# ikergarcia1996/AI-Generated-GTAV

Measured on AMD Instinct MI355X. Metric: generated frames/sec (32-frame clip, 100 noise steps), higher is better.
Workload: dtype fp16 (fp32 accumulate/residual)

## Files before the change

### ai-generated-gtav_amd/csrc/api.hip

```cpp
#include "api_internal.h"

#include <type_traits>

namespace gtav_shared {
thread_local hipEvent_t g_launch_ev[2] = {nullptr, nullptr};
static thread_local char g_err[1024] = "";
void set_error(const char* fmt, ...) {
    va_list ap;
    va_start(ap, fmt);
    vsnprintf(g_err, sizeof(g_err), fmt, ap);
    va_end(ap);
}
const char* last_error() { return g_err; }
}

namespace {
template <class T> struct twin_arg { typedef T type; };
template <> struct twin_arg<const f16*> { typedef const __bf16* type; };
template <> struct twin_arg<f16*> { typedef __bf16* type; };
#define GTAV_TWIN_STRUCT(S)                                                                                                                     \
    static_assert(sizeof(S) == sizeof(gtav_bf16::S) && alignof(S) == alignof(gtav_bf16::S) && std::is_standard_layout<S>::value &&             \
                      std::is_standard_layout<gtav_bf16::S>::value, #S ": the fp16 and the bf16 view differ");                                  \
    template <> struct twin_arg<const S&> { typedef const gtav_bf16::S& type; };                                                                \
    template <> struct twin_arg<const S*> { typedef const gtav_bf16::S* type; };
GTAV_TWIN_STRUCT(GemmParams)
GTAV_TWIN_STRUCT(LnPending)
GTAV_TWIN_STRUCT(GemmDwGroup)
GTAV_TWIN_STRUCT(AdamParam)
GTAV_TWIN_STRUCT(AdamItem)
#undef GTAV_TWIN_STRUCT
template <class Sig, class TwinSig, TwinSig* Fn> struct twin_call;
template <class... A, class... B, int (*Fn)(B...)> struct twin_call<int(A...), int(B...), Fn> {
    static_assert((std::is_same<typename twin_arg<A>::type, B>::value && ...), "a bf16 twin's signature differs from its fp16 launcher's");
    template <class To, class From> static To cast(From a) {
        if constexpr (std::is_same<To, From>::value) return a;
        else return reinterpret_cast<To>(a);
    }
    static int call(A... a) { return Fn(cast<B, A>(a)...); }
};
#define GTAV_OPS_F16(field, launcher) &launcher,
#define GTAV_OPS_BF16(field, launcher) &twin_call<decltype(launcher), decltype(gtav_bf16::launcher), &gtav_bf16::launcher>::call,
const OperandOps OPS_F16 = {GTAV_OPERAND_OPS(GTAV_OPS_F16) false};
const OperandOps OPS_BF16 = {GTAV_OPERAND_OPS(GTAV_OPS_BF16) true};
#undef GTAV_OPS_F16
#undef GTAV_OPS_BF16
}
const OperandOps& gtav::operand_ops(bool bf16) { return bf16 ? OPS_BF16 : OPS_F16; }

static thread_local bool g_op_bf16 = false;
static const OperandOps& op_ops() { return operand_ops(g_op_bf16); }
#define GTAV_OP_F16_ONLY(name) GTAV_REQUIRE(!g_op_bf16, name ": fp16 operands only, there is no bf16 twin of this launch (gtav_op_set_operand_dtype)")

extern "C" {

const char* gtav_last_error(void) { return last_error(); }
int gtav_abi_version(void) { return 4; }

int gtav_clamp_frames(float* x, int32_t B, int32_t F, int32_t first, int32_t n, float lo, float hi, void* stream) {
    GTAV_REQUIRE(x && B >= 1 && first >= 0 && first <= F && n >= 1, "clamp_frames: bad arguments");
    if (first == F) return 0;
    GTAV_REQUIRE((int64_t)F * n < (int64_t)1 << 31, "clamp_frames: sample of %d x %d floats too large", F, n);
    return launch_clamp_cols(x, B, F * n, first * n, F * n, lo, hi, (hipStream_t)stream);
}
int gtav_ddim_update(const float* x, const float* v, float* out, int32_t rows, int32_t n, const float* alpha_t,
                     const float* alpha_next, int32_t is_final, void* stream) {
    GTAV_REQUIRE(x && v && out && alpha_t && (alpha_next || is_final), "ddim_update: null argument");
    return launch_ddim_update(x, n, v, n, out, n, rows, n, alpha_t, alpha_next, is_final, (hipStream_t)stream);
}
int gtav_add_noise(const float* x, const float* noise, const float* alpha, float* out, int32_t rows, int32_t n, float clamp_abs,
                   void* stream) {
    return launch_add_noise(x, noise, alpha, out, rows, n, clamp_abs, (hipStream_t)stream);
}
int gtav_vtarget(const float* x, const float* noise, const float* alpha, float* vt, int32_t rows, int32_t n, float clamp_abs,
                 void* stream) {
    return launch_vtarget(x, noise, alpha, vt, rows, n, clamp_abs, (hipStream_t)stream);
}
static bool aligned16(const void* p) { return ((uintptr_t)p & 15) == 0; }
#define GTAV_RNG_ROWS(name, rows, n)                                                                                                    \
// ... 409 lines not shown
```

### ai-generated-gtav_amd/csrc/api_dit.hip

```cpp
#include "api_internal.h"

#ifdef GTAV_EXPERIMENTS
static int fold_alloc(gtav_dit* h) {
    gtav_dit::Fold& f = h->fold;
    if (f.ok) return 0;
    GTAV_REQUIRE(f.geom_ok, "dit_set_fold: this geometry has no LayerNorm fold (tokens per frame %d must be a multiple of 16 and >= 64, hidden %% 256 == 0)", h->P);
    Arena& a = h->arena;
    const int D = h->D;
    const size_t Mx = round_up(h->Mmax, 128);
    int rc = 0;
#define A_(expr) do { if (!rc) rc = (expr); } while (0)
    {
        const int nhb = h->L * 2, nseam = 2 * nhb + 1;
        f.col_c.assign(nseam, 0);
        int col = 0;
        for (int hb = 0; hb < nhb; ++hb) { f.col_c[2 * hb + 1] = col; col += 2 * h->Hm; }
        for (int hb = 0; hb < nhb; ++hb) { f.col_c[2 * hb] = col; col += 2 * 3 * D; }
        f.col_c[2 * nhb] = col; col += 2 * h->Nfin;
        f.CTW = col;
        f.n_groups = 2 * nseam; f.n_groups_a = 2 * nhb;
        f.Rp = round_up(h->max_rows, 128);
        A_(a.alloc_t(&f.ctab, (size_t)h->max_rows * f.CTW));
        A_(a.alloc_t(&f.ctab_cur, (size_t)h->maxB * h->maxT * f.CTW));
        A_(a.alloc_t(&f.stats, Mx * (size_t)(D / 64) * 2));
// ... 72 lines not shown

static int dit_cond_mlp(gtav_dit* h, int rows, bool have_actions, hipStream_t s) {
    const int ldhc = h->D + h->Apad;
    RET_IF(launch_skinny_f32(h->E, 256, h->w_t0, h->b_t0, h->HC, ldhc, rows, h->D, 256, 1, s));
    RET_IF(launch_skinny_f32(h->HC, ldhc, h->w_t2cat, have_actions ? h->b_t2a : h->b_t2, h->Sc, h->D, rows, h->D, ldhc, 1, s));
    return launch_skinny_f32(h->Sc, h->D, h->w_ada, h->b_ada, h->mod, h->MODW, rows, h->MODW, h->D, 0, s);
}

static int dit_cond(gtav_dit* h, const int64_t* t64, int rows, int Tq, const StepParams* sp, int use_cur, const float* actions,
                    int64_t act_outer, int64_t act_inner, hipStream_t s) {
    GTAV_REQUIRE(rows <= h->max_rows, "conditioning rows %d exceed max_cond_rows %d", rows, h->max_rows);
    RET_IF(launch_cond_inputs(t64, rows, Tq, sp, use_cur, h->sincos, h->E, actions, act_outer, act_inner, h->A, h->HC, h->D + h->Apad,
                              h->D, h->Apad, h->err_flag, s));
    RET_IF(dit_cond_mlp(h, rows, actions != nullptr, s));
    bool fa, fb;
    fold_policy(h, rows * h->P, fa, fb);
    return dit_fold_tables(h, rows, fa, fb, s);
}

struct DitPrefetch {
    const gtav_dit* h;
    int M, Tq, t0;
    bool on;
    DitPrefetch(const gtav_dit* h_, int M_, int Tq_, int t0_) : h(h_), M(M_), Tq(Tq_), t0(t0_) {
        const int pf_max_m = 1536;
        static const int pf_min_m = GTAV_ENV_INT("GTAV_PF_MIN_M", 256);
        on = h->w_prefetch && M >= pf_min_m && M <= pf_max_m;
        fill_on = M <= pf_max_m;
    }
    bool fill_on;
    int fill(int cls) const { return fill_on ? h->w_fill_cls[cls] : 0; }
    PrefetchDesc after(int hb, int pos) const {
        const int q = pos + 1, hb2 = hb + q / 4, consumer = (q + 3) % 4;
        if (!on || hb2 >= 2 * h->L) return kNoPrefetch;
        const int v = h->w_prefetch_cls[consumer];
        if (!v) return kNoPrefetch;
        const gtav_dit::Half& w2 = h->halves[hb2];
        const int D = h->D;
        const f16* W; int N, K, sk = 1;
        if (consumer == 3) { W = dit_half_fused(h, hb2, M, Tq, t0) ? w2.w_qkv_hm : w2.w_qkv; N = 3 * D; K = D; }
        else if (consumer == 0) { W = w2.w_out; N = D; K = D; sk = gemm_choose_splitk(M, D, D); }
        else if (consumer == 1) { W = w2.w_fc1; N = h->Hm; K = D; }
        else { W = w2.w_fc2; N = D; K = h->Hm_pad; sk = gemm_choose_splitk(M, D, h->Hm_pad); }
        const int nkt = K / 64;
        if (sk < 1 || nkt % sk || (sk >= 8 ? sk % 8 : 8 % sk)) sk = 1;
        return PrefetchDesc{W, cdiv(N, 128), nkt, sk, v >= 2 ? v : 0};
    }
};

static bool dit_resid_inplace(const gtav_dit* h, int M, int K) {
    return gemm_pp_ok(M, h->D, K, EPI_RESID) || (gemm_choose_splitk(M, h->D, K) == 1 && M >= h->resid_inplace_min_m) || gemm_resid_inplace_ok(M, h->D, K, h->P);
}

static int dit_forward_core(gtav_dit* h, const float* x_src, const int* frame_index, int B, int Tq, int t0,
                            const float* mod, const int* mod_rows, const float* ctab, float* v_out, hipStream_t s) {
    const int D = h->D, P = h->P, NB = B * Tq, M = NB * P;
    GTAV_REQUIRE(M <= h->Mmax, "forward: %d tokens exceed workspace (%d)", M, h->Mmax);
    bool fold_a, fold_b;
    fold_policy(h, M, fold_a, fold_b);
    const DitPrefetch pf(h, M, Tq, t0);
    DeferredResid rd{h->parts, h->parts_rows * (size_t)D, h->resid, M, D, &h->prof, s};
    auto gate = [&](const float* g) { return ResidGate{g, h->MODW, mod_rows, P}; };
    auto ln = [&](const OperandOps& o, const float* shift, const float* scale, int* ef) -> int {
        PROF(h, PC_LN, s, o.ln_modulate(h->resid, D, h->xn, D, M, D, shift, scale, h->MODW, mod_rows, P, rd.take(), ef, s));
        return 0;
    };
    const int g_embed = 2 * h->L, g_final = 2 * h->L + 1;
    PROF(h, PC_OTHER, s, h->ops(g_embed).patchify(x_src, frame_index, NB, h->C, h->H, h->W, h->p, h->xp, h->Kpe, 1.f, 0.f, h->err_of(g_embed), s));
    GemmParams pe = gemm_params(h->xp, h->Kpe, h->w_pe, M, D, h->Kpe);
    pe.bias = h->b_pe; pe.out = h->resid; pe.ldo = D;
    PROF(h, PC_OTHER, s, h->ops(g_embed).gemm(pe, EPI_F32, s));
    bool folded_in = false;
    for (int hb = 0; hb < 2 * h->L; ++hb) {
        const int l = hb / 2, hf = hb % 2;
        const gtav_dit::Half& w = h->halves[hb];
        const OperandOps& ops = h->ops(hb);
        int* const ef = h->err_of(hb);
        const float* mb = mod + (size_t)hb * 6 * D;
        const bool fused = dit_half_fused(h, hb, M, Tq, t0), fused_t = fused && hf == 1, fused_s = fused && hf == 0 && !folded_in;
        if (fused_t) rd.permute_rows(Tq, P);
        if (!folded_in) RET_IF(ln(ops, mb, mb + D, ef));
        GemmParams g = gemm_params(h->xn, D, fused_t || fused_s ? w.w_qkv_hm : w.w_qkv, M, 3 * D, D);
        g.D = D; g.S = P; g.err_flag = ef; g.pf = pf.after(hb, 0); g.wfill = pf.fill(3);
        if (folded_in) fold_consumer(h, g, 2 * hb, 3 * D, mod_rows, ctab);
        if (hf == 0) { g.qkv_mode = QKV_SPATIAL; g.rope_cs = h->rope_s.cs_dev; }
        else { g.qkv_mode = QKV_TEMPORAL; g.k = h->kvcache[l]; g.v = h->kvcache[l]; g.Tq = Tq; g.t0 = t0; g.Tmax = h->maxT; g.rope_cs = h->rope_t.cs_dev; }
        if (fused_t || fused_s) {
            g.out = h->ao; g.ldo = D;
            if (fused_t) PROF(h, PC_ATTN_T, s, launch_gemm_qkvt_attn(g, s));
            else PROF(h, PC_ATTN_S, s, launch_gemm_qkvs_attn(g, s));
        } else {
            if (hf == 0) { g.q = h->qs; g.k = h->ks; g.v = h->vts; }
            else g.q = h->qt;
            PROF(h, PC_QKV, s, ops.gemm(g, folded_in ? EPI_QKV_FOLD : EPI_QKV, s));
            if (hf == 0) PROF(h, PC_ATTN_S, s, ops.attn_spatial(h->qs, h->ks, h->vts, h->ao, NB, h->heads, P, s, false));
            else PROF(h, PC_ATTN_T, s, ops.attn_temporal(h->qt, h->kvcache[l], h->ao, B, P, D, Tq, t0, h->maxT, s));
        }
        folded_in = false;
        GemmParams fc1 = gemm_params(h->xn, D, w.w_fc1, M, h->Hm, D);
        fc1.bias = w.b_fc1; fc1.out = h->hbuf; fc1.ldo = h->Hm_pad; fc1.err_flag = ef; fc1.pf = pf.after(hb, 2); fc1.wfill = pf.fill(1);
        if (fold_a) {
            RET_IF(fold_producer(h, PC_OUT, h->ao, w.w_out, M, D, w.b_out, gate(mb + 2 * D), mb + 4 * D, s));
            fold_consumer(h, fc1, 2 * hb + 1, h->Hm, mod_rows, ctab);
            PROF(h, PC_FC1, s, launch_gemm(fc1, EPI_GELU_TANH_FOLD, s));
        } else {
            RET_IF(rd.gemm(ops, PC_OUT, h->ao, D, w.w_out, D, w.b_out, gate(mb + 2 * D), dit_resid_inplace(h, M, D), pf.after(hb, 1), nullptr, nullptr, pf.fill(0)));
            RET_IF(ln(ops, mb + 3 * D, mb + 4 * D, ef));
            PROF(h, PC_FC1, s, ops.gemm(fc1, EPI_GELU_TANH, s));
        }
        if (fold_b) {
            const float* next_scale = hb + 1 < 2 * h->L ? mod + (size_t)(hb + 1) * 6 * D + D : mod + (size_t)h->L * 12 * D + D;
            RET_IF(fold_producer(h, PC_FC2, h->hbuf, w.w_fc2, M, h->Hm_pad, w.b_fc2, gate(mb + 5 * D), next_scale, s));
            folded_in = true;
        } else {
            RET_IF(rd.gemm(ops, PC_FC2, h->hbuf, h->Hm_pad, w.w_fc2, h->Hm_pad, w.b_fc2, gate(mb + 5 * D), dit_resid_inplace(h, M, h->Hm_pad), pf.after(hb, 3), nullptr, nullptr, pf.fill(2)));
        }
    }
    const float* mf = mod + (size_t)h->L * 12 * D;
    if (!folded_in) RET_IF(ln(h->ops(g_final), mf, mf + D, h->err_of(g_final)));
    GemmParams fin = gemm_params(h->xn, D, h->w_final, M, h->Nfin, D);
    fin.bias = h->b_final; fin.out = h->fo; fin.ldo = h->Nfin;
    if (folded_in) fold_consumer(h, fin, 4 * h->L, h->Nfin, mod_rows, ctab);
    PROF(h, PC_OTHER, s, h->ops(g_final).gemm(fin, folded_in ? EPI_F32_FOLD : EPI_F32, s));
    PROF(h, PC_OTHER, s, launch_unpatchify(h->fo, h->Nfin, v_out, NB, h->C, h->H, h->W, h->p, 0, 1.f, 0.f, s));
    return h->prof.collect(s);
}

extern "C" {

int gtav_dit_create(const gtav_dit_config* c, gtav_dit** out) {
    GTAV_REQUIRE(c && out, "dit_create: null argument");
    GTAV_REQUIRE(c->hidden_size % 256 == 0 && c->hidden_size <= 2048, "hidden_size=%d must be a multiple of 256, <= 2048", c->hidden_size);
    GTAV_REQUIRE(c->num_heads > 0 && c->hidden_size / c->num_heads == 64 && c->hidden_size % c->num_heads == 0,
                 "only head_dim 64 is implemented (hidden %d, heads %d)", c->hidden_size, c->num_heads);
    GTAV_REQUIRE(c->input_h % c->patch_size == 0 && c->input_w % c->patch_size == 0, "input %dx%d not divisible by patch %d",
                 c->input_h, c->input_w, c->patch_size);
    GTAV_REQUIRE(c->max_frames >= 1 && c->max_frames <= 32, "max_frames=%d must be in [1, 32]", c->max_frames);
    GTAV_REQUIRE(c->max_batch >= 1 && c->depth >= 1, "bad max_batch/depth");
    RET_IF(skinny_init());
    gtav_dit* h = new gtav_dit();
    h->cfg = *c;
    h->D = c->hidden_size; h->L = c->depth; h->heads = c->num_heads; h->C = c->in_channels; h->p = c->patch_size;
    h->H = c->input_h; h->W = c->input_w; h->gh = h->H / h->p; h->gw = h->W / h->p; h->P = h->gh * h->gw;
    const int D = h->D;
    if ((h->P % 8) != 0) {
        set_error("tokens per frame P=%d must be a multiple of 8", h->P);
        delete h;
        return 2;
    }
    h->Hm = (int)(D * c->mlp_ratio); h->Hm_pad = round_up(h->Hm, 128);
    h->A = c->external_cond_dim > 0 ? c->external_cond_dim : 0; h->Apad = round_up(h->A > 0 ? h->A : 1, 32);
    h->MODW = h->L * 12 * D + 2 * D;
    h->Kpe = round_up(h->C * h->p * h->p, 64);
    h->Nfin = h->p * h->p * h->C;
    h->maxB = c->max_batch; h->maxT = c->max_frames; h->Mmax = h->maxB * h->maxT * h->P;
    h->max_rows = c->max_cond_rows > h->maxB * h->maxT ? c->max_cond_rows : h->maxB * h->maxT;
    Arena& a = h->arena;
    WeightTable& wt = h->wt;
    int rc = 0;
#define A_(expr) do { if (!rc) rc = (expr); } while (0)
    A_(a.alloc_t(&h->w_pe, (size_t)round_up(D, 128) * h->Kpe));
    h->n_groups = 2 * h->L + 2;
    h->grp_bf16.assign(h->n_groups, 0);
    wt.add_f16("x_embedder.proj.weight", D, h->C * h->p * h->p, h->w_pe, round_up(D, 128), h->Kpe, 2 * h->L);
    A_(a.alloc_t(&h->b_pe, D)); wt.add_f32("x_embedder.proj.bias", 1, D, h->b_pe, D);
    A_(a.alloc_t(&h->w_t0, (size_t)D * 256)); wt.add_f32("t_embedder.mlp.0.weight", D, 256, h->w_t0, 256);
    A_(a.alloc_t(&h->b_t0, D)); wt.add_f32("t_embedder.mlp.0.bias", 1, D, h->b_t0, D);
    const int ldhc = D + h->Apad;
    A_(a.alloc_t(&h->w_t2cat, (size_t)D * ldhc)); wt.add_f32("t_embedder.mlp.2.weight", D, D, h->w_t2cat, ldhc, 0);
    A_(a.alloc_t(&h->b_t2, D)); wt.add_f32("t_embedder.mlp.2.bias", 1, D, h->b_t2, D);
    A_(a.alloc_t(&h->b_ext, D)); A_(a.alloc_t(&h->b_t2a, D));
    if (h->A > 0) {
        wt.add_f32("external_cond.weight", D, h->A, h->w_t2cat, ldhc, D);
        wt.add_f32("external_cond.bias", 1, D, h->b_ext, D);
    }
// ... 1 lines not shown
    h->halves.resize(h->L * 2);
    h->fuse_sattn = h->P == 144 && D % 256 == 0;
    for (int l = 0; l < h->L && !rc; ++l)
        for (int hf = 0; hf < 2; ++hf) {
            gtav_dit::Half& w = h->halves[l * 2 + hf];
            char pre[64];
            snprintf(pre, sizeof(pre), "blocks.%d.%c_", l, hf == 0 ? 's' : 't');
            std::string P_(pre);
            const int grp = l * 2 + hf;
            A_(a.alloc_t(&w.w_qkv, (size_t)3 * D * D)); wt.add_f16(P_ + "attn.to_qkv.weight", 3 * D, D, w.w_qkv, 3 * D, D, grp);
            w.w_qkv_hm = nullptr;
            if (hf == 0 && h->P == 144 && D % 256 == 0) A_(a.alloc_t(&w.w_qkv_hm, (size_t)3 * D * D));
            A_(a.alloc_t(&w.w_out, (size_t)D * D)); wt.add_f16(P_ + "attn.to_out.weight", D, D, w.w_out, D, D, grp);
            A_(a.alloc_t(&w.b_out, D)); wt.add_f32(P_ + "attn.to_out.bias", 1, D, w.b_out, D);
            A_(a.alloc_t(&w.w_fc1, (size_t)h->Hm_pad * D)); wt.add_f16(P_ + "mlp.fc1.weight", h->Hm, D, w.w_fc1, h->Hm_pad, D, grp);
            A_(a.alloc_t(&w.b_fc1, h->Hm_pad)); wt.add_f32(P_ + "mlp.fc1.bias", 1, h->Hm, w.b_fc1, h->Hm);
            A_(a.alloc_t(&w.w_fc2, (size_t)D * h->Hm_pad)); wt.add_f16(P_ + "mlp.fc2.weight", D, h->Hm, w.w_fc2, D, h->Hm_pad, grp);
            A_(a.alloc_t(&w.b_fc2, D)); wt.add_f32(P_ + "mlp.fc2.bias", 1, D, w.b_fc2, D);
            const size_t row0 = (size_t)(l * 2 + hf) * 6 * D;
            wt.add_f32(P_ + "adaLN_modulation.1.weight", 6 * D, D, h->w_ada + row0 * D, D);
            wt.add_f32(P_ + "adaLN_modulation.1.bias", 1, 6 * D, h->b_ada + row0, 6 * D);
        }
    A_(a.alloc_t(&h->w_final, (size_t)round_up(h->Nfin, 128) * D));
    wt.add_f16("final_layer.linear.weight", h->Nfin, D, h->w_final, round_up(h->Nfin, 128), D, 2 * h->L + 1);
    A_(a.alloc_t(&h->b_final, round_up(h->Nfin, 128))); wt.add_f32("final_layer.linear.bias", 1, h->Nfin, h->b_final, h->Nfin);
    {
        const size_t row0 = (size_t)h->L * 12 * D;
        wt.add_f32("final_layer.adaLN_modulation.1.weight", 2 * D, D, h->w_ada + row0 * D, D);
        wt.add_f32("final_layer.adaLN_modulation.1.bias", 1, 2 * D, h->b_ada + row0, 2 * D);
    }
    A_(a.alloc_t(&h->sincos, (size_t)1000 * 256)); wt.add_f32("tables.timestep_sincos", 1000, 256, h->sincos, 256, 0, false);
    h->rope_s.npos = h->P; h->rope_t.npos = h->maxT;
    A_(a.alloc_t(&h->rope_s.cos_dev, (size_t)h->P * 64)); wt.add_f32("tables.rope_spatial_cos", h->P, 64, h->rope_s.cos_dev, 64, 0, false);
    A_(a.alloc_t(&h->rope_s.sin_dev, (size_t)h->P * 64)); wt.add_f32("tables.rope_spatial_sin", h->P, 64, h->rope_s.sin_dev, 64, 0, false);
    A_(a.alloc_t(&h->rope_t.cos_dev, (size_t)h->maxT * 64)); wt.add_f32("tables.rope_temporal_cos", h->maxT, 64, h->rope_t.cos_dev, 64, 0, false);
    A_(a.alloc_t(&h->rope_t.sin_dev, (size_t)h->maxT * 64)); wt.add_f32("tables.rope_temporal_sin", h->maxT, 64, h->rope_t.sin_dev, 64, 0, false);
    A_(a.alloc_t(&h->rope_s.cs_dev, (size_t)h->P * 64)); A_(a.alloc_t(&h->rope_t.cs_dev, (size_t)h->maxT * 64));
    A_(a.alloc_t(&h->freqs_s_dev, 16)); wt.add_f32("spatial_rotary_emb.freqs", 1, 16, h->freqs_s_dev, 16, 0, false);
    A_(a.alloc_t(&h->freqs_t_dev, 32)); wt.add_f32("temporal_rotary_emb.freqs", 1, 32, h->freqs_t_dev, 32, 0, false);
    const size_t Mx = round_up(h->Mmax, 128);
    A_(a.alloc_t(&h->xp, Mx * h->Kpe)); A_(a.alloc_t(&h->xn, Mx * D)); A_(a.alloc_t(&h->qs, Mx * D)); A_(a.alloc_t(&h->ks, Mx * D));
    A_(a.alloc_t(&h->vts, Mx * D)); A_(a.alloc_t(&h->qt, Mx * D)); A_(a.alloc_t(&h->ao, Mx * D)); A_(a.alloc_t(&h->hbuf, Mx * h->Hm_pad));
    h->kvcache.resize(h->L);
    for (int l = 0; l < h->L; ++l) A_(a.alloc_t(&h->kvcache[l], Mx * 2 * D));
    A_(a.alloc_t(&h->resid, Mx * D)); A_(a.alloc_t(&h->fo, Mx * h->Nfin));
    A_(a.alloc_t(&h->vout, Mx / h->P * h->C * h->H * h->W));
    h->parts_rows = (2 * Mx * D > (size_t)(8u << 20) ? 2 * Mx * D : (size_t)(8u << 20)) / D;
    A_(a.alloc_t(&h->parts, h->parts_rows * D));
    const size_t R = h->max_rows;
    A_(a.alloc_t(&h->E, R * 256)); A_(a.alloc_t(&h->HC, R * ldhc)); A_(a.alloc_t(&h->Sc, R * D)); A_(a.alloc_t(&h->mod, R * h->MODW));
    A_(a.alloc_t(&h->err_flag, 4 + h->n_groups)); A_(a.alloc_t(&h->frame_idx, (size_t)h->maxB * h->maxT)); A_(a.alloc_t(&h->ac_table, 1000));
    A_(a.alloc_t(&h->step_dev, 4)); A_(a.alloc_t(&h->mod_rows_dev, (size_t)h->maxB * h->maxT));
    A_(a.alloc_t(&h->mod_cur, (size_t)h->maxB * h->maxT * h->MODW)); A_(a.alloc_t(&h->mod_last, (size_t)h->maxB * h->maxT)); A_(a.alloc_t(&h->mod_changed, (size_t)h->maxB * h->maxT)); A_(a.alloc_t(&h->t_steps_dev, 1024));
    wt.err_words = h->err_flag; wt.err_per_group = true;
    h->use_graph = GTAV_ENV_INT("GTAV_GRAPH", 1) != 0;
    h->fold.geom_ok = h->P % 16 == 0 && h->P >= 64 && D % 256 == 0 && h->Hm % 128 == 0 && h->Nfin % 4 == 0;
#undef A_
    if (rc) {
        delete h;
        return rc;
    }
    *out = h;
    return 0;
}

void gtav_dit_destroy(gtav_dit* h) { delete h; }

int gtav_dit_set_weight(gtav_dit* h, const char* name, const float* src, int64_t numel, void* stream) {
    GTAV_REQUIRE(h && name && src, "dit_set_weight: null argument");
    std::string n(name);
    if (n.size() > 16 && n.compare(n.size() - 16, 16, "rotary_emb.freqs") == 0) {
        const bool spatial = n.rfind("spatial_", 0) == 0 || n.find(".s_attn.") != std::string::npos;
        n = spatial ? "spatial_rotary_emb.freqs" : "temporal_rotary_emb.freqs";
    }
    h->finalized = false;
    return h->wt.set(n.c_str(), src, numel, (hipStream_t)stream);
}

int gtav_dit_get_weight(gtav_dit* h, const char* name, float* dst, int64_t numel, void* stream) {
    GTAV_REQUIRE(h && name && dst, "dit_get_weight: null argument");
    return h->wt.get(name, dst, numel, (hipStream_t)stream);
}

int gtav_dit_finalize(gtav_dit* h, void* stream) {
    GTAV_REQUIRE(h, "dit_finalize: null handle");
    hipStream_t s = (hipStream_t)stream;
    RET_IF(h->wt.check_complete());
    GTAV_CHECK_HIP(hipStreamSynchronize(s));
    const int D = h->D;
    RET_IF(launch_add_f32(h->b_t2, h->b_ext, h->b_t2a, D, s));
    std::vector<float> fs(16), ft(32);
    if (h->wt.is_set("spatial_rotary_emb.freqs")) GTAV_CHECK_HIP(hipMemcpy(fs.data(), h->freqs_s_dev, 64, hipMemcpyDeviceToHost));
    else { std::vector<float> l = linspace_f32(1.0f, 128.0f, 16); for (int i = 0; i < 16; ++i) fs[i] = l[i] * (float)M_PI; }
    if (h->wt.is_set("temporal_rotary_emb.freqs")) GTAV_CHECK_HIP(hipMemcpy(ft.data(), h->freqs_t_dev, 128, hipMemcpyDeviceToHost));
    else for (int i = 0; i < 32; ++i) ft[i] = 1.0f / powf(10000.0f, (float)(2 * i) / 64.0f);
    if (!(h->wt.is_set("tables.rope_spatial_cos") && h->wt.is_set("tables.rope_spatial_sin"))) {
        std::vector<float> c, sn;
        build_axial_table(fs, h->gh, h->gw, c, sn);
        RET_IF(upload(h->rope_s.cos_dev, c)); RET_IF(upload(h->rope_s.sin_dev, sn));
    }
    if (!(h->wt.is_set("tables.rope_temporal_cos") && h->wt.is_set("tables.rope_temporal_sin"))) {
        std::vector<float> c((size_t)h->maxT * 64), sn((size_t)h->maxT * 64);
        for (int t = 0; t < h->maxT; ++t)
            for (int d = 0; d < 64; ++d) {
                const float ang = (float)t * ft[d / 2];
                c[t * 64 + d] = cosf(ang); sn[t * 64 + d] = sinf(ang);
            }
        RET_IF(upload(h->rope_t.cos_dev, c)); RET_IF(upload(h->rope_t.sin_dev, sn));
    }
    if (!h->wt.is_set("tables.timestep_sincos")) {
        std::vector<float> tab((size_t)1000 * 256);
        for (int k = 0; k < 128; ++k) {
            const float f = expf(-logf(10000.0f) * (float)k / 128.0f);
            for (int t = 0; t < 1000; ++t) {
                const float arg = (float)t * f;
                tab[(size_t)t * 256 + k] = cosf(arg);
                tab[(size_t)t * 256 + 128 + k] = sinf(arg);
            }
        }
        RET_IF(upload(h->sincos, tab));
    }
    for (size_t hb = 0; hb < h->halves.size(); ++hb) {
        gtav_dit::Half& w = h->halves[hb];
        if (w.w_qkv_hm) RET_IF(launch_qkv_head_major(w.w_qkv, w.w_qkv_hm, D, s, (hb & 1) ? 0 : 1));
    }
    RET_IF(launch_rope_interleave(h->rope_s.cos_dev, h->rope_s.sin_dev, h->rope_s.cs_dev, h->P, s));
    RET_IF(launch_rope_interleave(h->rope_t.cos_dev, h->rope_t.sin_dev, h->rope_t.cs_dev, h->maxT, s));
    GTAV_CHECK_HIP(hipStreamSynchronize(s));
    h->finalized = true;
    return 0;
}

int gtav_dit_forward(gtav_dit* h, const float* x, const int64_t* t, const float* actions, float* out, int32_t B, int32_t T,
                     void* stream) {
    GTAV_REQUIRE(h && x && t && out, "dit_forward: null argument");
    GTAV_REQUIRE(h->finalized, "dit_forward: call gtav_dit_finalize first");
    GTAV_REQUIRE(B >= 1 && B <= h->maxB && T >= 1 && T <= h->maxT, "dit_forward: B=%d T=%d outside capacity (%d, %d)", B, T, h->maxB, h->maxT);
    GTAV_REQUIRE(!actions || h->A > 0, "dit_forward: model has no external_cond");
    hipStream_t s = (hipStream_t)stream;
    h->prepared.valid = false;
    h->kvrec.valid = false;
    RET_IF(dit_cond(h, t, B * T, 1, nullptr, 0, actions, h->A, 0, s));
    return dit_forward_core(h, x, nullptr, B, T, 0, h->mod, nullptr, h->fold.ctab, out, s);
}

int gtav_dit_set_schedule(gtav_dit* h, const float* ac, int32_t n) {
    GTAV_REQUIRE(h && ac && n == 1000, "dit_set_schedule: expected 1000 alphas_cumprod values");
    h->ac_host.assign(ac, ac + n);
    GTAV_CHECK_HIP(hipMemcpy(h->ac_table, ac, n * sizeof(float), hipMemcpyHostToDevice));
    return 0;
}

static int denoise_step_body(gtav_dit* h, float* x, int B, int F, int T, const float* actions, int mode, float* v_out,
                             bool prepared, hipStream_t s) {
    const size_t fsz = (size_t)h->C * h->H * h->W;
    const int Tq = mode == 1 ? 1 : T, t0 = mode == 1 ? T - 1 : 0;
    if (!prepared) RET_IF(dit_cond(h, nullptr, B * Tq, Tq, h->step_dev, mode == 1, actions, (int64_t)F * h->A, h->A, s));
    RET_IF(dit_forward_core(h, x, h->frame_idx, B, Tq, t0, prepared ? h->mod_cur : h->mod, nullptr, prepared ? h->fold.ctab_cur : h->fold.ctab, h->vout, s));
    const float* vlast = h->vout + (size_t)(Tq - 1) * fsz;
    RET_IF(launch_ddim_update_step(x, F, vlast, (size_t)Tq * fsz, B, (int)fsz, h->step_dev, s));
    if (v_out) RET_IF(launch_copy_rows_f32(vlast, (size_t)Tq * fsz, v_out, fsz, B, fsz, s));
    return 0;
}

int gtav_dit_prepare_frame(gtav_dit* h, int32_t B, int32_t F, int32_t start, int32_t cur, int32_t t_ctx,
                           const int32_t* t_steps_host, int32_t n_steps, const float* actions, void* stream) {
    GTAV_REQUIRE(h && t_steps_host, "prepare_frame: null argument");
    GTAV_REQUIRE(h->finalized, "prepare_frame: finalize the model first");
    const int T = cur - start + 1;
    GTAV_REQUIRE(start >= 0 && cur < F && T >= 1 && T <= h->maxT && B >= 1 && B <= h->maxB && n_steps >= 1 && n_steps <= 1024,
                 "prepare_frame: bad window [%d, %d] / steps %d", start, cur, n_steps);
    GTAV_REQUIRE(!actions || h->A > 0, "prepare_frame: model has no external_cond");
    const int rows = B * (T - 1) + n_steps * B;
    GTAV_REQUIRE(rows <= h->max_rows, "prepare_frame: %d conditioning rows exceed max_cond_rows %d", rows, h->max_rows);
    hipStream_t s = (hipStream_t)stream;
    GTAV_CHECK_HIP(hipStreamSynchronize(s));
    GTAV_CHECK_HIP(hipMemcpy(h->t_steps_dev, t_steps_host, n_steps * sizeof(int), hipMemcpyHostToDevice));
    RET_IF(launch_cond_inputs_frame(rows, B, T, F, start, cur, t_ctx, h->t_steps_dev, h->sincos, h->E, actions, h->A, h->HC, h->D + h->Apad,
                                    h->D, h->Apad, h->err_flag, s));
    RET_IF(dit_cond_mlp(h, rows, actions != nullptr, s));
    {
        bool fa, fb, fa1, fb1;
        fold_policy(h, B * T * h->P, fa, fb);
        fold_policy(h, B * h->P, fa1, fb1);
        RET_IF(dit_fold_tables(h, rows, fa || fa1, fb || fb1, s));
        h->prepared.fold_tables = fa || fa1 || fb || fb1;
    }
    GTAV_CHECK_HIP(hipMemsetAsync(h->mod_last, 0xFF, (size_t)h->maxB * h->maxT * sizeof(int), s));
    h->prepared.valid = true; h->prepared.B = B; h->prepared.F = F; h->prepared.start = start; h->prepared.cur = cur;
    h->prepared.n_steps = n_steps; h->prepared.actions = actions;
    return 0;
}

static int dit_step_graph(gtav_dit* h, float* x, int B, int F, int T, const float* actions, int mode, float* v_out, bool prepared, hipGraphExec_t* out) {
    *out = nullptr;
    const gtav_dit::GraphKey key{B, F, T, mode * 2 + (prepared ? 1 : 0), x, actions, v_out};
    auto it = h->graphs.find(key);
    if (it == h->graphs.end()) {
        if (h->graphs.size() > 64) h->drop_graphs();
        h->graphs[key] = nullptr;
        return 0;
    }
    *out = it->second;
    if (*out) return 0;
    hipGraph_t graph = nullptr;
    hipGraphExec_t exec = nullptr;
    int rc = 0;
    bool ok = h->cap_stream || hipStreamCreateWithFlags(&h->cap_stream, hipStreamNonBlocking) == hipSuccess;
    if (ok && hipStreamBeginCapture(h->cap_stream, hipStreamCaptureModeThreadLocal) != hipSuccess) {
        (void)hipGetLastError();
        ok = false;
    } else if (ok) {
        rc = denoise_step_body(h, x, B, F, T, actions, mode, v_out, prepared, h->cap_stream);
        ok = hipStreamEndCapture(h->cap_stream, &graph) == hipSuccess && !rc && graph;
        ok = ok && hipGraphInstantiate(&exec, graph, nullptr, nullptr, 0) == hipSuccess && exec;
        if (graph) (void)hipGraphDestroy(graph);
    }
    if (ok) *out = it->second = exec;
    else h->use_graph = false;
    return rc;
}

int gtav_dit_denoise_step(gtav_dit* h, float* x, int32_t B, int32_t F, int32_t start, int32_t cur, int32_t t_ctx,
                          int32_t t_cur, int32_t t_next, int32_t is_final, const float* actions, int32_t mode,
                          int32_t cond_step, float* v_out, void* stream) {
    GTAV_REQUIRE(h && x, "denoise_step: null argument");
    GTAV_REQUIRE(h->finalized && !h->ac_host.empty(), "denoise_step: finalize the model and set the schedule first");
    const int T = cur - start + 1;
    GTAV_REQUIRE(start >= 0 && cur < F && T >= 1 && T <= h->maxT && B >= 1 && B <= h->maxB, "denoise_step: bad window [%d, %d] of %d frames", start, cur, F);
    GTAV_REQUIRE(t_cur >= 0 && t_cur < 1000 && t_next >= 0 && t_next < 1000 && t_ctx >= 0 && t_ctx < 1000, "denoise_step: timestep out of range");
    GTAV_REQUIRE(!actions || h->A > 0, "denoise_step: model has no external_cond");
    GTAV_REQUIRE(mode == 0 || mode == 1, "denoise_step: mode %d", mode);
    const bool prepared = cond_step >= 0;
    if (prepared)
        GTAV_REQUIRE(h->prepared.valid && h->prepared.B == B && h->prepared.F == F && h->prepared.start == start &&
                         h->prepared.cur == cur && cond_step < h->prepared.n_steps && h->prepared.actions == actions,
                     "denoise_step: cond_step=%d but gtav_dit_prepare_frame was not called for this window", cond_step);
    else
        h->prepared.valid = false;
    if (mode == 1) {
        GTAV_REQUIRE(h->kvrec.valid && h->kvrec.B == B && h->kvrec.F == F && h->kvrec.start == start && h->kvrec.cur == cur &&
                         h->kvrec.x == (const void*)x,
                     "denoise_step: context-cached step (mode 1) on window [%d, %d] without a preceding full-window step (mode 0) "
                     "on the same batch / window / latent buffer: the temporal K/V caches would be stale", start, cur);
    } else {
        h->kvrec.valid = true; h->kvrec.B = B; h->kvrec.F = F; h->kvrec.start = start; h->kvrec.cur = cur; h->kvrec.x = x;
    }
    hipStream_t s = (hipStream_t)stream;
    StepParams sp;
    sp.first = start; sp.cur = cur; sp.t_ctx = t_ctx; sp.t_cur = t_cur; sp.is_final = is_final != 0;
    sp.alpha_t = h->ac_host[t_cur]; sp.alpha_next = h->ac_host[t_next]; sp.cond_step = cond_step;
    RET_IF(launch_step_setup(h->step_dev, sp, h->frame_idx, h->mod_rows_dev, prepared ? h->mod_last : nullptr, h->mod_changed, B, mode == 1 ? 1 : T, T, F,
                             mode == 1, s));
    if (prepared) RET_IF(launch_gather_rows(h->mod, h->mod_rows_dev, h->mod_changed, h->mod_cur, B * (mode == 1 ? 1 : T), h->MODW,
                                            h->prepared.fold_tables ? h->fold.ctab : nullptr, h->fold.ctab_cur, h->fold.CTW, s));
    hipGraphExec_t exec = nullptr;
    if (h->use_graph && !h->prof.on) RET_IF(dit_step_graph(h, x, B, F, T, actions, mode, v_out, prepared, &exec));
    if (!exec) return denoise_step_body(h, x, B, F, T, actions, mode, v_out, prepared, s);
    GTAV_CHECK_HIP(hipGraphLaunch(exec, s));
    return 0;
}

int gtav_dit_set_graph(gtav_dit* h, int32_t enable) {
    GTAV_REQUIRE(h, "dit_set_graph: null handle");
    h->use_graph = enable != 0;
    return 0;
}

int gtav_dit_set_weight_prefetch(gtav_dit* h, int32_t enable) {
    GTAV_REQUIRE(h, "dit_set_weight_prefetch: null handle");
    GTAV_REQUIRE(enable == 0 || enable == 1 || (enable >> 16) == 1,
                 "dit_set_weight_prefetch: mode %d (0 off, 1 on, 0x10000 | per-class nibbles: bits 0-3 out-proj's weight, 4-7 fc1's, 8-11 fc2's, 12-15 to_qkv's; "
                 "nibble 0 = not prefetched, 1 = the whole slice, k >= 2 = the first k K tiles of every row tile)", enable);
    int cls[4];
    for (int c = 0; c < 4; ++c) cls[c] = enable == 0 ? 0 : enable == 1 ? 1 : (enable >> (4 * c)) & 15;
    const bool on = cls[0] || cls[1] || cls[2] || cls[3];
    if (h->w_prefetch != on || memcmp(cls, h->w_prefetch_cls, sizeof(cls))) h->drop_graphs();
    h->w_prefetch = on;
    memcpy(h->w_prefetch_cls, cls, sizeof(cls));
    return 0;
}

int gtav_dit_set_weight_fill_policy(gtav_dit* h, int32_t mode) {
    GTAV_REQUIRE(h, "dit_set_weight_fill_policy: null handle");
    GTAV_REQUIRE((mode & ~0x1111) == 0,
                 "dit_set_weight_fill_policy: mode %d (one nibble per class: bits 0-3 out-proj's weight, 4-7 fc1's, 8-11 fc2's, 12-15 to_qkv's; "
                 "nibble 0 = default cache policy, 1 = non-temporal fills)", mode);
    int cls[4];
    for (int c = 0; c < 4; ++c) cls[c] = (mode >> (4 * c)) & 15;
    if (memcmp(cls, h->w_fill_cls, sizeof(cls))) h->drop_graphs();
    memcpy(h->w_fill_cls, cls, sizeof(cls));
    return 0;
}

#ifdef GTAV_EXPERIMENTS
int gtav_dit_set_fold(gtav_dit* h, int32_t mode, int32_t min_tokens_a, int32_t min_tokens_b) {
    GTAV_REQUIRE(h && mode >= 0 && mode <= 2, "dit_set_fold: mode %d", mode);
    if (min_tokens_a >= 0) h->fold.min_m_a = min_tokens_a;
    if (min_tokens_b >= 0) h->fold.min_m_b = min_tokens_b;
    if (mode == 2 || (mode == 1 && (h->fold.min_m_a < (1 << 30) || h->fold.min_m_b < (1 << 30)))) RET_IF(fold_alloc(h));
    h->drop_graphs();
    h->prepared.valid = false;
    h->fold.mode = mode;
    return 0;
}
#endif

static int dit_set_fused(gtav_dit* h, bool& flag, int hf, bool geom_ok, bool enable) {
    if (flag != enable) h->drop_graphs();
    if (enable && geom_ok) {
        for (int l = 0; l < h->L; ++l) {
            gtav_dit::Half& w = h->halves[l * 2 + hf];
            if (w.w_qkv_hm) continue;
            RET_IF(h->arena.alloc_t(&w.w_qkv_hm, (size_t)3 * h->D * h->D));
            if (h->finalized) RET_IF(launch_qkv_head_major(w.w_qkv, w.w_qkv_hm, h->D, nullptr, hf ? 0 : 1));
        }
        if (h->finalized) GTAV_CHECK_HIP(hipDeviceSynchronize());
    }
    flag = enable;
    return 0;
}
int gtav_dit_set_fused_temporal(gtav_dit* h, int32_t enable) {
    GTAV_REQUIRE(h, "dit_set_fused_temporal: null handle");
    return dit_set_fused(h, h->fuse_tattn, 1, h->P % 16 == 0 && h->D % 256 == 0 && h->maxT >= 5, enable != 0);
}
int gtav_dit_set_fused_spatial(gtav_dit* h, int32_t enable) {
    GTAV_REQUIRE(h, "dit_set_fused_spatial: null handle");
    return dit_set_fused(h, h->fuse_sattn, 0, h->P == 144 && h->D % 256 == 0, enable != 0);
}

int gtav_dit_fused_launches(gtav_dit* h, int32_t B, int32_t T, int32_t t0) {
    if (!h || B < 1 || T < 1) return 0;
    int mask = 0;
    for (int hb = 0; hb < 2 * h->L; ++hb)
        if (dit_half_fused(h, hb, B * T * h->P, T, t0)) mask |= (hb & 1) ? 2 : 1;
    return mask;
}

int gtav_dit_profile(gtav_dit* h, int32_t enable) {
    GTAV_REQUIRE(h, "dit_profile: null handle");
    h->prof.reset(enable != 0);
    return 0;
}
int gtav_dit_profile_read(gtav_dit* h, double* ms_by_class, int64_t* launches_by_class) {
    GTAV_REQUIRE(h && ms_by_class && launches_by_class, "dit_profile_read: null argument");
    h->prof.read(ms_by_class, launches_by_class);
    return 0;
}

static int dit_read_err_words(gtav_dit* h, std::vector<int>& words, hipStream_t s) {
    words.assign(4 + h->n_groups, 0);
    GTAV_CHECK_HIP(hipMemcpyAsync(words.data(), h->err_flag, words.size() * sizeof(int), hipMemcpyDeviceToHost, s));
    GTAV_CHECK_HIP(hipStreamSynchronize(s));
    GTAV_CHECK_HIP(hipMemsetAsync(h->err_flag, 0, words.size() * sizeof(int), s));
    return 0;
}

int gtav_dit_check(gtav_dit* h, void* stream) {
    GTAV_REQUIRE(h, "dit_check: null handle");
    std::vector<int> w;
    RET_IF(dit_read_err_words(h, w, (hipStream_t)stream));
    int flag = w[0] | w[1];
    for (int g = 0; g < h->n_groups; ++g) flag |= w[4 + g];
    return report_err_flag(flag, "DiT");
}

int gtav_dit_set_operand_dtype(gtav_dit* h, int32_t group, int32_t dtype) {
    GTAV_REQUIRE(h, "dit_set_operand_dtype: null handle");
    GTAV_REQUIRE(dtype == GTAV_OPERAND_F16 || dtype == GTAV_OPERAND_BF16, "dit_set_operand_dtype: dtype %d (0 = fp16, 1 = bf16)", dtype);
    GTAV_REQUIRE(group >= -1 && group < h->n_groups, "dit_set_operand_dtype: group %d outside [-1, %d)", group, h->n_groups);
    if (h->tr.on && h->tr.bf16)
        GTAV_REQUIRE(dtype == GTAV_OPERAND_BF16, "dit_set_operand_dtype: a bf16 training handle keeps bf16 operands in every group (its masters, optimizer state and "
                     "loss scale were set up for them; create a new handle to train on fp16 operands)");
    else
        GTAV_REQUIRE(!h->tr.on || dtype == GTAV_OPERAND_F16, "dit_set_operand_dtype: a training handle keeps fp16 operands (its backward pass and loss scaling are fp16)");
    int changed = 0;
    for (int g = (group < 0 ? 0 : group); g < (group < 0 ? h->n_groups : group + 1); ++g) {
        if ((h->grp_bf16[g] != 0) == (dtype == GTAV_OPERAND_BF16)) continue;
        GTAV_REQUIRE(!(h->tr.on && h->tr.mixed), "dit_set_operand_dtype: group %d of this training handle has the other type; a training handle changes it with "
                     "gtav_dit_train_set_group_dtype", g);
        h->grp_bf16[g] = dtype == GTAV_OPERAND_BF16;
        changed += 1 + h->wt.set_dtype(g, dtype == GTAV_OPERAND_BF16);
    }
    if (changed) {
        h->finalized = false;
        h->kvrec.valid = false;
        h->drop_graphs();
    }
    h->any_bf16 = false;
    for (unsigned char b : h->grp_bf16) h->any_bf16 |= b != 0;
    return 0;
}

int gtav_dit_get_operand_dtype(gtav_dit* h, int32_t group, int32_t* dtype) {
    GTAV_REQUIRE(h && dtype && group >= 0 && group < h->n_groups, "dit_get_operand_dtype: bad argument (group %d of %d)", group, h ? h->n_groups : 0);
    *dtype = h->grp_bf16[group] ? GTAV_OPERAND_BF16 : GTAV_OPERAND_F16;
    return 0;
}

int gtav_dit_operand_groups(gtav_dit* h, int32_t* n_groups) {
    GTAV_REQUIRE(h && n_groups, "dit_operand_groups: null argument");
    *n_groups = h->n_groups;
    return 0;
}

int gtav_dit_autorange(gtav_dit* h, int32_t* n_switched, void* stream) {
    GTAV_REQUIRE(h && n_switched, "dit_autorange: null argument");
    *n_switched = 0;
    std::vector<int> w;
    RET_IF(dit_read_err_words(h, w, (hipStream_t)stream));
    int other = w[0];
    for (int g = 0; g < h->n_groups; ++g) {
        other |= w[4 + g] & ~ERR_F16_SAT;
        if ((w[4 + g] & ERR_F16_SAT) && !h->grp_bf16[g]) {
            RET_IF(gtav_dit_set_operand_dtype(h, g, GTAV_OPERAND_BF16));
            *n_switched += 1;
        }
    }
    return report_err_flag(other, "DiT");
}

}
```

### ai-generated-gtav_amd/csrc/api_internal.h

```cpp
#pragma once
#include "../../include/gtav_amd.h"
#include "../../include/gtav_amd_testing.h"
#include "ops.h"
#include "ops_bf16.h"

#include <cmath>
#include <cstdarg>
#include <cstdio>
#include <cstdlib>
#include <cstring>
#include <map>
#include <string>
#include <tuple>
#include <vector>

using namespace gtav;

#define RET_IF(expr)            \
    do {                        \
        int _rc = (expr);       \
        if (_rc) return _rc;    \
    } while (0)

namespace gtav {
// ... 268 lines not shown
        GTAV_REQUIRE(!pending, "train_block_forward: a re-run starts from a stored block input");
        memset(&pend, 0, sizeof(pend));
        pend.k_load = k;
        pending = true;
        return 0;
    }
};

}
}
using namespace gtav::api;

struct gtav_dit {
    Profiler prof;
    gtav_dit_config cfg;
    int D, L, heads, P, gh, gw, C, p, H, W, Hm, Hm_pad, A, Apad, MODW, Kpe, Nfin, maxB, maxT, Mmax, max_rows;
    Arena arena;
    WeightTable wt;
    f16 *w_pe = nullptr, *w_final = nullptr;
    struct Half { f16 *w_qkv, *w_out, *w_fc1, *w_fc2; float *b_out, *b_fc1, *b_fc2; f16* w_qkv_hm; };
    std::vector<Half> halves;
    float *b_pe = nullptr, *b_final = nullptr;
    float *w_t0, *b_t0, *w_t2cat, *b_t2, *b_ext, *b_t2a, *w_ada, *b_ada;
    float* sincos = nullptr;
    bool sincos_set = false;
    RopeTable rope_s, rope_t;
    std::vector<float> freqs_s, freqs_t;
    float *freqs_s_dev = nullptr, *freqs_t_dev = nullptr;
    f16 *xp, *xn, *qs, *ks, *vts, *qt, *ao, *hbuf;
    std::vector<f16*> kvcache;
    float *resid, *fo, *vout, *E, *HC, *Sc, *mod, *parts;
    size_t parts_rows = 0;
    int* err_flag = nullptr;
    std::vector<unsigned char> grp_bf16;
    int n_groups = 0;
    bool any_bf16 = false;
    const OperandOps& ops(int g) const { return operand_ops(grp_bf16[g] != 0); }
    int* err_of(int g) const { return err_flag + 4 + g; }
    int* frame_idx = nullptr;
    StepParams* step_dev = nullptr;
    int* mod_rows_dev = nullptr;
    float* mod_cur = nullptr;
    int *mod_last = nullptr, *mod_changed = nullptr;
    int* t_steps_dev = nullptr;
    struct { bool valid = false, fold_tables = false; int B = 0, F = 0, start = 0, cur = 0, n_steps = 0; const float* actions = nullptr; } prepared;
    struct { bool valid = false; int B = 0, F = 0, start = 0, cur = 0; const void* x = nullptr; } kvrec;
    struct GraphKey {
        int B, F, T, mode;
        const void *x, *actions, *vout;
        bool operator<(const GraphKey& o) const {
            return std::tie(B, F, T, mode, x, actions, vout) < std::tie(o.B, o.F, o.T, o.mode, o.x, o.actions, o.vout);
        }
    };
    std::map<GraphKey, hipGraphExec_t> graphs;
    bool use_graph = true;
    bool fuse_tattn = false;
    bool fuse_sattn = false;
    bool w_prefetch = true;
    int w_prefetch_cls[4] = {1, 4, 4, 1};
    int w_fill_cls[4] = {0, 0, 0, 0};
    int resid_inplace_min_m = GTAV_ENV_INT("GTAV_RESID_INPLACE_MIN_M", 1 << 30);
    struct Fold {
        bool geom_ok = false;
        bool ok = false;
        int mode = 1;
        int min_m_a = 1 << 30, min_m_b = 1 << 30;
        int CTW = 0, n_groups = 0, n_groups_a = 0, Rp = 0;
        std::vector<int> col_c;
        float *ctab = nullptr, *ctab_cur = nullptr, *stats = nullptr;
        f16* sx = nullptr;
        GemmGroup* groups_dev = nullptr;
        int *gcol_dev = nullptr, *gscale_dev = nullptr;
    } fold;
    hipStream_t cap_stream = nullptr;
    void drop_graphs() {
        for (auto& kv : graphs)
            if (kv.second) (void)hipGraphExecDestroy(kv.second);
        graphs.clear();
    }
    ~gtav_dit() {
        drop_graphs();
        if (cap_stream) (void)hipStreamDestroy(cap_stream);
    }
    float* ac_table = nullptr;
    std::vector<float> ac_host;
    bool finalized = false;
    struct Train {
        bool on = false, have_fwd = false, have_actions = false;
        bool bf16 = false;
        bool mixed = false;
        int* range_words = nullptr;
        std::vector<AdamItem> adam_items_host;
        int adam_n[2] = {0, 0};
        int window = 8;
        bool recompute = false;
        int rc_block = -1;
        std::vector<float*> kshift;
        size_t saved_bytes = 0;
        int B = 0, T = 0, M = 0, Mp = 0, rows = 0;
        float loss_scale = 65536.0f;
        float grad_div = 1.0f;
        std::vector<Slot*> params;
        struct Linear { Slot *w = nullptr, *b = nullptr; };
        struct HalfSlots { Linear qkv, out, fc1, fc2, ada; };
        std::vector<HalfSlots> hs;
        Linear fin, fin_ada, pe, t0, t2, ext;
        float* grad_arena = nullptr;
        size_t grad_count = 0;
        float* ctl = nullptr;
        float *ln_part = nullptr;
        float *red_ws = nullptr, *sumsq_part = nullptr;
        size_t red_ws_floats = 0;
        AdamParam* adam_params = nullptr;
        AdamItem* adam_items = nullptr;
        int adam_n_items = 0;
        std::vector<float*> res;
        struct HB { f16 *xnA, *ao, *y1, *xnB, *u, *hh, *y2, *q, *k, *v; };
        std::vector<HB> hb;
        f16 *xnF = nullptr, *xp = nullptr;
        float *z0 = nullptr, *cpre = nullptr;
        float *dres = nullptr, *dtmp = nullptr, *stats = nullptr, *dmod = nullptr, *dSc = nullptr, *ada_part = nullptr, *dc = nullptr, *dh0 = nullptr, *dz0 = nullptr;
        f16 *g_d = nullptr, *g_d2 = nullptr, *g_h = nullptr, *g_u = nullptr, *g_qkv = nullptr, *dao = nullptr, *tA = nullptr, *tB = nullptr, *dfo = nullptr;
        f16 *tAg[4] = {nullptr, nullptr, nullptr, nullptr}, *tBg[4] = {nullptr, nullptr, nullptr, nullptr};
    } tr;
};
```

### ai-generated-gtav_amd/csrc/api_train.hip

```cpp
#include "api_internal.h"

static int g_dw_grouped = GTAV_ENV_INT("GTAV_DW_GROUPED", 1);
static int g_fuse_gelu_fwd = GTAV_ENV_INT("GTAV_FUSE_GELU_FWD", 1);
static int g_fuse_gelu = GTAV_ENV_INT("GTAV_FUSE_GELU_BWD", 1);
static int g_fuse_ln = GTAV_ENV_INT("GTAV_FUSE_LN_BWD", 1);
static int g_fuse_gate = GTAV_ENV_INT("GTAV_FUSE_GATE", 1);
static int g_dw_tn = GTAV_ENV_INT("GTAV_DW_TN", 1);

static int train_window_ok(const gtav_dit* h) {
    if (h->tr.window > 8) {
        GTAV_REQUIRE(h->maxT <= h->tr.window, "train_enable: gtav_dit_train_allow_window allowed training windows of at most %d frames on this handle; it was created "
                     "with max_frames=%d", h->tr.window, h->maxT);
        return 0;
    }
    GTAV_REQUIRE(h->maxT <= 8, "train_enable: training is implemented for windows of at most 8 frames (the backward temporal attention and the adaLN-gradient "
                 "reduction are sized for it); this handle was created with max_frames=%d", h->maxT);
    return 0;
}

static int train_linear(gtav_dit* h, const std::string& n, gtav_dit::Train::Linear* out, bool bias = true) {
    out->w = h->wt.find(n + ".weight");
    out->b = bias ? h->wt.find(n + ".bias") : nullptr;
    GTAV_REQUIRE(out->w && out->w->grad && (!bias || (out->b && out->b->grad)), "train_enable: the model has no trainable Linear '%s'", n.c_str());
    return 0;
// ... 260 lines not shown
    RET_IF(train_branch_seam(h, i - 1, gn, rd, s));
    RET_IF(h->ops(gn).ln_modulate(tr.res[2 * i - 1], D, last ? tr.xnF : tr.g_d, D, tr.M, D, mb, mb + D, h->MODW, nullptr, h->P, rd.take(), train_fwd_err(h, gn), s));
    tr.rc_block = l;
    return 0;
}

extern "C" {


int gtav_dit_train_param_count(gtav_dit* h, int64_t* numel) {
    GTAV_REQUIRE(h && numel, "train_param_count: null argument");
    int64_t c = 0;
    for (auto& kv : h->wt.slots)
        if (WeightTable::trainable_name(kv.first)) c += (int64_t)kv.second.R * kv.second.C;
    *numel = c;
    return 0;
}

int gtav_dit_set_loss_scale(gtav_dit* h, float scale) {
    GTAV_REQUIRE(h && scale > 0.f, "set_loss_scale: bad argument");
    h->tr.loss_scale = scale;
    return 0;
}

int gtav_dit_set_grad_divisor(gtav_dit* h, float divisor) {
    GTAV_REQUIRE(h && h->tr.on && divisor >= 1.0f, "set_grad_divisor: bad argument");
    h->tr.grad_div = divisor;
    return 0;
}
int gtav_dit_zero_grad(gtav_dit* h, void* stream) {
    GTAV_REQUIRE(h && h->tr.on, "zero_grad: training is not enabled");
    RET_IF(launch_fill_f32(h->tr.grad_arena, h->tr.grad_count, 0.f, (hipStream_t)stream));
    if (h->tr.mixed) RET_IF(launch_err_fold(h->err_flag, nullptr, 1, h->n_groups, (hipStream_t)stream));
    return launch_err_clear(h->err_flag, ERR_F16_SAT | ERR_NONFINITE, (hipStream_t)stream);
}

int gtav_dit_get_grad(gtav_dit* h, const char* name, float* dst, int64_t numel, void* stream) {
    GTAV_REQUIRE(h && name && dst && h->tr.on, "get_grad: bad argument / training is not enabled");
    auto it = h->wt.slots.find(name);
    GTAV_REQUIRE(it != h->wt.slots.end() && it->second.grad, "get_grad: '%s' is not a trainable parameter", name);
    GTAV_REQUIRE(numel == (int64_t)it->second.R * it->second.C, "get_grad: '%s' size mismatch", name);
    GTAV_CHECK_HIP(hipMemcpyAsync(dst, it->second.grad, numel * sizeof(float), hipMemcpyDeviceToDevice, (hipStream_t)stream));
    return 0;
}

int gtav_dit_train_forward(gtav_dit* h, const float* x, const int64_t* t64, const float* actions, float* out, int32_t B, int32_t T, void* stream) {
    GTAV_REQUIRE(h && x && t64 && out, "train_forward: null argument");
    GTAV_REQUIRE(h->tr.on && h->finalized, "train_forward: call gtav_dit_train_enable, load the weights and finalize first");
    GTAV_REQUIRE(B >= 1 && B <= h->maxB && T >= 1 && T <= h->maxT, "train_forward: B=%d T=%d outside capacity (%d, %d)", B, T, h->maxB, h->maxT);
    GTAV_REQUIRE(!actions || h->A > 0, "train_forward: model has no external_cond");
    hipStream_t s = (hipStream_t)stream;
    gtav_dit::Train& tr = h->tr;
    const int D = h->D, P = h->P, NB = B * T, M = NB * P, L = h->L, rows = NB, ldhc = D + h->Apad;
    h->prepared.valid = false;
    h->kvrec.valid = false;
    tr.rc_block = -1;
    RET_IF(launch_cond_inputs(t64, rows, 1, nullptr, 0, h->sincos, h->E, actions, h->A, 0, h->A, h->HC, ldhc, D, h->Apad, h->err_flag, s));
    RET_IF(launch_skinny_f32(h->E, 256, h->w_t0, h->b_t0, tr.z0, D, rows, D, 256, 0, s));
    RET_IF(launch_silu(tr.z0, D, h->HC, ldhc, rows, D, s));
    RET_IF(launch_skinny_f32(h->HC, ldhc, h->w_t2cat, actions ? h->b_t2a : h->b_t2, tr.cpre, D, rows, D, ldhc, 0, s));
    RET_IF(launch_silu(tr.cpre, D, h->Sc, D, rows, D, s));
    RET_IF(launch_skinny_f32(h->Sc, D, h->w_ada, h->b_ada, h->mod, h->MODW, rows, h->MODW, D, 0, s));
    const float* mod = h->mod;
    const OperandOps& oe = h->ops(2 * L), &ofin = h->ops(2 * L + 1);
    RET_IF(oe.patchify(x, nullptr, NB, h->C, h->H, h->W, h->p, tr.xp, h->Kpe, 1.f, 0.f, train_fwd_err(h, 2 * L), s));
    GemmParams g = gemm_params(tr.xp, h->Kpe, h->w_pe, M, D, h->Kpe);
    g.bias = h->b_pe; g.out = tr.res[0]; g.ldo = D;
    RET_IF(oe.gemm(g, EPI_F32, s));
    DeferredResid rd{h->parts, h->parts_rows * (size_t)D, nullptr, M, D, nullptr, s};
    for (int l = 0; l < L; ++l) RET_IF(train_block_forward(h, l, B, T, false, rd, s));
    const float* mf = mod + (size_t)L * 12 * D;
    RET_IF(train_branch_seam(h, 2 * L - 1, 2 * L + 1, rd, s));
    RET_IF(ofin.ln_modulate(tr.res[4 * L - 1], D, tr.xnF, D, M, D, mf, mf + D, h->MODW, nullptr, P, rd.take(), train_fwd_err(h, 2 * L + 1), s));
    g = gemm_params(tr.xnF, D, h->w_final, M, h->Nfin, D);
    g.bias = h->b_final; g.out = h->fo; g.ldo = h->Nfin;
    RET_IF(ofin.gemm(g, EPI_F32, s));
    RET_IF(launch_unpatchify(h->fo, h->Nfin, out, NB, h->C, h->H, h->W, h->p, 0, 1.f, 0.f, s));
    if (tr.mixed) RET_IF(launch_err_fold(h->err_flag, tr.range_words, 0, h->n_groups, s));
    tr.B = B; tr.T = T; tr.M = M; tr.Mp = round_up(M, 64); tr.rows = rows; tr.have_actions = actions != nullptr; tr.have_fwd = true;
    tr.rc_block = L - 1;
    return 0;
}

int gtav_dit_train_get_residual(gtav_dit* h, int32_t k, float* dst, int64_t numel, void* stream) {
    GTAV_REQUIRE(h && dst && h->tr.on && h->tr.have_fwd, "train_get_residual: no saved forward");
    GTAV_REQUIRE(k >= 0 && k <= 4 * h->L, "train_get_residual: k=%d must be in [0, %d]", k, 4 * h->L);
    GTAV_REQUIRE(!h->tr.recompute || k % 4 == 0, "train_get_residual: k=%d is a state inside a block, which a handle in recompute mode (gtav_dit_train_set_recompute) "
                 "does not keep: k must be a multiple of 4 (block inputs, 4 * depth = the input of the final layer)", k);
    GTAV_REQUIRE(numel == (int64_t)h->tr.M * h->D, "train_get_residual: expected %lld elements", (long long)h->tr.M * h->D);
    GTAV_CHECK_HIP(hipMemcpyAsync(dst, h->tr.res[k], numel * sizeof(float), hipMemcpyDeviceToDevice, (hipStream_t)stream));
    return 0;
}

}

struct TrainBackward {
    gtav_dit* h;
    gtav_dit::Train& tr;
    hipStream_t s;
    const int D, P, L, B, T, M, Mp, NB, rows, Hp, MODW;
    const OperandOps* op;
    bool defer_dw = false, tn_dw, fuse_ln, fuse_gate, defer_bias;
    GemmDwGroup dwg[GEMM_DW_MAX_GROUPS];
    int ndw = 0;

    TrainBackward(gtav_dit* h_, hipStream_t s_)
        : h(h_), tr(h_->tr), s(s_), D(h->D), P(h->P), L(h->L), B(tr.B), T(tr.T), M(tr.M), Mp(tr.Mp), NB(B * T), rows(tr.rows), Hp(h->Hm_pad), MODW(h->MODW), op(&h->ops(2 * L + 1)) {
// ... 147 lines not shown
    GTAV_REQUIRE(h && v_pred && v_target, "train_backward: null argument");
    GTAV_REQUIRE(h->tr.on && h->tr.have_fwd, "train_backward: no saved forward (gtav_dit_train_forward)");
    GTAV_REQUIRE(phase_begin >= 0 && phase_begin <= phase_end && phase_end <= h->L + 2, "train_backward: phases [%d, %d) outside [0, %d]", phase_begin, phase_end,
                 h->L + 2);
    GTAV_REQUIRE(h->Nfin <= 64, "train_backward: a final projection wider than 64 features is not implemented");
    TrainBackward bw(h, (hipStream_t)stream);
    const int L = h->L;
    if (phase_begin <= 0 && 0 < phase_end) RET_IF(bw.final_layer(v_pred, v_target));
    for (int i = 2 * L - 1; i >= 0; --i) {
        const int l = i / 2, phase = L - l;
        if (phase < phase_begin || phase >= phase_end) continue;
        if (h->tr.recompute && h->tr.rc_block != l) RET_IF(train_rerun_block(h, l, bw.s));
        RET_IF(bw.half_block(i));
    }
    if (phase_begin <= L + 1 && L + 1 < phase_end) RET_IF(bw.embedders());
    return 0;
}

int gtav_dit_train_backward(gtav_dit* h, const float* v_pred, const float* v_target, void* stream) {
    GTAV_REQUIRE(h, "train_backward: null handle");
    return gtav_dit_train_backward_phases(h, v_pred, v_target, 0, h->L + 2, stream);
}

int gtav_dit_train_param_range(gtav_dit* h, const char* prefix, int64_t* offset, int64_t* count) {
    GTAV_REQUIRE(h && prefix && offset && count && h->tr.on, "train_param_range: bad argument / training is not enabled");
    const size_t plen = strlen(prefix);
    int64_t off = -1, cnt = 0, last_end = -1;
    for (auto& kv : h->wt.slots) {
        Slot& sl = kv.second;
        if (!sl.grad || kv.first.compare(0, plen, prefix) != 0) continue;
        const int64_t o = sl.grad - h->tr.grad_arena, n = (int64_t)sl.R * sl.C;
        if (off < 0) off = o;
        GTAV_REQUIRE(last_end < 0 || o == last_end, "train_param_range: parameters with prefix '%s' are not contiguous in the arena", prefix);
        last_end = o + n;
        cnt += n;
    }
    GTAV_REQUIRE(off >= 0, "train_param_range: no trainable parameter starts with '%s'", prefix);
    *offset = off;
    *count = cnt;
    return 0;
}

int gtav_dit_adamw_step(gtav_dit* h, float lr, float beta1, float beta2, float eps, float weight_decay, float max_grad_norm, void* stream) {
    GTAV_REQUIRE(h && h->tr.on, "adamw_step: training is not enabled");
    hipStream_t s = (hipStream_t)stream;
    gtav_dit::Train& tr = h->tr;
    if (tr.mixed) RET_IF(launch_err_fold(h->err_flag, tr.range_words, 0, h->n_groups, s));
    RET_IF(launch_sumsq(tr.grad_arena, tr.grad_count, tr.sumsq_part, s));
    RET_IF(launch_clip_coef(tr.ctl, tr.sumsq_part, sumsq_parts(tr.grad_count), 1.0f / (tr.loss_scale * tr.grad_div), max_grad_norm, beta1, beta2, h->err_flag, s));
    for (int ty = 0; ty < 2; ++ty)
        if (tr.adam_n[ty])
            RET_IF(operand_ops(ty != 0).adamw_multi(tr.adam_params, tr.adam_items + (ty ? tr.adam_n[0] : 0), tr.adam_n[ty], tr.ctl, lr, beta1, beta2, eps, weight_decay, s));
    RET_IF(launch_add_f32(h->b_t2, h->b_ext, h->b_t2a, h->D, s));
    h->prepared.valid = false;
    h->kvrec.valid = false;
    return 0;
}

}

static int train_partition_items(gtav_dit* h) {
    gtav_dit::Train& tr = h->tr;
    bool any_f16 = false;
    for (unsigned char b : h->grp_bf16) any_f16 |= b == 0;
    std::vector<AdamItem> part[2];
    for (const AdamItem& it : tr.adam_items_host) {
        const Slot* sl = tr.params[it.param];
        part[sl->kind == SLOT_F16_PAD ? (sl->bf16 ? 1 : 0) : (any_f16 ? 0 : 1)].push_back(it);
    }
    tr.adam_n[0] = (int)part[0].size(); tr.adam_n[1] = (int)part[1].size();
    part[0].insert(part[0].end(), part[1].begin(), part[1].end());
    GTAV_REQUIRE((int)part[0].size() == tr.adam_n_items, "train_set_group_dtype: the optimizer's work items do not add up");
    GTAV_CHECK_HIP(hipMemcpy(tr.adam_items, part[0].data(), part[0].size() * sizeof(AdamItem), hipMemcpyHostToDevice));
    return 0;
}

static int train_switch_groups(gtav_dit* h, int g0, int g1, bool bf16, hipStream_t s, int* n_changed) {
    int changed = 0;
    for (int g = g0; g < g1; ++g) {
        if ((h->grp_bf16[g] != 0) == bf16) continue;
        h->grp_bf16[g] = bf16;
        ++changed;
        for (auto& kv : h->wt.slots) {
            Slot& sl = kv.second;
            if (sl.kind != SLOT_F16_PAD || sl.group != g) continue;
            sl.bf16 = bf16;
            if (!sl.set) continue;
            GTAV_REQUIRE(sl.master, "train_set_group_dtype: '%s' has no fp32 master", kv.first.c_str());
            RET_IF(operand_ops(bf16).convert_pad(sl.master, sl.C, sl.R, sl.C, (f16*)sl.dst, sl.Rp, sl.Cp, 1.0f, 1, s, h->tr.range_words + g));
            if (sl.wT) RET_IF(operand_ops(bf16).convert_T(sl.master, sl.C, sl.R, sl.C, sl.wT, s));
        }
    }
    *n_changed = changed;
    if (!changed) return 0;
    h->any_bf16 = false;
    for (unsigned char b : h->grp_bf16) h->any_bf16 |= b != 0;
    h->tr.have_fwd = false;
    h->tr.rc_block = -1;
    h->prepared.valid = false;
    h->kvrec.valid = false;
    h->drop_graphs();
    GTAV_CHECK_HIP(hipStreamSynchronize(s));
    return train_partition_items(h);
}

static int train_mixed_handle(gtav_dit* h, const char* who) {
    GTAV_REQUIRE(h, "%s: null handle", who);
    GTAV_REQUIRE(h->tr.on, "%s: training is not enabled", who);
    GTAV_REQUIRE(h->tr.mixed, "%s: this training handle has one operand type for every group; opt in with gtav_dit_train_allow_mixed between gtav_dit_create and "
                 "gtav_dit_train_enable", who);
    return 0;
}

extern "C" {

int gtav_dit_train_set_group_dtype(gtav_dit* h, int32_t group, int32_t dtype, void* stream) {
    RET_IF(train_mixed_handle(h, "train_set_group_dtype"));
    GTAV_REQUIRE(dtype == GTAV_OPERAND_F16 || dtype == GTAV_OPERAND_BF16, "train_set_group_dtype: dtype %d (0 = fp16, 1 = bf16)", dtype);
    GTAV_REQUIRE(group >= -1 && group < h->n_groups, "train_set_group_dtype: group %d outside [-1, %d)", group, h->n_groups);
    int n = 0;
    return train_switch_groups(h, group < 0 ? 0 : group, group < 0 ? h->n_groups : group + 1, dtype == GTAV_OPERAND_BF16, (hipStream_t)stream, &n);
}

int gtav_dit_train_range_words(gtav_dit* h, int32_t* words_host, void* stream) {
    RET_IF(train_mixed_handle(h, "train_range_words"));
    GTAV_REQUIRE(words_host, "train_range_words: null argument");
    hipStream_t s = (hipStream_t)stream;
    static_assert(sizeof(int32_t) == sizeof(int), "the error words are 32-bit");
    GTAV_CHECK_HIP(hipMemcpyAsync(words_host, h->tr.range_words, (size_t)h->n_groups * sizeof(int), hipMemcpyDeviceToHost, s));
    GTAV_CHECK_HIP(hipStreamSynchronize(s));
    GTAV_CHECK_HIP(hipMemsetAsync(h->tr.range_words, 0, (size_t)h->n_groups * sizeof(int), s));
    return 0;
}

int gtav_dit_train_autorange(gtav_dit* h, const int32_t* merged_words_host, int32_t* n_switched, void* stream) {
    RET_IF(train_mixed_handle(h, "train_autorange"));
    GTAV_REQUIRE(n_switched, "train_autorange: null argument");
    *n_switched = 0;
    hipStream_t s = (hipStream_t)stream;
    std::vector<int32_t> sticky(h->n_groups, 0);
    if (merged_words_host) sticky.assign(merged_words_host, merged_words_host + h->n_groups);
    else RET_IF(gtav_dit_train_range_words(h, sticky.data(), stream));
    std::vector<int> w(4 + h->n_groups, 0);
    GTAV_CHECK_HIP(hipMemcpyAsync(w.data(), h->err_flag, w.size() * sizeof(int), hipMemcpyDeviceToHost, s));
    GTAV_CHECK_HIP(hipStreamSynchronize(s));
    GTAV_CHECK_HIP(hipMemsetAsync(h->err_flag, 0, w.size() * sizeof(int), s));
    int other = w[0] | w[1];
    for (int g = 0; g < h->n_groups; ++g) {
        other |= w[4 + g];
        const bool switch_it = (sticky[g] & ERR_F16_SAT) && !h->grp_bf16[g];
        other |= switch_it ? sticky[g] & ~ERR_F16_SAT : sticky[g];
        if (switch_it) {
// ... 59 lines not shown
```

### ai-generated-gtav_amd/csrc/common.h

```cpp
#pragma once
#include <hip/hip_runtime.h>
#include <hip/hip_fp16.h>
#include <hip/hip_ext.h>
#include <stdint.h>

#ifdef GTAV_BF16_OPERANDS
#define GTAV_F16_T __bf16
#else
#define GTAV_F16_T _Float16
#endif

namespace gtav {

typedef GTAV_F16_T f16;
typedef GTAV_F16_T f16x4 __attribute__((ext_vector_type(4)));
typedef GTAV_F16_T f16x8 __attribute__((ext_vector_type(8)));
typedef GTAV_F16_T f16x2 __attribute__((ext_vector_type(2)));
typedef float f32x4 __attribute__((ext_vector_type(4)));
typedef float f32x16 __attribute__((ext_vector_type(16)));

__device__ __forceinline__ f32x4 mfma16(f16x8 a, f16x8 b, f32x4 c, int, int, int) {
#ifdef GTAV_BF16_OPERANDS
    return __builtin_amdgcn_mfma_f32_16x16x32_bf16(a, b, c, 0, 0, 0);
#else
// ... 30 lines not shown
using gtav_shared::last_error;
#define GTAV_LAUNCH(kern, grid, block, shmem, stream, ...)                                                              \
    do {                                                                                                                \
        if (gtav_shared::g_launch_ev[0]) {                                                                                     \
            hipExtLaunchKernelGGL(kern, grid, block, shmem, stream, gtav_shared::g_launch_ev[0], gtav_shared::g_launch_ev[1], 0, __VA_ARGS__); \
            gtav_shared::g_launch_ev[0] = nullptr;                                                                             \
        } else {                                                                                                        \
            hipLaunchKernelGGL(kern, grid, block, shmem, stream, __VA_ARGS__);                                          \
        }                                                                                                               \
    } while (0)

#define GTAV_CHECK_HIP(expr)                                                              \
    do {                                                                                  \
        hipError_t _e = (expr);                                                           \
        if (_e != hipSuccess) {                                                           \
            gtav::set_error("%s failed: %s (%s:%d)", #expr, hipGetErrorString(_e), __FILE__, __LINE__); \
            return 1;                                                                     \
        }                                                                                 \
    } while (0)

#define GTAV_REQUIRE(cond, ...)                                                           \
    do {                                                                                  \
        if (!(cond)) {                                                                    \
            gtav::set_error(__VA_ARGS__);                                                 \
            return 2;                                                                     \
        }                                                                                 \
    } while (0)

#ifdef GTAV_EXPERIMENTS
#define GTAV_ENV_INT(name, dflt) (getenv(name) ? atoi(getenv(name)) : (dflt))
#define GTAV_DBG(p, bits) ((p).debug & (bits))
#define GTAV_LAB_BUILD true
#else
#define GTAV_ENV_INT(name, dflt) (dflt)
#define GTAV_DBG(p, bits) false
#define GTAV_LAB_BUILD false
#endif

static inline int cdiv(int a, int b) { return (a + b - 1) / b; }
static inline int round_up(int a, int b) { return cdiv(a, b) * b; }

__host__ __device__ __forceinline__ size_t tiled_off(int r, int k, int K) {
    return ((size_t)(r >> 7) * (size_t)(K >> 6) + (size_t)(k >> 6)) * 8192 + (size_t)((r & 127) * 64) +
           (size_t)(((((k >> 3) & 7) ^ (r & 7)) << 3) + (k & 7));
}

}
namespace gtav_shared {
struct PrefetchDesc {
    const void* next;
    int rt, nkt, splitk;
    int kt_limit;
};
}
namespace gtav {
using gtav_shared::PrefetchDesc;
__device__ __forceinline__ void l2_prefetch_slice(const PrefetchDesc& d, int xcd, int j, int nb, int t, int nt, unsigned& sink) {
    const int sk = d.splitk;
    int ks0, ksn, rt0, rtn;
    if (sk >= 8) {
        ksn = sk >> 3; ks0 = xcd * ksn; rt0 = 0; rtn = d.rt;
    } else {
        const int per = 8 / sk, part = xcd % per;
        ks0 = xcd / per; ksn = 1;
        rt0 = part * d.rt / per; rtn = (part + 1) * d.rt / per - rt0;
    }
    const int kpt = d.nkt / sk;
    const int lim = d.kt_limit > 0 && d.kt_limit < kpt ? d.kt_limit : kpt;
    const int per_rt = ksn * lim;
    const int lines = rtn * per_rt * 128;
    const int l0 = (int)((long long)lines * j / nb), l1 = (int)((long long)lines * (j + 1) / nb);
    for (int l = l0 + t; l < l1; l += nt) {
        const int tile = l >> 7, r = tile / per_rt, rem = tile - r * per_rt, sl = rem / lim, k = rem - sl * lim;
        const char* a = (const char*)d.next + ((size_t)(rt0 + r) * d.nkt + (size_t)(ks0 + sl) * kpt + k) * 16384 + (l & 127) * 128;
        asm volatile("global_load_dword %0, %1, off" : "+v"(sink) : "v"(a) : "memory");
    }
}
static inline bool prefetch_desc_ok(const PrefetchDesc& d) {
    return !d.next || (d.rt > 0 && d.nkt > 0 && d.splitk >= 1 && d.nkt % d.splitk == 0 && (d.splitk >= 8 ? d.splitk % 8 == 0 : 8 % d.splitk == 0));
}

#ifdef GTAV_BF16_OPERANDS
constexpr float F16_MAX = 3.3895313892515355e38f;
#else
constexpr float F16_MAX = 65504.0f;
#endif
constexpr int ERR_TIMESTEP = 1, ERR_F16_SAT = 2, ERR_NONFINITE = 4;
__device__ __forceinline__ f16x4 sat4(float a, float b, float c, float d, float& amax) {
    amax = __builtin_fmaxf(__builtin_fmaxf(__builtin_fabsf(a), __builtin_fabsf(b)), amax);
    amax = __builtin_fmaxf(__builtin_fmaxf(__builtin_fabsf(c), __builtin_fabsf(d)), amax);
    return f16x4{(f16)__builtin_amdgcn_fmed3f(a, -F16_MAX, F16_MAX), (f16)__builtin_amdgcn_fmed3f(b, -F16_MAX, F16_MAX),
                 (f16)__builtin_amdgcn_fmed3f(c, -F16_MAX, F16_MAX), (f16)__builtin_amdgcn_fmed3f(d, -F16_MAX, F16_MAX)};
}
__device__ __forceinline__ void sat_report(float amax, int* err_flag) {
    if (err_flag && amax > F16_MAX) atomicOr(err_flag, ERR_F16_SAT);
}

__device__ __forceinline__ float group8_sum(float v) {
    v += __builtin_bit_cast(float, __builtin_amdgcn_update_dpp(0, __builtin_bit_cast(int, v), 0xB1, 0xF, 0xF, true));
    v += __builtin_bit_cast(float, __builtin_amdgcn_update_dpp(0, __builtin_bit_cast(int, v), 0x4E, 0xF, 0xF, true));
    v += __builtin_bit_cast(float, __builtin_amdgcn_update_dpp(0, __builtin_bit_cast(int, v), 0x141, 0xF, 0xF, true));
    return v;
}

__device__ __forceinline__ float silu_f(float x) { return x / (1.0f + __expf(-x)); }

__device__ __forceinline__ float gelu_tanh_f(float x) {
    const float a = -2.0f * 1.4426950408889634f * 0.7978845608028654f, b = a * 0.044715f;
    const float e = __builtin_amdgcn_exp2f(x * __builtin_fmaf(x * x, b, a));
// ... 109 lines not shown
```

### ai-generated-gtav_amd/csrc/elementwise.hip

```cpp
#include "ops.h"

#include <cstdlib>
#include <type_traits>

#include <cstring>

namespace gtav {

namespace {

template <int MODE, int NV>
__global__ __launch_bounds__(256) void ln_wave_row_kernel(const float* __restrict__ x, int ldx, f16* __restrict__ out, int M, int D,
                                                          const float* __restrict__ p0, const float* __restrict__ p1, int mod_stride,
                                                          const int* __restrict__ rows, int rows_per_mod, int flags, int* err_flag) {
    const int lane = threadIdx.x & 63;
    const int m = blockIdx.x * 4 + (threadIdx.x >> 6);
    if (m >= M) return;
    const float* xr = x + (size_t)m * ldx;
    f32x4 v[NV], av[NV], bv[NV];
#pragma unroll
    for (int i = 0; i < NV; ++i) v[i] = *(const f32x4*)(xr + i * 256 + lane * 4);
    const float *a, *b;
    if (MODE == 0) {
        int row = m / rows_per_mod;
// ... 119 lines not shown
    if (lane == 0) { red[wid] = s1; red[8 + wid] = s2; }
    if (!LN_DBG(pd, 0x400)) __syncthreads();
    if (PEND && act) {
        float* xw = pd.x_out ? pd.x_out + (size_t)m * ldx + c : xr + c;
        if (LN_DBG(pd, 0x800)) {}
        else if (pd.flags & 1) store16_sc1(xw, v);
        else *(f32x4*)xw = v;
    }
    float t1 = 0.f, t2 = 0.f;
#pragma unroll
    for (int i = 0; i < 8; ++i) { t1 += i < nw ? red[i] : 0.f; t2 += i < nw ? red[8 + i] : 0.f; }
    const float m1 = t1 / (float)D;
    const float var = fmaxf(t2 / (float)D - m1 * m1, 0.f);
    const float rstd = 1.0f / sqrtf(var + 1e-6f);
    if (!act) return;
    const float dd[4] = {a0 - m1, a1 - m1, a2 - m1, a3 - m1};
    float yv[4], amax = 0.f;
#pragma unroll
    for (int e = 0; e < 4; ++e) {
        const float xh = dd[e] * rstd;
        if (MODE == 0) {
            const float sc = av[e] + 1e-6f;
            yv[e] = xh * (1.0f + sc) + bv[e];
        } else {
            yv[e] = xh * av[e] + bv[e];
        }
    }
    int mo = m;
    if (pd.tperm_T > 0) {
        const int fr = m / pd.tperm_P, pp = m - fr * pd.tperm_P, bb = fr / pd.tperm_T, tt = fr - bb * pd.tperm_T;
        mo = ((bb * (pd.tperm_P >> 4) + (pp >> 4)) * pd.tperm_T + tt) * 16 + (pp & 15);
    }
    if (!LN_DBG(pd, 0x1000)) store_f16x4_paired<1>(out + tiled_off(mo, c, D), sat4(yv[0], yv[1], yv[2], yv[3], amax), lane, pd.flags & 2);
    else if (yv[0] == 1.2345f) out[0] = (f16)yv[1];
    sat_report(amax, pd.err_flag);
}

__global__ __launch_bounds__(256) void branch_rows_kernel(const float* __restrict__ parts, int nsplit, size_t slab_stride, int ld, const float* __restrict__ bias,
                                                          f16* __restrict__ y, int N, size_t n4, int* err_flag) {
    const size_t i = (size_t)blockIdx.x * 256 + threadIdx.x;
    float am = 0.f;
    if (i < n4) {
        const int per_row = N >> 2;
        const size_t m = i / per_row;
        const int c = (int)(i - m * per_row) * 4;
        const float* pp = parts + m * ld + c;
        f32x4 acc = bias ? *(const f32x4*)(bias + c) : f32x4{0.f, 0.f, 0.f, 0.f};
        for (int sp = 0; sp < nsplit; ++sp) acc = acc + *(const f32x4*)(pp + (size_t)sp * slab_stride);
        *(f16x4*)(y + m * ld + c) = sat4(acc[0], acc[1], acc[2], acc[3], am);
    }
    sat_report(am, err_flag);
}

__global__ void patchify_kernel(const float* __restrict__ img, const int* __restrict__ frame_index, int NB, int C, int H,
                                int W, int p, f16* __restrict__ out, int ldo, float a, float b, int* err_flag) {
    const int gh = H / p, gw = W / p, Kp = C * p * p;
    const size_t total = (size_t)NB * gh * gw * ldo;
    for (size_t idx = (size_t)blockIdx.x * blockDim.x + threadIdx.x; idx < total; idx += (size_t)gridDim.x * blockDim.x) {
        const int k = (int)(idx % ldo);
        const size_t m = idx / ldo;
        float val = 0.f;
        if (k < Kp) {
            const int pw = k % p, ph = (k / p) % p, c = k / (p * p);
            const int x = (int)(m % gw), y = (int)((m / gw) % gh), nb = (int)(m / ((size_t)gw * gh));
            const int f = frame_index ? frame_index[nb] : nb;
            val = a * img[(((size_t)f * C + c) * H + (y * p + ph)) * W + (x * p + pw)] + b;
            if (!(__builtin_fabsf(val) <= F16_MAX)) {
                if (err_flag) atomicOr(err_flag, val != val || __builtin_isinf(val) ? ERR_NONFINITE : ERR_F16_SAT);
                if (val == val) val = __builtin_amdgcn_fmed3f(val, -F16_MAX, F16_MAX);
            }
        }
        out[tiled_off((int)m, k, ldo)] = (f16)val;
    }
}

__global__ __launch_bounds__(256) void patchify4_kernel(const float* __restrict__ img, const int* __restrict__ frame_index, int C, int H, int W, int p,
                                                      f16* __restrict__ out, int ldo, float a, float b, int* err_flag) {
    const int gh = H / p, gw = W / p, Kp = C * p * p, pp = p * p;
    const int m = blockIdx.x;
    const int x = m % gw, y = (m / gw) % gh, nb = m / (gw * gh);
    const int f = frame_index ? frame_index[nb] : nb;
    const float* base = img + ((size_t)f * C * H + (size_t)y * p) * W + x * p;
    int flags = 0;
    for (int k = 4 * threadIdx.x; k < ldo; k += 4 * blockDim.x) {
        float v[4] = {0.f, 0.f, 0.f, 0.f};
        if (k < Kp) {
            const int c = k / pp, rem = k - c * pp, ph = rem / p, pw = rem - ph * p;
            const float4 t = *(const float4*)(base + ((size_t)c * H + ph) * W + pw);
            v[0] = a * t.x + b; v[1] = a * t.y + b; v[2] = a * t.z + b; v[3] = a * t.w + b;
#pragma unroll
            for (int e = 0; e < 4; ++e)
                if (!(__builtin_fabsf(v[e]) <= F16_MAX)) {
                    flags |= (v[e] != v[e] || __builtin_isinf(v[e])) ? ERR_NONFINITE : ERR_F16_SAT;
                    if (v[e] == v[e]) v[e] = __builtin_amdgcn_fmed3f(v[e], -F16_MAX, F16_MAX);
                }
        }
        *(f16x4*)(out + tiled_off(m, k, ldo)) = f16x4{(f16)v[0], (f16)v[1], (f16)v[2], (f16)v[3]};
    }
    if (flags && err_flag) atomicOr(err_flag, flags);
}

__global__ void unpatchify_kernel(const float* __restrict__ y, int ldy, float* __restrict__ img, int NB, int C, int H, int W,
                                  int p, int order, float a, float b) {
    const int gh = H / p, gw = W / p;
    const size_t total = (size_t)NB * C * H * W;
    for (size_t idx = (size_t)blockIdx.x * blockDim.x + threadIdx.x; idx < total; idx += (size_t)gridDim.x * blockDim.x) {
        const int xx = (int)(idx % W), yy = (int)((idx / W) % H), c = (int)((idx / ((size_t)W * H)) % C);
        const int nb = (int)(idx / ((size_t)W * H * C));
        const int ph = yy % p, pw = xx % p;
        const size_t m = ((size_t)nb * gh + yy / p) * gw + xx / p;
        const int f = order == 0 ? (ph * p + pw) * C + c : (c * p + ph) * p + pw;
        img[idx] = a * y[m * ldy + f] + b;
    }
}

__global__ void convert_pad_f16_kernel(const float* __restrict__ src, int lds, int R, int C, f16* __restrict__ dst, int Rp,
                                       int Cp, float scale, int tiled, int* err_flag) {
    const size_t total = (size_t)Rp * Cp;
    bool sat = false;
    for (size_t idx = (size_t)blockIdx.x * blockDim.x + threadIdx.x; idx < total; idx += (size_t)gridDim.x * blockDim.x) {
        const int c = (int)(idx % Cp);
        const size_t r = idx / Cp;
        float v = 0.f;
        if (r < (size_t)R && c < C) v = src[r * lds + c] * scale;
        if (v == v) {
            sat |= __builtin_fabsf(v) > F16_MAX;
// ... 17 lines not shown
    const int i = blockIdx.x * blockDim.x + threadIdx.x;
    if (i < npos * 32) {
        const int pos = i >> 5, k = i & 31;
        cs[(size_t)pos * 64 + 2 * k] = cos_t[(size_t)pos * 64 + 2 * k];
        cs[(size_t)pos * 64 + 2 * k + 1] = sin_t[(size_t)pos * 64 + 2 * k];
    }
}

__global__ void fill_f32_kernel(float* dst, size_t n, float v) {
    for (size_t idx = (size_t)blockIdx.x * blockDim.x + threadIdx.x; idx < n; idx += (size_t)gridDim.x * blockDim.x) dst[idx] = v;
}

__global__ void axpy_f32_kernel(float* y, const float* x, float alpha, size_t n) {
    for (size_t idx = (size_t)blockIdx.x * blockDim.x + threadIdx.x; idx < n; idx += (size_t)gridDim.x * blockDim.x) y[idx] += alpha * x[idx];
}

__global__ void add_f32_kernel(const float* a, const float* b, float* out, size_t n) {
    for (size_t idx = (size_t)blockIdx.x * blockDim.x + threadIdx.x; idx < n; idx += (size_t)gridDim.x * blockDim.x)
        out[idx] = a[idx] + b[idx];
}

__global__ void step_setup_kernel(StepParams* dst, StepParams v, int* frame_idx, int* mod_rows, int* last_rows, int* changed, int B, int Tq, int T,
                                  int F, int use_cur) {
    if (threadIdx.x == 0) *dst = v;
    const int first = use_cur ? v.cur : v.first;
    for (int i = threadIdx.x; i < B * Tq; i += blockDim.x) {
        const int b = i / Tq, tl = i - b * Tq;
        frame_idx[i] = b * F + first + tl;
        if (v.cond_step >= 0) {
            const int tw = use_cur ? T - 1 : tl;
            const int r = tw < T - 1 ? b * (T - 1) + tw : B * (T - 1) + v.cond_step * B + b;
            mod_rows[i] = r;
            if (last_rows) {
                changed[i] = last_rows[i] != r;
                last_rows[i] = r;
            }
        }
    }
}

__global__ __launch_bounds__(256) void gather_rows_kernel(const float* __restrict__ table, const int* __restrict__ rows, const int* __restrict__ changed,
                                                          float* __restrict__ cur, int W, const float* __restrict__ table2, float* __restrict__ cur2, int W2) {
    const int slot = blockIdx.y;
    if (!changed[slot]) return;
    const int nb1 = (W + 1023) >> 10;
    if ((int)blockIdx.x < nb1) {
        const size_t c = ((size_t)blockIdx.x * 256 + threadIdx.x) * 4;
        if (c >= (size_t)W) return;
        *(f32x4*)(cur + (size_t)slot * W + c) = *(const f32x4*)(table + (size_t)rows[slot] * W + c);
    } else {
        const size_t c = ((size_t)(blockIdx.x - nb1) * 256 + threadIdx.x) * 4;
        if (c >= (size_t)W2) return;
        *(f32x4*)(cur2 + (size_t)slot * W2 + c) = *(const f32x4*)(table2 + (size_t)rows[slot] * W2 + c);
    }
}

__global__ __launch_bounds__(256) void ctab_inputs_kernel(const float* __restrict__ mod, int MODW, int R, int Rp, int D, const int* __restrict__ col,
                                                          const int* __restrict__ is_scale, f16* __restrict__ sx, size_t group_stride) {
    const int g = blockIdx.y;
    const size_t idx = (size_t)blockIdx.x * 256 + threadIdx.x;
    const int per_row = D >> 3;
    const int r = (int)(idx / per_row), k = (int)(idx - (size_t)r * per_row) * 8;
    if (r >= Rp) return;
    union { f16x8 h; u32x4 u; } o;
    if (r < R) {
        const float* src = mod + (size_t)r * MODW + col[g] + k;
        const f32x4 a = *(const f32x4*)src, b = *(const f32x4*)(src + 4);
        const bool sc = is_scale[g] != 0;
        float v[8] = {a[0], a[1], a[2], a[3], b[0], b[1], b[2], b[3]};
#pragma unroll
        for (int e = 0; e < 8; ++e) {
            float x = sc ? 1.0f + (v[e] + 1e-6f) : v[e];
            x = __builtin_amdgcn_fmed3f(x, -F16_MAX, F16_MAX);
            o.h[e] = (f16)x;
        }
    } else {
#pragma unroll
        for (int e = 0; e < 8; ++e) o.h[e] = (f16)0.f;
    }
    *(u32x4*)(sx + (size_t)g * group_stride + tiled_off(r, k, D)) = o.u;
}

__global__ void cond_inputs_frame_kernel(int rows, int B, int T, int F, int start, int cur, int t_ctx, const int* __restrict__ t_steps,
                                         const float* __restrict__ sincos, float* __restrict__ E,
                                         const float* __restrict__ actions, int A, float* __restrict__ HC, int ldhc, int D,
                                         int Apad, int* err_flag) {
    const int r = blockIdx.x;
    if (r >= rows) return;
    const int nctx = B * (T - 1);
    int t, b, frame;
    if (r < nctx) {
        b = r / (T - 1);
        frame = start + (r - b * (T - 1));
        t = t_ctx;
    } else {
        const int q = r - nctx;
        const int sidx = q / B;
        b = q - sidx * B;
        frame = cur;
        t = t_steps[sidx];
    }
    if (t < 0 || t > 999) {
        if (threadIdx.x == 0 && err_flag) atomicOr(err_flag, 1);
        t = t < 0 ? 0 : 999;
    }
    for (int j = threadIdx.x; j < 256; j += blockDim.x) E[(size_t)r * 256 + j] = sincos[(size_t)t * 256 + j];
    const float* arow = actions ? actions + ((size_t)b * F + frame) * A : nullptr;
    for (int j = threadIdx.x; j < Apad; j += blockDim.x) HC[(size_t)r * ldhc + D + j] = (arow && j < A) ? arow[j] : 0.f;
}

__global__ void cond_inputs_kernel(const int64_t* __restrict__ t64, int rows, int Tq, const StepParams* __restrict__ sp, int use_cur,
                                   const float* __restrict__ sincos, float* __restrict__ E, const float* __restrict__ actions,
                                   long long act_outer, long long act_inner, int A, float* __restrict__ HC, int ldhc, int D,
                                   int Apad, int* err_flag) {
    const int r = blockIdx.x;
    if (r >= rows) return;
    const int ro = r / Tq, ri = r - ro * Tq;
    long long t;
    int frame0 = 0;
    if (t64) {
        t = (long long)t64[r];
    } else {
        t = ri == Tq - 1 ? sp->t_cur : sp->t_ctx;
        frame0 = use_cur ? sp->cur : sp->first;
    }
    if (t < 0 || t > 999) {
        if (threadIdx.x == 0 && err_flag) atomicOr(err_flag, 1);
        t = t < 0 ? 0 : 999;
    }
    for (int j = threadIdx.x; j < 256; j += blockDim.x) E[(size_t)r * 256 + j] = sincos[(size_t)t * 256 + j];
    const float* arow = actions ? actions + ro * act_outer + (frame0 + ri) * act_inner : nullptr;
    for (int j = threadIdx.x; j < Apad; j += blockDim.x) HC[(size_t)r * ldhc + D + j] = (arow && j < A) ? arow[j] : 0.f;
}

__device__ __forceinline__ float ddim_one(float xc, float vp, float at, float an, int is_final) {
    const float x0 = sqrtf(at) * xc - sqrtf(1.0f - at) * vp;
    if (is_final) return x0;
    const float eps = (sqrtf(1.0f / at) * xc - x0) / sqrtf(1.0f / at - 1.0f);
    return sqrtf(an) * x0 + sqrtf(1.0f - an) * eps;
}

__global__ void ddim_update_kernel(const float* __restrict__ x, size_t x_stride, const float* __restrict__ v, size_t v_stride,
                                   float* __restrict__ out, size_t out_stride, int n, const float* __restrict__ alpha_t,
                                   const float* __restrict__ alpha_next, int is_final) {
    const int b = blockIdx.y;
    const float at = alpha_t[b];
    const float an = alpha_next ? alpha_next[b] : 1.f;
    for (int i = blockIdx.x * blockDim.x + threadIdx.x; i < n; i += gridDim.x * blockDim.x)
        out[b * out_stride + i] = ddim_one(x[b * x_stride + i], v[b * v_stride + i], at, an, is_final);
}

__global__ void ddim_update_step_kernel(float* __restrict__ x, size_t frames_per_sample, const float* __restrict__ v,
                                        size_t v_stride, int n, const StepParams* __restrict__ sp) {
    const int b = blockIdx.y;
    const float at = sp->alpha_t, an = sp->alpha_next;
    const int fin = sp->is_final;
    float* xf = x + ((size_t)b * frames_per_sample + sp->cur) * n;
    for (int i = blockIdx.x * blockDim.x + threadIdx.x; i < n; i += gridDim.x * blockDim.x)
        xf[i] = ddim_one(xf[i], v[b * v_stride + i], at, an, fin);
}

__device__ __forceinline__ float clamp_noise(float z, float clamp_abs) { return fminf(fmaxf(z, -clamp_abs), clamp_abs); }
__device__ __forceinline__ float add_noise_one(float x, float z, float sa, float s1) {
#pragma clang fp contract(off)
    return x * sa + s1 * z;
}
__device__ __forceinline__ float vtarget_one(float x, float z, float sa, float s1) {
#pragma clang fp contract(off)
    return sa * z - s1 * x;
}

__global__ void add_noise_kernel(const float* __restrict__ x, const float* __restrict__ noise, const float* __restrict__ alpha,
                                 float* __restrict__ out, int n, float clamp_abs) {
    const int r = blockIdx.y;
    const float a = alpha[r];
    const float sa = sqrtf(a), s1 = sqrtf(1.0f - a);
    for (int i = blockIdx.x * blockDim.x + threadIdx.x; i < n; i += gridDim.x * blockDim.x) {
        const size_t o = (size_t)r * n + i;
        out[o] = add_noise_one(x[o], clamp_noise(noise[o], clamp_abs), sa, s1);
    }
}

__global__ void vtarget_kernel(const float* __restrict__ x, const float* __restrict__ noise, const float* __restrict__ alpha,
                               float* __restrict__ vt, int n, float clamp_abs) {
    const int r = blockIdx.y;
    const float a = alpha[r];
    const float sa = sqrtf(a), s1 = sqrtf(1.0f - a);
    for (int i = blockIdx.x * blockDim.x + threadIdx.x; i < n; i += gridDim.x * blockDim.x) {
        const size_t o = (size_t)r * n + i;
        vt[o] = vtarget_one(x[o], clamp_noise(noise[o], clamp_abs), sa, s1);
    }
}
// ... 346 lines not shown

int launch_copy_f32(const float* src, int lds, int R, int C, float* dst, int ldd, int c0, hipStream_t stream) {
    hipLaunchKernelGGL(copy_f32_kernel, dim3(grid_for((size_t)R * C)), dim3(256), 0, stream, src, lds, R, C, dst, ldd, c0);
    GTAV_CHECK_HIP(hipGetLastError());
    return 0;
}

int launch_rope_interleave(const float* cos_t, const float* sin_t, float* cs, int npos, hipStream_t stream) {
    hipLaunchKernelGGL(rope_interleave_kernel, dim3(cdiv(npos * 32, 256)), dim3(256), 0, stream, cos_t, sin_t, cs, npos);
    GTAV_CHECK_HIP(hipGetLastError());
    return 0;
}

int launch_fill_f32(float* dst, size_t n, float v, hipStream_t stream) {
    hipLaunchKernelGGL(fill_f32_kernel, dim3(grid_for(n)), dim3(256), 0, stream, dst, n, v);
    GTAV_CHECK_HIP(hipGetLastError());
    return 0;
}

int launch_axpy_f32(float* y, const float* x, float alpha, size_t n, hipStream_t stream) {
    hipLaunchKernelGGL(axpy_f32_kernel, dim3(grid_for(n)), dim3(256), 0, stream, y, x, alpha, n);
    GTAV_CHECK_HIP(hipGetLastError());
    return 0;
}

int launch_calib_spin(unsigned long long ticks, unsigned long long* dev_ticks, hipStream_t stream) {
    GTAV_LAUNCH(calib_spin_kernel, dim3(1), dim3(64), 0, stream, ticks, dev_ticks);
    GTAV_CHECK_HIP(hipGetLastError());
    return 0;
}

int launch_add_f32(const float* a, const float* b, float* out, size_t n, hipStream_t stream) {
    hipLaunchKernelGGL(add_f32_kernel, dim3(grid_for(n)), dim3(256), 0, stream, a, b, out, n);
    GTAV_CHECK_HIP(hipGetLastError());
    return 0;
}

int launch_step_setup(StepParams* dst, const StepParams& v, int* frame_idx, int* mod_rows, int* last_rows, int* changed, int B, int Tq, int T, int F,
                      int use_cur, hipStream_t stream) {
    hipLaunchKernelGGL(step_setup_kernel, dim3(1), dim3(64), 0, stream, dst, v, frame_idx, mod_rows, last_rows, changed, B, Tq, T, F, use_cur);
    GTAV_CHECK_HIP(hipGetLastError());
    return 0;
}

int launch_gather_rows(const float* table, const int* rows, const int* changed, float* cur, int slots, int W, const float* table2, float* cur2, int W2,
                       hipStream_t stream) {
    GTAV_REQUIRE(W % 4 == 0 && W2 % 4 == 0 && slots > 0, "gather_rows: W=%d W2=%d slots=%d", W, W2, slots);
    hipLaunchKernelGGL(gather_rows_kernel, dim3(cdiv(W, 1024) + (table2 ? cdiv(W2, 1024) : 0), slots), dim3(256), 0, stream, table, rows, changed, cur, W,
                       table2, cur2, table2 ? W2 : 0);
    GTAV_CHECK_HIP(hipGetLastError());
    return 0;
}

int launch_ctab_inputs(const float* mod, int MODW, int R, int Rp, int D, const int* col, const int* is_scale, int n_groups, f16* sx, size_t group_stride,
                       hipStream_t stream) {
    GTAV_REQUIRE(D % 64 == 0 && Rp % 128 == 0 && R <= Rp && n_groups > 0, "ctab_inputs: bad geometry");
    const size_t threads = (size_t)Rp * (D >> 3);
    hipLaunchKernelGGL(ctab_inputs_kernel, dim3((unsigned)((threads + 255) / 256), n_groups), dim3(256), 0, stream, mod, MODW, R, Rp, D, col, is_scale, sx,
                       group_stride);
    GTAV_CHECK_HIP(hipGetLastError());
    return 0;
}

int launch_cond_inputs_frame(int rows, int B, int T, int F, int start, int cur, int t_ctx, const int* t_steps, const float* sincos,
                             float* E, const float* actions, int A, float* HC, int ldhc, int D, int Apad, int* err_flag,
                             hipStream_t stream) {
    hipLaunchKernelGGL(cond_inputs_frame_kernel, dim3(rows), dim3(256), 0, stream, rows, B, T, F, start, cur, t_ctx, t_steps, sincos,
                       E, actions, A, HC, ldhc, D, Apad, err_flag);
    GTAV_CHECK_HIP(hipGetLastError());
    return 0;
}

int launch_cond_inputs(const int64_t* t64, int rows, int Tq, const StepParams* sp, int use_cur, const float* sincos, float* E,
                       const float* actions, int64_t act_outer, int64_t act_inner, int A, float* HC, int ldhc, int D, int Apad,
                       int* err_flag, hipStream_t stream) {
    GTAV_REQUIRE(rows > 0 && Tq > 0 && (t64 || sp), "cond_inputs: bad rows/Tq/timesteps");
    hipLaunchKernelGGL(cond_inputs_kernel, dim3(rows), dim3(256), 0, stream, t64, rows, Tq, sp, use_cur, sincos, E, actions,
                       (long long)act_outer, (long long)act_inner, A, HC, ldhc, D, Apad, err_flag);
    GTAV_CHECK_HIP(hipGetLastError());
    return 0;
}

int launch_ddim_update(const float* x, size_t x_stride, const float* v, size_t v_stride, float* out, size_t out_stride,
                       int B, int n, const float* alpha_t, const float* alpha_next, int is_final, hipStream_t stream) {
    hipLaunchKernelGGL(ddim_update_kernel, dim3(cdiv(n, 256), B), dim3(256), 0, stream, x, x_stride, v, v_stride, out,
                       out_stride, n, alpha_t, alpha_next, is_final);
    GTAV_CHECK_HIP(hipGetLastError());
    return 0;
}

int launch_ddim_update_step(float* x, size_t frames_per_sample, const float* v, size_t v_stride, int B, int n,
                            const StepParams* sp, hipStream_t stream) {
    hipLaunchKernelGGL(ddim_update_step_kernel, dim3(cdiv(n, 256), B), dim3(256), 0, stream, x, frames_per_sample, v, v_stride,
                       n, sp);
    GTAV_CHECK_HIP(hipGetLastError());
    return 0;
}

int launch_add_noise(const float* x, const float* noise, const float* alpha, float* out, int rows, int n, float clamp_abs,
                     hipStream_t stream) {
    hipLaunchKernelGGL(add_noise_kernel, dim3(cdiv(n, 256), rows), dim3(256), 0, stream, x, noise, alpha, out, n, clamp_abs);
    GTAV_CHECK_HIP(hipGetLastError());
    return 0;
}

int launch_vtarget(const float* x, const float* noise, const float* alpha, float* vt, int rows, int n, float clamp_abs,
// ... 87 lines not shown
```

### ai-generated-gtav_amd/csrc/gemm.h

```cpp
#pragma once
#include "common.h"
#include "gemm_plan.h"

namespace gtav {

enum GemmEpi : int {
    EPI_F32 = 0,
    EPI_F16 = 1,
    EPI_GELU_TANH = 2,
    EPI_GELU_ERF = 3,
    EPI_RESID = 4,
    EPI_QKV = 5,
    EPI_PARTIAL = 6,
    EPI_F16_TILED = 7,
    EPI_RESID_FOLD = 8,
    EPI_QKV_FOLD = 9,
    EPI_GELU_TANH_FOLD = 10,
    EPI_F32_FOLD = 11,
};
constexpr bool epi_is_fold_consumer(int e) { return e == EPI_QKV_FOLD || e == EPI_GELU_TANH_FOLD || e == EPI_F32_FOLD; }
constexpr int epi_base(int e) { return e == EPI_QKV_FOLD ? EPI_QKV : e == EPI_GELU_TANH_FOLD ? EPI_GELU_TANH : e == EPI_F32_FOLD ? EPI_F32 : e; }

enum QkvMode : int {
    QKV_SPATIAL = 0,
    QKV_TEMPORAL = 1,
};

constexpr int GEMM_SK_MAX_SPLIT = 128;
constexpr size_t gemm_sk_ws_bytes() { return (size_t)GEMM_SK_MAX_SPLIT * 256 * 256 * 4; }
constexpr size_t gemm_sk_flag_bytes() { return (size_t)GEMM_SK_MAX_SPLIT * 4; }

#include "gemm_typed.inc"
using gtav_shared::gemm_pp_ok, gtav_shared::gemm_resid_inplace_ok, gtav_shared::gemm_choose_splitk;
#ifdef GTAV_EXPERIMENTS
void gemm_set_stamps(unsigned long long* buf, int max_blocks);
#endif

}
```

### ai-generated-gtav_amd/csrc/gemm.hip

```cpp
#include "gemm.h"
#include "attn_tile.h"

#include <cstdlib>
#include <cstring>
#include <type_traits>
#include <hip/hip_ext.h>

namespace gtav {
using namespace gtav_shared;

namespace {

constexpr int TN = 128, TK = 64;
constexpr int TILE_BYTES = 128 * TK * 2;

typedef const __attribute__((address_space(1))) void* gptr_t;
typedef __attribute__((address_space(3))) void* lptr_t;

__device__ __forceinline__ void glds16(const char* src, char* lds_wave_base) {
    __builtin_amdgcn_global_load_lds((gptr_t)src, (lptr_t)lds_wave_base, 16, 0, 0);
}

__device__ __forceinline__ void glds16_s(const void* sbase, unsigned voff, unsigned lds_addr) {
    unsigned keep;
// ... 1057 lines not shown
                const int nb = m / p.S;
                tok_a[j] = nb;
                tok_b[j] = m - nb * p.S;
                tok_pos[j] = tok_b[j];
            } else {
                const int fr = m / p.S;
                const int b = fr / p.Tq;
                const int tfr = p.t0 + (fr - b * p.Tq);
                tok_a[j] = (b * p.Tmax + tfr) * p.S + (m - fr * p.S);
                tok_b[j] = 0;
                tok_pos[j] = tfr;
            }
        }
    }
    if constexpr (EPI == EPI_RESID && !FOLD) {
        int grow[FJ];
#pragma unroll
        for (int j = 0; j < FJ; ++j) {
            int mm = m0 + 16 * FJ * wm + 16 * j + li;
            mm = mm < p.M ? mm : p.M - 1;
            grow[j] = 0;
            if (p.gate) {
                grow[j] = mm / p.rows_per_gate;
                if (p.gate_rows) grow[j] = p.gate_rows[grow[j]];
            }
        }
        f32x4 xo[2][FJ], gt[2][FJ];
        auto loads = [&](int i, f32x4 (&xv)[FJ], f32x4 (&gv)[FJ]) {
            const int n = n0 + 16 * FI * wn + 16 * i + 4 * g;
#pragma unroll
            for (int j = 0; j < FJ; ++j) {
                const int m = m0 + 16 * FJ * wm + 16 * j + li;
                xv[j] = f32x4{0.f, 0.f, 0.f, 0.f};
                gv[j] = f32x4{1.f, 1.f, 1.f, 1.f};
                if (n < p.N && m < p.M) {
                    xv[j] = *(const f32x4*)((const float*)p.out + (size_t)m * p.ldo + n);
                    if (p.gate) gv[j] = *(const f32x4*)(p.gate + (size_t)grow[j] * p.gate_stride + n);
                }
            }
        };
        loads(0, xo[0], gt[0]);
#pragma unroll
        for (int i = 0; i < FI; ++i) {
            if (i + 1 < FI) loads(i + 1, xo[(i + 1) & 1], gt[(i + 1) & 1]);
            const int n = n0 + 16 * FI * wn + 16 * i + 4 * g;
#pragma unroll
            for (int j = 0; j < FJ; ++j) {
                const int m = m0 + 16 * FJ * wm + 16 * j + li;
                if (n < p.N && m < p.M) {
                    const f32x4 x = xo[i & 1][j] + gt[i & 1][j] * (acc[i][j] + pbias[i]);
                    float* dst = (float*)p.out + (size_t)m * p.ldo + n;
                    if (p.out_sc1) store16_sc1(dst, x);
                    else *(f32x4*)dst = x;
                }
            }
        }
        return;
    }
#pragma unroll
    for (int i = 0; i < FI; ++i) {
        const int n = n0 + 16 * FI * wn + 16 * i + 4 * g;
        if (n >= p.N) continue;
        const f32x4 bv = pbias[i];
        int which = 0, nn = n, head = 0, d = 0;
        if constexpr (EPI == EPI_QKV) {
            which = n >= 2 * p.D ? 2 : (n >= p.D ? 1 : 0);
            nn = n - which * p.D;
            head = nn >> 6;
            d = nn & 63;
        }
#pragma unroll
        for (int j = 0; j < FJ; ++j) {
            const int m = m0 + 16 * FJ * wm + 16 * j + li;
            if (m >= p.M) continue;
            f32x4 v;
            if constexpr (FOLD) {
                const float* cf = (const float*)ft.cb + fold_frame_of(ft, m0 + 16 * FJ * wm + 16 * j) * 2 * TNB + (n - n0);
                v = fold_apply(acc[i][j], ft.mu[j], ft.rs[j], *(const f32x4*)cf, *(const f32x4*)(cf + TNB));
            } else {
                v = acc[i][j] + bv;
            }
            if constexpr (EPI == EPI_PARTIAL) {
                float* dst = (float*)p.out + ((size_t)ks * p.M + m) * p.ldo + n;
                if (p.out_sc1) store16_sc1(dst, v);
                else *(f32x4*)dst = v;
            } else if constexpr (EPI == EPI_F32) {
                *(f32x4*)((float*)p.out + (size_t)m * p.ldo + n) = v;
            } else if constexpr (EPI == EPI_F16) {
                *(uint2*)((f16*)p.out + (size_t)m * p.ldo + n) = pack4(amax, v[0], v[1], v[2], v[3]);
            } else if constexpr (EPI == EPI_QKV) {
                if (which < 2) {
                    const f32x4 cs = *(const f32x4*)(rope_tab(p, n) + tok_pos[j] * 64 + d);
                    v = rope4(v, cs);
                }
                const uint2 pk = pack4(amax, v[0], v[1], v[2], v[3]);
                if (p.qkv_mode == QKV_SPATIAL) {
                    const int heads = p.D >> 6;
                    f16* base = which == 0 ? p.q : p.k;
                    f16* dst = base + ((size_t)(tok_a[j] * heads + head) * p.S + tok_b[j]) * 64 + d;
                    *(uint2*)dst = pk;
                } else {
                    if (which == 0) {
                        *(uint2*)(p.q + (size_t)m * p.D + nn) = pk;
                    } else {
                        f16* base = p.k + (size_t)tok_a[j] * 2 * p.D + (which == 2 ? p.D : 0);
                        *(uint2*)(base + nn) = pk;
// ... 1282 lines not shown
    if (tn) {
        GTAV_REQUIRE(K % 128 == 0, "gemm_dw_grouped: the transpose-free form contracts over whole 128-token row tiles (K=%d)", K);
        GTAV_LAUNCH(gemm256_dw_grouped_kernel<true>, dim3(gs.first[n]), dim3(512), 0, stream, p, gs);
    } else {
        GTAV_LAUNCH(gemm256_dw_grouped_kernel<false>, dim3(gs.first[n]), dim3(512), 0, stream, p, gs);
    }
    GTAV_CHECK_HIP(hipGetLastError());
    return 0;
}

int launch_gemm_grouped(const GemmGroup* groups_dev, int n_groups, int max_N, int M, int K, hipStream_t stream) {
    GTAV_REQUIRE(groups_dev && n_groups > 0 && n_groups < 65536 && M > 0 && max_N > 0 && K > 0 && K % TK == 0, "gemm_grouped: bad arguments");
    GemmParams p;
    memset(&p, 0, sizeof(p));
    p.M = M; p.N = max_N; p.K = K; p.splitk = 1;
    const dim3 grid(cdiv(M, 96) * cdiv(max_N, 128), n_groups);
    hipLaunchKernelGGL((gemm_grouped_kernel<4, 4, 2, 3>), grid, dim3(384), 0, stream, p, groups_dev);
    GTAV_CHECK_HIP(hipGetLastError());
    return 0;
}


int launch_gemm(const GemmParams& p_in, int epi_x, hipStream_t stream) {
    GemmParams p = p_in;
    const int epi = epi_base(epi_x);
    const bool fold_c = epi_is_fold_consumer(epi_x), fold_p = epi_x == EPI_RESID_FOLD;
    if (fold_c || fold_p) {
        GTAV_REQUIRE(p.f_P > 0 && p.f_P % 16 == 0 && p.M % p.f_P == 0, "gemm/fold: %d tokens per frame must be a multiple of 16 and divide M=%d", p.f_P, p.M);
        if (fold_c) {
            GTAV_REQUIRE(p.f_stats && p.f_c1 && p.f_c2 && p.f_ldc >= p.N && p.f_nslot == p.K / 64 && p.f_nslot % 4 == 0,
                         "gemm/fold: consumer needs the row statistics (K/64 = %d slots, a multiple of 4) and the c1 / c2 tables", p.K / 64);
            GTAV_REQUIRE(!p.bias, "gemm/fold: the bias of a fold consumer lives in its c2 table");
            if (epi == EPI_QKV) GTAV_REQUIRE(p.qkv_mode == QKV_TEMPORAL || p.S % 16 == 0, "gemm/fold: spatial QKV needs S %% 16 == 0");
        } else {
            GTAV_REQUIRE(p.gate && p.f_scale && p.f_stats_out && p.f_a && p.N % 64 == 0 && p.ldo >= p.N,
                         "gemm/fold: producer needs gate, next scale, statistics and operand buffers, N %% 64 == 0");
        }
    }
    GTAV_REQUIRE(prefetch_desc_ok(p.pf), "gemm: bad prefetch descriptor (row tiles %d, K tiles %d, K slices %d)", p.pf.rt, p.pf.nkt, p.pf.splitk);
    GTAV_REQUIRE(p.K > 0 && p.K % TK == 0, "gemm: K=%d must be a positive multiple of %d", p.K, TK);
    GTAV_REQUIRE(p.M > 0 && p.N > 0 && p.N % 4 == 0, "gemm: bad M=%d N=%d", p.M, p.N);
    GTAV_REQUIRE(((uintptr_t)p.X & 15) == 0 && ((uintptr_t)p.W & 15) == 0, "gemm: operands must be 16-byte aligned");
    if (epi == EPI_QKV) {
        GTAV_REQUIRE(p.N == 3 * p.D && p.D % 128 == 0, "gemm/qkv: N=%d must equal 3*D, D=%d %% 128 == 0", p.N, p.D);
        GTAV_REQUIRE(p.S > 0 && p.q && p.k && p.rope_cs, "gemm/qkv: missing buffers");
        if (p.qkv_mode == QKV_SPATIAL) {
            GTAV_REQUIRE(p.S % 4 == 0 && p.M % p.S == 0 && p.v, "gemm/qkv spatial: S=%d must divide M=%d, S %% 4 == 0", p.S, p.M);
        } else {
            GTAV_REQUIRE(p.Tq > 0 && p.M % (p.S * p.Tq) == 0 && p.t0 + p.Tq <= p.Tmax, "gemm/qkv temporal: bad frame geometry");
        }
    } else {
        GTAV_REQUIRE(p.out && p.ldo >= p.N && p.ldo % 4 == 0, "gemm: bad output ldo=%d", p.ldo);
        if (epi == EPI_RESID && p.gate) GTAV_REQUIRE(p.rows_per_gate > 0, "gemm/resid: rows_per_gate");
        if (epi == EPI_GELU_TANH || epi == EPI_GELU_ERF || epi == EPI_F16_TILED) GTAV_REQUIRE(p.ldo % 64 == 0, "gemm/gelu: tile-major output needs ldo %% 64 == 0");
        if (fold_p) GTAV_REQUIRE(p.splitk <= 1, "gemm/fold: the producer epilogue needs the complete sum (no split-K)");
        if (epi == EPI_PARTIAL) GTAV_REQUIRE(p.splitk >= 1 && (p.K / TK) % p.splitk == 0, "gemm/partial: splitk=%d must divide K/64=%d", p.splitk, p.K / TK);
    }
    GemmPlan plan;
    if (int rc_ = gemm_plan(GemmProblem{p.M, p.N, p.K, epi_x, p.qkv_mode, p.S, p.splitk, p.gate ? p.rows_per_gate : 0}, &plan)) return rc_;
    if (fold_c || fold_p) {
        const int span = gemm_shape(plan.shape)->span();
        GTAV_REQUIRE(p.f_P >= span, "gemm/fold: frames of %d tokens are shorter than the token span (%d) of a wave of block shape %d", p.f_P, span, plan.shape);
    }
    const int dbg = gemm_debug();
    p.tm.gn = plan.gn;
    lab_fields(p, 3 | 16 | 32 | 2048 | 8192 | 16384 | 0x1F0000);
    p.out_sc1 = (dbg & 8) ? 0 : 1;
    if (dbg & 0x800000) p.pf.next = nullptr;
    switch (epi_x) {
#ifdef GTAV_EXPERIMENTS
        case EPI_RESID_FOLD: return launch_epi<EPI_RESID_FOLD>(p, plan, stream);
        case EPI_QKV_FOLD: return launch_epi<EPI_QKV_FOLD>(p, plan, stream);
        case EPI_GELU_TANH_FOLD: return launch_epi<EPI_GELU_TANH_FOLD>(p, plan, stream);
        case EPI_F32_FOLD: return launch_epi<EPI_F32_FOLD>(p, plan, stream);
#else
        case EPI_RESID_FOLD: case EPI_QKV_FOLD: case EPI_GELU_TANH_FOLD: case EPI_F32_FOLD:
            GTAV_REQUIRE(false, "gemm: the LayerNorm-fold epilogues exist only in the experiments build (csrc/build.sh exp)");
#endif
        case EPI_F32: return launch_epi<EPI_F32>(p, plan, stream);
        case EPI_F16: return launch_epi<EPI_F16>(p, plan, stream);
        case EPI_GELU_TANH: return launch_epi<EPI_GELU_TANH>(p, plan, stream);
        case EPI_GELU_ERF: return launch_epi<EPI_GELU_ERF>(p, plan, stream);
        case EPI_RESID: return launch_epi<EPI_RESID>(p, plan, stream);
        case EPI_QKV: return launch_epi<EPI_QKV>(p, plan, stream);
        case EPI_PARTIAL: return launch_epi<EPI_PARTIAL>(p, plan, stream);
        case EPI_F16_TILED: return launch_epi<EPI_F16_TILED>(p, plan, stream);
        default: GTAV_REQUIRE(false, "gemm: unknown epilogue %d", epi_x);
    }
    return 0;
}

}
```

### ai-generated-gtav_amd/csrc/gemm_plan.h

```cpp
#pragma once

namespace gtav_shared {

constexpr int GEMM_TK = 64;

enum GemmFamily : int {
    GF_K128,
    GF_G,
    GF_T256,
    GF_L,
    GF_LP,
    GF_LW,
    GF_LAB,
};

struct GemmShape {
    int id, family;
    int ns;
    int fi, fj, wn, wm, nl;
    bool product;
    constexpr int tokens() const { return 16 * fj * wm; }
    constexpr int features() const { return 16 * fi * wn; }
    constexpr int threads() const { return 64 * (wn * wm + nl); }
    constexpr int span() const { return 16 * fj; }
// ... 6 lines not shown
    {7,  GF_T256,   2, 8, 4, 2, 4, 0, true},
    {8,  GF_G,      4, 3, 2, 2, 3, 0, false},
    {9,  GF_G,      4, 4, 2, 2, 3, 0, false},
    {11, GF_G,      4, 2, 1, 2, 3, 0, true},
    {12, GF_G,      2, 4, 3, 2, 4, 0, true},
    {13, GF_G,      2, 4, 3, 2, 2, 0, true},
    {14, GF_G,      4, 2, 2, 2, 3, 0, true},
    {16, GF_LAB,    3, 4, 3, 2, 4, 8, false},
    {17, GF_T256,   2, 8, 4, 2, 4, 0, false},
    {18, GF_LW,     4, 1, 6, 8, 1, 4, false},
    {20, GF_L,      4, 2, 3, 4, 2, 4, true},
    {21, GF_L,      3, 4, 4, 4, 2, 4, false},
    {22, GF_LW,     4, 2, 3, 4, 2, 4, false},
    {23, GF_L,      4, 4, 3, 2, 2, 4, false},
    {24, GF_L,      4, 2, 1, 2, 3, 2, true},
    {25, GF_L,      5, 2, 3, 4, 2, 4, false},
    {26, GF_L,      4, 2, 2, 2, 3, 2, true},
    {27, GF_L,      8, 2, 1, 2, 3, 2, false},
    {28, GF_L,      8, 2, 1, 2, 3, 4, false},
    {29, GF_L,      4, 2, 3, 4, 3, 4, true},
    {30, GF_LP,     4, 4, 3, 2, 4, 4, false},
    {31, GF_LP,     3, 4, 3, 2, 4, 4, true},
    {32, GF_LP,     3, 4, 4, 4, 2, 4, false},
    {33, GF_LP,     3, 4, 4, 2, 4, 4, false},
    {40, GF_LAB,    2, 8, 4, 2, 4, 0, false},
    {41, GF_LAB,    2, 6, 4, 2, 4, 0, false},
    {42, GF_LAB,    2, 4, 4, 4, 4, 0, false},
};

constexpr const GemmShape* gemm_shape(int id) {
    for (const GemmShape& s : GEMM_SHAPES)
        if (s.id == id) return &s;
    return nullptr;
}
inline int gemm_tiles(int shape, int M, int N) {
    const GemmShape& s = *gemm_shape(shape);
    return ((M + s.tokens() - 1) / s.tokens()) * ((N + s.features() - 1) / s.features());
}

struct GemmProblem { int M, N, K, epi, qkv_mode, S, splitk, rows_per_gate; };
struct GemmPlan { int shape, ns, splitk, gn, tile_tokens, tile_features, blocks, threads; };

constexpr bool GEMM_LAB_BUILD = GTAV_LAB_BUILD;

int gemm_plan(const GemmProblem& g, GemmPlan* plan, bool lab = GEMM_LAB_BUILD);
int gemm_choose_gn(int M, int N, int K, int tmb, int tnb, int splitk, bool lab = GEMM_LAB_BUILD);
bool gemm_pp_ok(int M, int N, int K, int epi, bool lab = GEMM_LAB_BUILD);
bool gemm_resid_inplace_ok(int M, int N, int K, int rows_per_gate, bool lab = GEMM_LAB_BUILD);
int gemm_choose_splitk(int M, int N, int K, bool lab = GEMM_LAB_BUILD);

void gemm_set_stages(int ns);
void gemm_set_wm(int wm);
bool gemm_forced_wfill();
int gemm_debug(bool lab = GEMM_LAB_BUILD);
void gemm_set_debug(int bits);

}
```

### ai-generated-gtav_amd/csrc/gemm_plan.hip

```cpp
#include "gemm.h"

#include <cstdlib>

namespace gtav_shared {
using namespace gtav;

static thread_local int t_force_stages = 0, t_force_shape = 0, t_force_wfill = 0;
static thread_local int t_env_shape = GTAV_ENV_INT("GTAV_GEMM_SHAPE", 0);
void gemm_set_stages(int ns) { t_force_stages = ns; }
void gemm_set_wm(int wm) { t_force_shape = wm & 0xFF; t_force_wfill = wm >> 8 & 1; t_env_shape = 0; }
bool gemm_forced_wfill() { return t_force_wfill != 0; }
static int forced_shape(bool lab) { return t_force_shape ? t_force_shape : lab ? t_env_shape : 0; }

struct LabKnobs {
    int debug = 0;
    int lp = 1;
    int resid_inplace = 1;
    int splitk_old = 0;
    int l_for_8 = 1;
    int gn = 0;
    int pp = 0;
};
static const LabKnobs g_lab_off = {};
#ifdef GTAV_EXPERIMENTS
static LabKnobs g_lab = {GTAV_ENV_INT("GTAV_GEMM_DEBUG", 0), GTAV_ENV_INT("GTAV_LP", 1), GTAV_ENV_INT("GTAV_RESID_INPLACE", 1), GTAV_ENV_INT("GTAV_SPLITK_OLD", 0),
                         GTAV_ENV_INT("GTAV_L_FOR_8", 1), GTAV_ENV_INT("GTAV_GEMM_GN", 0), GTAV_ENV_INT("GTAV_PP", 0)};
static const LabKnobs& knobs(bool lab) { return lab ? g_lab : g_lab_off; }
void gemm_set_debug(int bits) { g_lab.debug = bits; }
bool gemm_pp_ok(int M, int N, int K, int epi, bool lab) {
    if (!(epi == EPI_GELU_TANH || epi == EPI_GELU_ERF || epi == EPI_QKV || epi == EPI_RESID)) return false;
    if (K % GEMM_TK != 0 || K / GEMM_TK < 14 || M % 8 != 0 || N % 8 != 0) return false;
    return knobs(lab).pp && gemm_tiles(16, M, N) >= 224;
}
static int lab_shape_for_20(const LabKnobs& k, bool foldish, int ksteps) {
    int wm = (k.debug & 128) ? 25 : 20;
    if (wm == 20 && (k.debug & 0x1000000) && !foldish && ksteps % 4 == 0) wm = 22;
    if (wm == 20 && (k.debug & 0x2000000) && !foldish && ksteps % 8 == 0) wm = 18;
    return wm;
}
static int lab_shape_for_fc1(const LabKnobs& k, int wm, int epi_x, int M, int N) {
    if (epi_x == EPI_GELU_TANH && (k.debug & 0x600000) && cdiv(M, 128) * cdiv(N, 256) >= 512) return (k.debug & 0x200000) ? 33 : 32;
    return wm;
}
#else
static const LabKnobs& knobs(bool) { return g_lab_off; }
bool gemm_pp_ok(int, int, int, int, bool) { return false; }
static int lab_shape_for_20(const LabKnobs&, bool, int) { return 20; }
static int lab_shape_for_fc1(const LabKnobs&, int wm, int, int, int) { return wm; }
#endif
int gemm_debug(bool lab) { return knobs(lab).debug; }

static bool lp_takes(int M, int N, int K, bool lab) { return knobs(lab).lp && N <= 2048 && N % 8 == 0 && K >= 512 && gemm_tiles(31, M, N) >= 160; }
bool gemm_resid_inplace_ok(int M, int N, int K, int rows_per_gate, bool lab) {
    const int forced = forced_shape(lab);
    return knobs(lab).resid_inplace && lp_takes(M, N, K, lab) && (rows_per_gate == 0 || rows_per_gate >= 32) && (forced == 0 || forced == 31);
}
int gemm_choose_splitk(int M, int N, int K, bool lab) {
    if (lp_takes(M, N, K, lab)) return 1;
    if (knobs(lab).debug & 256) return 1;
    const int tiles = gemm_tiles(3, M, N);
    int s = 1;
    const int min_slice = (tiles >= 48 && !knobs(lab).splitk_old) ? 512 : 256;
    while (tiles * s < 192 && s < 8 && (K / GEMM_TK) % (s * 2) == 0 && K / (s * 2) >= min_slice) s *= 2;
    if (s == 1 && K >= 4096 && (K / GEMM_TK) % 2 == 0) {
// ... 100 lines not shown
```

### ai-generated-gtav_amd/csrc/gemm_typed.inc

```
struct GemmParams {
    const f16* X;
    int ldx;
    int wfill;
    const f16* W;
    int M, N, K;
    int debug;
    unsigned long long* stamps;
    int* err_flag;
    int out_sc1;
    int splitk;
    const float* bias;
    void* out2;
    void* out;
    int ldo;
    const float* gate;
    int gate_stride;
    const int* gate_rows;
    int rows_per_gate;
    int qkv_mode;
    f16* q;
    f16* k;
    f16* v;
    int D;
    int S;
    int Tq;
    int t0;
    int Tmax;
    const float* rope_cs;
    const float* rope_cs_q;
    struct TileMap { int tiles_m, tiles_n, gn, group, tiles; unsigned rcp_tiles, rcp_group, rcp_gn, rcp_gnlast; } tm;
    int f_P;
    const int* f_rows;
    const float* f_stats;
    int f_nslot;
    const float* f_c1;
    const float* f_c2;
    int f_ldc;
    float* f_stats_out;
    const float* f_scale;
    f16* f_a;
    PrefetchDesc pf;
    float* sk_ws;
    int* sk_flags;
    int sk_dp, sk_r;
};
static_assert(sizeof(GemmParams) == 352, "GemmParams: every build and both operand types must see the same struct");

struct GemmGroup { const f16* X; const f16* W; float* out; const float* bias; int N; int ldo; };
int launch_gemm_grouped(const GemmGroup* groups_dev, int n_groups, int max_N, int M, int K, hipStream_t stream);

constexpr int GEMM_DW_MAX_GROUPS = 4;
struct GemmDwGroup { const f16* X; const f16* W; float* out; int M; int N; int ldo; };
static_assert(sizeof(GemmDwGroup) == 40, "GemmDwGroup: every build and both operand types must see the same struct");
bool gemm_dw_grouped_ok(const GemmDwGroup* g, int n, int K);
int launch_gemm_dw_grouped(const GemmDwGroup* g, int n, int K, int* err_flag, hipStream_t stream, bool tn = false);

int launch_gemm(const GemmParams& p, int epi, hipStream_t stream);
bool gemm_qkvt_attn_ok(int M, int D, int S, int Tq, int t0);
int launch_gemm_qkvt_attn(const GemmParams& p, hipStream_t stream);
bool gemm_qkvs_attn_ok(int M, int D, int S);
int launch_gemm_qkvs_attn(const GemmParams& p, hipStream_t stream);
bool gemm_tn_ok(int M, int N, int K);
bool gemm_tn_pays(int M, int N, int K);
int launch_gemm_tn(const GemmParams& p, hipStream_t stream);
```

### ai-generated-gtav_amd/csrc/ops.h

```cpp
#pragma once
#include "common.h"
#include "gemm.h"

namespace gtav {

#include "ops_typed.inc"

int launch_skinny_f32(const float* X, int ldx, const float* W, const float* bias, float* Y, int ldy, int M, int N,
                      int K, int act_silu, hipStream_t stream);
int skinny_init();

struct StepParams {
    int first;
    int cur;
    int t_ctx;
    int t_cur;
    int is_final;
    float alpha_t, alpha_next;
    int cond_step;
};
int launch_step_setup(StepParams* dst, const StepParams& v, int* frame_idx, int* mod_rows, int* last_rows, int* changed, int B, int Tq, int T, int F,
                      int use_cur, hipStream_t stream);
int launch_gather_rows(const float* table, const int* rows, const int* changed, float* cur, int slots, int W, const float* table2, float* cur2, int W2,
                       hipStream_t stream);
int launch_cond_inputs_frame(int rows, int B, int T, int F, int start, int cur, int t_ctx, const int* t_steps, const float* sincos,
                             float* E, const float* actions, int A, float* HC, int ldhc, int D, int Apad, int* err_flag,
                             hipStream_t stream);

int launch_unpatchify(const float* y, int ldy, float* img, int NB, int C, int H, int W, int p, int order, float a,
                      float b, hipStream_t stream);

int launch_copy_f32_strided(const float* src, int lds, int R, int C, float* dst, int ldd, hipStream_t stream);
int launch_copy_rows_f32(const float* src, size_t src_stride, float* dst, size_t dst_stride, int rows, size_t n, hipStream_t stream);
int launch_clamp_cols(float* buf, int M, int ld, int c0, int c1, float lo, float hi, hipStream_t stream);
int launch_frames_to_u8(const float* img, uint8_t* out, int N, int H, int W, hipStream_t stream);
int launch_moments_to_latents(const float* mom, float* lat, int N, int hw, int latent, int mom_ch, float scale, hipStream_t stream);
int launch_latents_to_tokens(const float* lat, float* z, int N, int hw, int latent, hipStream_t stream);
int launch_resize_aa(const void* src, int src_is_u8_strip, float* dst, int n, int H, int W, int OH, int OW, hipStream_t stream);
int launch_copy_f32(const float* src, int lds, int R, int C, float* dst, int ldd, int c0, hipStream_t stream);
int launch_fill_f32(float* dst, size_t n, float v, hipStream_t stream);
int launch_rope_interleave(const float* cos_t, const float* sin_t, float* cs, int npos, hipStream_t stream);
int launch_add_f32(const float* a, const float* b, float* out, size_t n, hipStream_t stream);
int launch_calib_spin(unsigned long long ticks, unsigned long long* dev_ticks, hipStream_t stream);
int launch_axpy_f32(float* y, const float* x, float alpha, size_t n, hipStream_t stream);

int launch_cond_inputs(const int64_t* t64, int rows, int Tq, const StepParams* sp, int use_cur, const float* sincos ,
                       float* E, const float* actions, int64_t act_outer, int64_t act_inner, int A, float* HC, int ldhc,
                       int D, int Apad, int* err_flag, hipStream_t stream);

int launch_ddim_update(const float* x, size_t x_stride, const float* v, size_t v_stride, float* out, size_t out_stride,
                       int B, int n, const float* alpha_t, const float* alpha_next, int is_final, hipStream_t stream);
int launch_ddim_update_step(float* x, size_t frames_per_sample, const float* v, size_t v_stride, int B, int n,
                            const StepParams* sp, hipStream_t stream);

int launch_add_noise(const float* x, const float* noise, const float* alpha , float* out, int rows, int n,
                     float clamp_abs, hipStream_t stream);
int launch_vtarget(const float* x, const float* noise, const float* alpha , float* vt, int rows, int n,
                   float clamp_abs, hipStream_t stream);
int launch_mse(const float* a, size_t a_stride, const float* b, size_t b_stride, int rows, int n, float* out_scalar,
               hipStream_t stream);

struct RngDraw {
    uint64_t seed;
    uint32_t draw, sample0, slot0, slots_per_sample;
};
int launch_rng_bits(uint32_t* out, int rows, int n, const RngDraw& d, hipStream_t stream);
int launch_rng_normal(float* out, size_t sample_stride, int rows, int n, const RngDraw& d, float clamp_abs, hipStream_t stream);
int launch_noise_window_rng(const float* x, const float* alpha , float* x_noisy, float* v_target , int B, int W, int n, const RngDraw& d,
                            float clamp_abs, hipStream_t stream);
int launch_vae_posterior_sample(const float* moments, float* z, int frames, int tokens, int L, const RngDraw& d, hipStream_t stream);

int launch_ln_mod_bwd(const float* dxn, const float* x, const float* scale, int mod_stride, int rows_per_mod, int M, int D, float* dres, int accumulate,
                      float* stats, hipStream_t stream);
// ... 30 lines not shown
```

### ai-generated-gtav_amd/csrc/ops_bf16.h

```cpp
#pragma once
#include "ops.h"

namespace gtav_bf16 {
typedef __bf16 f16;
using gtav_shared::PrefetchDesc;
#include "gemm_typed.inc"
#include "ops_typed.inc"
}

namespace gtav {

#define GTAV_OPERAND_OPS(F)                                 \
    F(gemm, launch_gemm)                                    \
    F(ln_modulate, launch_ln_modulate)                      \
    F(ln_affine, launch_ln_affine)                          \
    F(patchify, launch_patchify)                            \
    F(convert_pad, launch_convert_pad_f16)                  \
    F(unpad, launch_unpad_f16_to_f32)                       \
    F(attn_spatial, launch_attn_spatial)                    \
    F(attn_temporal, launch_attn_temporal)                  \
                     \
    F(gemm_tn, launch_gemm_tn)                              \
    F(gemm_dw_grouped, launch_gemm_dw_grouped)              \
    F(transpose_tiled, launch_transpose_tiled_f16)          \
    F(convert_T, launch_convert_T_f16)                      \
    F(gelu_tiled, launch_gelu_tiled)                        \
    F(gelu_bwd_tiled, launch_gelu_bwd_tiled)                \
    F(gelu_bwd_tiled_colsum, launch_gelu_bwd_tiled_colsum)  \
    F(gate_bwd, launch_gate_bwd)                            \
    F(frame_reduce_gate, launch_frame_reduce_gate)          \
    F(gate_bwd_fused, launch_gate_bwd_fused)                \
    F(colsum_tiled, launch_colsum_tiled_f16)                \
    F(to_tiled, launch_to_tiled_f16)                        \
    F(mse_bwd_patch, launch_mse_bwd_patch)                  \
    F(attn_spatial_bwd, launch_attn_spatial_bwd)            \
    F(attn_temporal_bwd, launch_attn_temporal_bwd)          \
    F(adamw_multi, launch_adamw_multi)                      \
    F(branch_rows, launch_branch_rows)

struct OperandOps {
#define GTAV_OPS_FIELD(field, launcher) decltype(&launcher) field;
    GTAV_OPERAND_OPS(GTAV_OPS_FIELD)
#undef GTAV_OPS_FIELD
    bool bf16;
};
const OperandOps& operand_ops(bool bf16);

}
```

### ai-generated-gtav_amd/csrc/ops_typed.inc

```

int launch_ctab_inputs(const float* mod, int MODW, int R, int Rp, int D, const int* col, const int* is_scale, int n_groups, f16* sx, size_t group_stride,
                       hipStream_t stream);

struct LnPending {
    const float* parts;
    int nsplit;
    size_t slab_stride;
    int ld;
    const float* bias;
    const float* gate;
    int gate_stride;
    const int* gate_rows;
    int rows_per_gate;
    int flags;
    int* err_flag;
    float* x_out;
    f16* y_save;
    int tperm_T, tperm_P;
    float* k_save;
    const float* k_load;
};
static_assert(sizeof(LnPending) == 120, "LnPending: every build and both operand types must see the same struct");

int launch_ln_modulate(float* x, int ldx, f16* out, int ldo, int M, int D, const float* shift, const float* scale,
                       int mod_stride, const int* rows, int rows_per_mod, const LnPending* pend, int* err_flag, hipStream_t stream);
int launch_ln_affine(float* x, int ldx, f16* out, int ldo, int M, int D, const float* gamma, const float* beta,
                     const LnPending* pend, int* err_flag, hipStream_t stream);
int launch_branch_rows(const float* parts, int nsplit, size_t slab_stride, int ld, const float* bias, f16* y, int M, int N, int* err_flag, hipStream_t stream);

int launch_patchify(const float* img, const int* frame_index, int NB, int C, int H, int W, int p, f16* out, int ldo,
                    float a, float b, int* err_flag, hipStream_t stream);

int launch_convert_pad_f16(const float* src, int lds, int R, int C, f16* dst, int Rp, int Cp, float scale, int tiled,
                           hipStream_t stream, int* err_flag = nullptr);
int launch_unpad_f16_to_f32(const f16* src, int lds, int R, int C, float* dst, int tiled, hipStream_t stream);
int launch_qkv_head_major(const f16* src, f16* dst, int D, hipStream_t stream, int mode = 0);

int launch_transpose_tiled_f16(const f16* src, int R, int C, f16* dst, hipStream_t stream);
int launch_convert_T_f16(const float* src, int lds, int R, int C, f16* dst, hipStream_t stream);
int launch_gelu_tiled(const f16* u, f16* h, size_t n, hipStream_t stream);
int launch_gelu_bwd_tiled(const f16* dh, const f16* u, f16* du, size_t n, int* err_flag, hipStream_t stream);
int launch_gelu_bwd_tiled_colsum(const f16* dh, const f16* u, f16* du, int M, int N, float* db, float* ws, int* err_flag, hipStream_t stream);
int launch_gate_bwd(const float* dres, const float* gate, int mod_stride, int rows_per_mod, int M, int D, f16* dy_tiled, int* err_flag, hipStream_t stream);
int launch_frame_reduce_gate(const float* dres, const f16* y, int frames, int P, int D, float* dgate, int mod_stride, hipStream_t stream);
int launch_gate_bwd_fused(const float* dres, const f16* y, const float* gate, int mod_stride, int frames, int P, int D, f16* dy_tiled, float* dgate, float* db,
                          float* ws, int* err_flag, hipStream_t stream);
int launch_colsum_tiled_f16(const f16* dy, int M, int N, float* db, float* ws, hipStream_t stream);
int launch_to_tiled_f16(const float* a, int M, int D, f16* out, int* err_flag, hipStream_t stream);
int launch_mse_bwd_patch(const float* vpred, const float* vtarget, int B, int T, int C, int H, int W, int p, float scale, f16* dfo, int ldf, int* err_flag,
                         hipStream_t stream);
int launch_attn_spatial_bwd(const f16* Q, const f16* K, const f16* Vt, const f16* dO, int NB, int heads, int S, int D, const float* rope_cs, f16* dqkv,
                            int* err_flag, hipStream_t stream);
int launch_attn_temporal_bwd(const f16* q, const f16* kv, const f16* dO, int B, int P, int D, int T, int Tmax, const float* rope_cs, f16* dqkv, int* err_flag,
                             hipStream_t stream);
struct AdamParam {
    float* p; int ldp, R, C;
    const float* g; float *m, *v;
    f16* w16; int Cp16;
    f16* wT; int RpT;
};
static_assert(sizeof(AdamParam) == 80, "AdamParam: every build and both operand types must see the same struct");
struct AdamItem { int param; unsigned start; };
static_assert(sizeof(AdamItem) == 8, "AdamItem: every build and both operand types must see the same struct");
int launch_adamw_multi(const AdamParam* params, const AdamItem* items, int n_items, const float* ctl, float lr, float beta1, float beta2, float eps, float wd,
                       hipStream_t stream);

int launch_attn_spatial(const f16* Q, const f16* K, const f16* Vt, f16* O, int NB, int heads, int S, hipStream_t stream, bool q_prescaled = false);
int launch_attn_temporal(const f16* q, const f16* kv, f16* O, int B, int P, int D, int Tq, int t0, int Tmax,
                         hipStream_t stream);
```

### include/gtav_amd_testing.h

```cpp
#ifndef GTAV_AMD_TESTING_H
#define GTAV_AMD_TESTING_H

#include <stdint.h>

#define GTAV_GEMM_WM_NT_WEIGHT_FILLS 0x100

#ifdef __cplusplus
extern "C" {
#endif

void gtav_op_gemm_set_stages(int32_t ns);
void gtav_op_gemm_set_wm(int32_t wm);
void gtav_op_set_operand_dtype(int32_t dtype);
int gtav_op_attn_spatial_prescaled(const void* q, const void* k, const void* vt, void* o, int32_t NB, int32_t heads, int32_t S, void* stream);

int gtav_op_train_ln_mod_bwd(int32_t fused, const float* dxn, const float* x, const float* scale, int32_t mod_stride, int32_t frames, int32_t P, int32_t D,
                             float* dres, int32_t accumulate, float* dshift, float* dscale, float* ws, int64_t ws_floats, void* stream);
int gtav_op_train_gate_bwd(int32_t fused, const float* dres, const void* y, const float* gate, int32_t mod_stride, int32_t frames, int32_t P, int32_t D,
                           void* dy_tiled, float* dgate, float* db, float* ws, int64_t ws_floats, int32_t* err, void* stream);
int gtav_op_train_gelu_bwd(int32_t fused, const void* dh, const void* u, void* du, int32_t M, int32_t N, float* db, float* ws, int64_t ws_floats, int32_t* err,
                           void* stream);
int gtav_op_train_colsum_tiled(const void* dy, int32_t M, int32_t N, float* db, float* ws, int64_t ws_floats, void* stream);
int gtav_op_train_colsum_f32(const float* a, int32_t lda, int32_t M, int32_t N, float* db, float* ws, int64_t ws_floats, void* stream);
int gtav_op_train_colsum_reduce_multi(const float* const* ws, float* const* db, const int32_t* splits, const int32_t* N, int32_t njobs, void* stream);
int gtav_op_train_mse_bwd_patch(const float* vpred, const float* vtarget, int32_t B, int32_t T, int32_t C, int32_t H, int32_t W, int32_t p, float scale, void* dfo,
                                int32_t ldf, int32_t* err, void* stream);
int gtav_op_train_to_tiled(const float* a, int32_t M, int32_t D, void* out, int32_t* err, void* stream);
int gtav_op_train_transpose_tiled(const void* src, int32_t R, int32_t C, void* dst, void* stream);
int gtav_op_train_convert_t(const float* src, int32_t lds, int32_t R, int32_t C, void* dst, void* stream);
int gtav_op_train_silu(const float* x, int32_t ldx, float* y, int32_t ldy, int32_t R, int32_t C, void* stream);
int gtav_op_train_silu_bwd(const float* dy, int32_t lddy, const float* x, int32_t ldx, float* dx, int32_t lddx, int32_t R, int32_t C, void* stream);
int gtav_op_train_gemm_tn_f32(const float* dY, int32_t lddy, const float* X, int32_t ldx, int32_t R, int32_t N, int32_t K, float* dW, int32_t lddw, void* stream);
int gtav_op_train_gemm_nn_f32(const float* dY, int32_t lddy, const float* W, int32_t ldw, int32_t R, int32_t N, int32_t K, float* dX, int32_t lddx, void* stream);
int gtav_op_train_ada_bwd_dx(const float* dmod, int32_t MODW, const float* W, int32_t D, int32_t R, float* dSc, float* part, int64_t part_floats, void* stream);

int gtav_op_ln_pending(int32_t mode, float* x, int32_t ldx, void* out, int32_t M, int32_t D, const float* p0, const float* p1, int32_t mod_stride,
                       const int32_t* rows, int32_t rows_per_mod, const float* parts, int32_t nsplit, int64_t slab_stride, int32_t ld, const float* bias,
                       const float* gate, int32_t gate_stride, const int32_t* gate_rows, int32_t rows_per_gate, float* x_out, void* y_save, int32_t tperm_T,
                       int32_t tperm_P, float* k_save, const float* k_load, int32_t* err, void* stream);
int gtav_op_branch_rows(const float* parts, int32_t nsplit, int64_t slab_stride, int32_t ld, const float* bias, void* y, int32_t M, int32_t N, int32_t* err,
                        void* stream);

#ifdef __cplusplus
}
#endif
#endif
```

Baseline: 5.500.

## Fuse sampler step setup, gather and patchify into one head kernel; fuse DDIM into final GEMM

Each denoise step now starts with a single head kernel that does step setup, modulation-row gather and patchify, where before it issued separate launches. The DDIM update and the copy of the last velocity are folded into the final projection GEMM epilogue, replacing unpatchify, ddim_update and copy_rows. The head node of the captured graph is patched per step through hipGraphExecKernelNodeSetParams, and prepare_frame is skipped when its conditioning key (step list, action rows) matches the last call. This adds graph-node patching logic, fallbacks when the node cannot be updated, and a blocking device-to-host copy of the action rows on every prepare_frame call.

```diff
diff --git a/ai-generated-gtav_amd/csrc/api.hip b/ai-generated-gtav_amd/csrc/api.hip
--- a/ai-generated-gtav_amd/csrc/api.hip
+++ b/ai-generated-gtav_amd/csrc/api.hip
@@ -22,8 +22,10 @@
     static_assert(sizeof(S) == sizeof(gtav_bf16::S) && alignof(S) == alignof(gtav_bf16::S) && std::is_standard_layout<S>::value &&             \
                       std::is_standard_layout<gtav_bf16::S>::value, #S ": the fp16 and the bf16 view differ");                                  \
     template <> struct twin_arg<const S&> { typedef const gtav_bf16::S& type; };                                                                \
-    template <> struct twin_arg<const S*> { typedef const gtav_bf16::S* type; };
+    template <> struct twin_arg<const S*> { typedef const gtav_bf16::S* type; };                                                                \
+    template <> struct twin_arg<S*> { typedef gtav_bf16::S* type; };
 GTAV_TWIN_STRUCT(GemmParams)
+GTAV_TWIN_STRUCT(StepHead)
 GTAV_TWIN_STRUCT(LnPending)
 GTAV_TWIN_STRUCT(GemmDwGroup)
 GTAV_TWIN_STRUCT(AdamParam)
diff --git a/ai-generated-gtav_amd/csrc/api_dit.hip b/ai-generated-gtav_amd/csrc/api_dit.hip
--- a/ai-generated-gtav_amd/csrc/api_dit.hip
+++ b/ai-generated-gtav_amd/csrc/api_dit.hip
@@ -148,8 +148,9 @@
     return gemm_pp_ok(M, h->D, K, EPI_RESID) || (gemm_choose_splitk(M, h->D, K) == 1 && M >= h->resid_inplace_min_m) || gemm_resid_inplace_ok(M, h->D, K, h->P);
 }
 
+struct StepFuse { bool head, tail; float* x; int F; float* v_last; };
 static int dit_forward_core(gtav_dit* h, const float* x_src, const int* frame_index, int B, int Tq, int t0,
-                            const float* mod, const int* mod_rows, const float* ctab, float* v_out, hipStream_t s) {
+                            const float* mod, const int* mod_rows, const float* ctab, float* v_out, hipStream_t s, const StepFuse* sf = nullptr) {
     const int D = h->D, P = h->P, NB = B * Tq, M = NB * P;
     GTAV_REQUIRE(M <= h->Mmax, "forward: %d tokens exceed workspace (%d)", M, h->Mmax);
     bool fold_a, fold_b;
@@ -162,7 +163,7 @@
         return 0;
     };
     const int g_embed = 2 * h->L, g_final = 2 * h->L + 1;
-    PROF(h, PC_OTHER, s, h->ops(g_embed).patchify(x_src, frame_index, NB, h->C, h->H, h->W, h->p, h->xp, h->Kpe, 1.f, 0.f, h->err_of(g_embed), s));
+    if (!(sf && sf->head)) PROF(h, PC_OTHER, s, h->ops(g_embed).patchify(x_src, frame_index, NB, h->C, h->H, h->W, h->p, h->xp, h->Kpe, 1.f, 0.f, h->err_of(g_embed), s));
     GemmParams pe = gemm_params(h->xp, h->Kpe, h->w_pe, M, D, h->Kpe);
     pe.bias = h->b_pe; pe.out = h->resid; pe.ldo = D;
     PROF(h, PC_OTHER, s, h->ops(g_embed).gemm(pe, EPI_F32, s));
@@ -217,6 +218,13 @@
     GemmParams fin = gemm_params(h->xn, D, h->w_final, M, h->Nfin, D);
     fin.bias = h->b_final; fin.out = h->fo; fin.ldo = h->Nfin;
     if (folded_in) fold_consumer(h, fin, 4 * h->L, h->Nfin, mod_rows, ctab);
+    if (sf && sf->tail) {
+        GTAV_REQUIRE(!folded_in, "forward: the fused tail of a sampler step has no LayerNorm-fold form");
+        fin.out = v_out;
+        fin.dd = GemmParams::Ddim{sf->x, sf->v_last, h->step_dev, h->C, h->H, h->W, h->p, Tq, sf->F};
+        PROF(h, PC_OTHER, s, h->ops(g_final).gemm(fin, EPI_F32_DDIM, s));
+        return h->prof.collect(s);
+    }
     PROF(h, PC_OTHER, s, h->ops(g_final).gemm(fin, folded_in ? EPI_F32_FOLD : EPI_F32, s));
     PROF(h, PC_OTHER, s, launch_unpatchify(h->fo, h->Nfin, v_out, NB, h->C, h->H, h->W, h->p, 0, 1.f, 0.f, s));
     return h->prof.collect(s);
@@ -324,6 +332,8 @@
     A_(a.alloc_t(&h->err_flag, 4 + h->n_groups)); A_(a.alloc_t(&h->frame_idx, (size_t)h->maxB * h->maxT)); A_(a.alloc_t(&h->ac_table, 1000));
     A_(a.alloc_t(&h->step_dev, 4)); A_(a.alloc_t(&h->mod_rows_dev, (size_t)h->maxB * h->maxT));
     A_(a.alloc_t(&h->mod_cur, (size_t)h->maxB * h->maxT * h->MODW)); A_(a.alloc_t(&h->mod_last, (size_t)h->maxB * h->maxT)); A_(a.alloc_t(&h->mod_changed, (size_t)h->maxB * h->maxT)); A_(a.alloc_t(&h->t_steps_dev, 1024));
+    h->head_last_words = (size_t)step_head_last_words(h->maxB * h->maxT, h->MODW, 0);
+    A_(a.alloc_t(&h->head_last, h->head_last_words));
     wt.err_words = h->err_flag; wt.err_per_group = true;
     h->use_graph = GTAV_ENV_INT("GTAV_GRAPH", 1) != 0;
     h->fold.geom_ok = h->P % 16 == 0 && h->P >= 64 && D % 256 == 0 && h->Hm % 128 == 0 && h->Nfin % 4 == 0;
@@ -346,6 +356,7 @@
         n = spatial ? "spatial_rotary_emb.freqs" : "temporal_rotary_emb.freqs";
     }
     h->finalized = false;
+    h->invalidate_prepared();
     return h->wt.set(n.c_str(), src, numel, (hipStream_t)stream);
 }
 
@@ -410,7 +421,7 @@
     GTAV_REQUIRE(B >= 1 && B <= h->maxB && T >= 1 && T <= h->maxT, "dit_forward: B=%d T=%d outside capacity (%d, %d)", B, T, h->maxB, h->maxT);
     GTAV_REQUIRE(!actions || h->A > 0, "dit_forward: model has no external_cond");
     hipStream_t s = (hipStream_t)stream;
-    h->prepared.valid = false;
+    h->invalidate_prepared();
     h->kvrec.valid = false;
     RET_IF(dit_cond(h, t, B * T, 1, nullptr, 0, actions, h->A, 0, s));
     return dit_forward_core(h, x, nullptr, B, T, 0, h->mod, nullptr, h->fold.ctab, out, s);
@@ -423,12 +434,43 @@
     return 0;
 }
 
+static int step_setup_unfused(gtav_dit* h, const StepParams& sp, int B, int F, int T, int mode, bool prepared, hipStream_t s) {
+    RET_IF(launch_step_setup(h->step_dev, sp, h->frame_idx, h->mod_rows_dev, prepared ? h->mod_last : nullptr, h->mod_changed, B, mode == 1 ? 1 : T, T, F,
+                             mode == 1, s));
+    if (prepared) RET_IF(launch_gather_rows(h->mod, h->mod_rows_dev, h->mod_changed, h->mod_cur, B * (mode == 1 ? 1 : T), h->MODW,
+                                            h->prepared.fold_tables ? h->fold.ctab : nullptr, h->fold.ctab_cur, h->fold.CTW, s));
+    return 0;
+}
+
+static int step_forget_rows(gtav_dit* h, hipStream_t s) {
+    GTAV_CHECK_HIP(hipMemsetAsync(h->mod_last, 0xFF, (size_t)h->maxB * h->maxT * sizeof(int), s));
+    GTAV_CHECK_HIP(hipMemsetAsync(h->head_last, 0xFF, h->head_last_words * sizeof(int), s));
+    return 0;
+}
+
+static StepHead step_head_args(gtav_dit* h, const StepParams& sp, const float* x, int B, int F, int T, int mode, bool prepared) {
+    StepHead a;
+    memset(&a, 0, sizeof(a));
+    a.v = sp;
+    a.step_dev = h->step_dev; a.frame_idx = h->frame_idx; a.mod_rows = h->mod_rows_dev;
+    a.B = B; a.Tq = mode == 1 ? 1 : T; a.T = T; a.F = F; a.use_cur = mode == 1;
+    if (prepared) { a.table = h->mod; a.cur = h->mod_cur; a.W = h->MODW; a.last = h->head_last; }
+    a.x = x; a.xp = h->xp; a.err_flag = h->err_of(2 * h->L);
+    a.C = h->C; a.H = h->H; a.Wimg = h->W; a.p = h->p; a.ldo = h->Kpe;
+    return a;
+}
+
 static int denoise_step_body(gtav_dit* h, float* x, int B, int F, int T, const float* actions, int mode, float* v_out,
-                             bool prepared, hipStream_t s) {
+                             bool prepared, hipStream_t s, StepHead* head, bool fuse_tail) {
     const size_t fsz = (size_t)h->C * h->H * h->W;
     const int Tq = mode == 1 ? 1 : T, t0 = mode == 1 ? T - 1 : 0;
+    if (head) PROF(h, PC_OTHER, s, h->ops(2 * h->L).step_head(head, s));
     if (!prepared) RET_IF(dit_cond(h, nullptr, B * Tq, Tq, h->step_dev, mode == 1, actions, (int64_t)F * h->A, h->A, s));
-    RET_IF(dit_forward_core(h, x, h->frame_idx, B, Tq, t0, prepared ? h->mod_cur : h->mod, nullptr, prepared ? h->fold.ctab_cur : h->fold.ctab, h->vout, s));
+    bool fa, fb;
+    fold_policy(h, B * Tq * h->P, fa, fb);
+    const StepFuse sf{head != nullptr, fuse_tail && !fb, x, F, v_out};
+    RET_IF(dit_forward_core(h, x, h->frame_idx, B, Tq, t0, prepared ? h->mod_cur : h->mod, nullptr, prepared ? h->fold.ctab_cur : h->fold.ctab, h->vout, s, &sf));
+    if (sf.tail) return 0;
     const float* vlast = h->vout + (size_t)(Tq - 1) * fsz;
     RET_IF(launch_ddim_update_step(x, F, vlast, (size_t)Tq * fsz, B, (int)fsz, h->step_dev, s));
     if (v_out) RET_IF(launch_copy_rows_f32(vlast, (size_t)Tq * fsz, v_out, fsz, B, fsz, s));
@@ -446,6 +488,21 @@
     const int rows = B * (T - 1) + n_steps * B;
     GTAV_REQUIRE(rows <= h->max_rows, "prepare_frame: %d conditioning rows exceed max_cond_rows %d", rows, h->max_rows);
     hipStream_t s = (hipStream_t)stream;
+    h->prepared.B = B; h->prepared.F = F; h->prepared.start = start; h->prepared.cur = cur; h->prepared.n_steps = n_steps; h->prepared.actions = actions;
+    gtav_dit::CondKey& ck = h->cond_key;
+    std::vector<float> arows;
+    if (actions) {
+        arows.resize((size_t)B * T * h->A);
+        GTAV_CHECK_HIP(hipMemcpy2DAsync(arows.data(), (size_t)T * h->A * sizeof(float), actions + (size_t)start * h->A, (size_t)F * h->A * sizeof(float),
+                                        (size_t)T * h->A * sizeof(float), B, hipMemcpyDeviceToHost, s));
+        GTAV_CHECK_HIP(hipStreamSynchronize(s));
+    }
+    if (gtav_shared::step_fusion_mode() != 0 && ck.valid && h->prepared.valid && ck.B == B && ck.T == T && ck.t_ctx == t_ctx && ck.have_actions == (actions != nullptr) &&
+        ck.t_steps.size() == (size_t)n_steps && !memcmp(ck.t_steps.data(), t_steps_host, n_steps * sizeof(int)) && ck.action_rows.size() == arows.size() &&
+        (arows.empty() || !memcmp(ck.action_rows.data(), arows.data(), arows.size() * sizeof(float))))
+        return 0;
+    h->invalidate_prepared();
+    RET_IF(h->prof.begin(PC_OTHER, s));
     GTAV_CHECK_HIP(hipStreamSynchronize(s));
     GTAV_CHECK_HIP(hipMemcpy(h->t_steps_dev, t_steps_host, n_steps * sizeof(int), hipMemcpyHostToDevice));
     RET_IF(launch_cond_inputs_frame(rows, B, T, F, start, cur, t_ctx, h->t_steps_dev, h->sincos, h->E, actions, h->A, h->HC, h->D + h->Apad,
@@ -458,23 +515,31 @@
         RET_IF(dit_fold_tables(h, rows, fa || fa1, fb || fb1, s));
         h->prepared.fold_tables = fa || fa1 || fb || fb1;
     }
-    GTAV_CHECK_HIP(hipMemsetAsync(h->mod_last, 0xFF, (size_t)h->maxB * h->maxT * sizeof(int), s));
-    h->prepared.valid = true; h->prepared.B = B; h->prepared.F = F; h->prepared.start = start; h->prepared.cur = cur;
-    h->prepared.n_steps = n_steps; h->prepared.actions = actions;
-    return 0;
-}
-
-static int dit_step_graph(gtav_dit* h, float* x, int B, int F, int T, const float* actions, int mode, float* v_out, bool prepared, hipGraphExec_t* out) {
+    RET_IF(step_forget_rows(h, s));
+    RET_IF(h->prof.end(s));
+    h->prepared.valid = true;
+    ck.valid = true; ck.have_actions = actions != nullptr; ck.B = B; ck.T = T; ck.t_ctx = t_ctx;
+    ck.t_steps.assign(t_steps_host, t_steps_host + n_steps);
+    ck.action_rows.swap(arows);
+    return h->prof.collect(s);
+}
+
+static int dit_step_graph(gtav_dit* h, float* x, int B, int F, int T, const float* actions, int mode, float* v_out, bool prepared, StepHead* head, bool fuse_tail,
+                          gtav_dit::StepGraph** out, bool* head_ok) {
     *out = nullptr;
+    *head_ok = true;
     const gtav_dit::GraphKey key{B, F, T, mode * 2 + (prepared ? 1 : 0), x, actions, v_out};
     auto it = h->graphs.find(key);
     if (it == h->graphs.end()) {
         if (h->graphs.size() > 64) h->drop_graphs();
-        h->graphs[key] = nullptr;
+        h->graphs[key] = gtav_dit::StepGraph();
         return 0;
     }
-    *out = it->second;
-    if (*out) return 0;
+    gtav_dit::StepGraph& g = it->second;
+    if (g.exec) {
+        *out = &g;
+        return 0;
+    }
     hipGraph_t graph = nullptr;
     hipGraphExec_t exec = nullptr;
     int rc = 0;
@@ -483,14 +548,39 @@
         (void)hipGetLastError();
         ok = false;
     } else if (ok) {
-        rc = denoise_step_body(h, x, B, F, T, actions, mode, v_out, prepared, h->cap_stream);
+        rc = denoise_step_body(h, x, B, F, T, actions, mode, v_out, prepared, h->cap_stream, head, fuse_tail);
         ok = hipStreamEndCapture(h->cap_stream, &graph) == hipSuccess && !rc && graph;
+        if (ok && head) {
+            hipGraphNode_t root = nullptr;
+            size_t n_roots = 0;
+            hipGraphNodeType type;
+            *head_ok = hipGraphGetRootNodes(graph, nullptr, &n_roots) == hipSuccess && n_roots == 1 && hipGraphGetRootNodes(graph, &root, &n_roots) == hipSuccess &&
+                       root && hipGraphNodeGetType(root, &type) == hipSuccess && type == hipGraphNodeTypeKernel &&
+                       hipGraphKernelNodeGetParams(root, &g.head_kp) == hipSuccess &&
+                       g.head_kp.gridDim.x == (unsigned)(head->nb_patch + head->B * head->Tq * head->nb_gather + 1) && g.head_kp.blockDim.x == 256;
+            if (!*head_ok) (void)hipGetLastError();
+            g.head = *head_ok ? root : nullptr;
+            g.head_args = *head;
+            ok = *head_ok;
+        }
         ok = ok && hipGraphInstantiate(&exec, graph, nullptr, nullptr, 0) == hipSuccess && exec;
-        if (graph) (void)hipGraphDestroy(graph);
-    }
-    if (ok) *out = it->second = exec;
-    else h->use_graph = false;
+        if (graph && !(ok && head)) (void)hipGraphDestroy(graph);
+    }
+    if (ok) {
+        g.exec = exec;
+        g.graph = head ? graph : nullptr;
+        *out = &g;
+    } else if (*head_ok) {
+        h->use_graph = false;
+    }
     return rc;
+}
+
+static int step_head_give_up(gtav_dit* h, const char* why, hipStream_t s) {
+    h->head_refused = true;
+    h->drop_graphs();
+    set_error("denoise_step: %s; this handle runs the step's setup launches in front of its captured steps from now on (same results)", why);
+    return step_forget_rows(h, s);
 }
 
 int gtav_dit_denoise_step(gtav_dit* h, float* x, int32_t B, int32_t F, int32_t start, int32_t cur, int32_t t_ctx,
@@ -509,7 +599,7 @@
                          h->prepared.cur == cur && cond_step < h->prepared.n_steps && h->prepared.actions == actions,
                      "denoise_step: cond_step=%d but gtav_dit_prepare_frame was not called for this window", cond_step);
     else
-        h->prepared.valid = false;
+        h->invalidate_prepared();
     if (mode == 1) {
         GTAV_REQUIRE(h->kvrec.valid && h->kvrec.B == B && h->kvrec.F == F && h->kvrec.start == start && h->kvrec.cur == cur &&
                          h->kvrec.x == (const void*)x,
@@ -522,14 +612,44 @@
     StepParams sp;
     sp.first = start; sp.cur = cur; sp.t_ctx = t_ctx; sp.t_cur = t_cur; sp.is_final = is_final != 0;
     sp.alpha_t = h->ac_host[t_cur]; sp.alpha_next = h->ac_host[t_next]; sp.cond_step = cond_step;
-    RET_IF(launch_step_setup(h->step_dev, sp, h->frame_idx, h->mod_rows_dev, prepared ? h->mod_last : nullptr, h->mod_changed, B, mode == 1 ? 1 : T, T, F,
-                             mode == 1, s));
-    if (prepared) RET_IF(launch_gather_rows(h->mod, h->mod_rows_dev, h->mod_changed, h->mod_cur, B * (mode == 1 ? 1 : T), h->MODW,
-                                            h->prepared.fold_tables ? h->fold.ctab : nullptr, h->fold.ctab_cur, h->fold.CTW, s));
-    hipGraphExec_t exec = nullptr;
-    if (h->use_graph && !h->prof.on) RET_IF(dit_step_graph(h, x, B, F, T, actions, mode, v_out, prepared, &exec));
-    if (!exec) return denoise_step_body(h, x, B, F, T, actions, mode, v_out, prepared, s);
-    GTAV_CHECK_HIP(hipGraphLaunch(exec, s));
+    const int fusion = gtav_shared::step_fusion_mode();
+    if (fusion != h->step_fusion) {
+        h->step_fusion = fusion;
+        h->drop_graphs();
+        RET_IF(step_forget_rows(h, s));
+    }
+    const bool fuse_tail = fusion != 0;
+    const bool fuse_head = fusion != 0 && !h->head_refused && !(prepared && h->prepared.fold_tables);
+    StepHead head = step_head_args(h, sp, x, B, F, T, mode, prepared);
+    if (!fuse_head) RET_IF(step_setup_unfused(h, sp, B, F, T, mode, prepared, s));
+    gtav_dit::StepGraph* g = nullptr;
+    if (h->use_graph && !h->prof.on) {
+        bool head_ok = true;
+        RET_IF(dit_step_graph(h, x, B, F, T, actions, mode, v_out, prepared, fuse_head ? &head : nullptr, fuse_tail, &g, &head_ok));
+        if (!head_ok) {
+            RET_IF(step_head_give_up(h, "the captured step does not start with its head launch", s));
+            RET_IF(step_setup_unfused(h, sp, B, F, T, mode, prepared, s));
+            return denoise_step_body(h, x, B, F, T, actions, mode, v_out, prepared, s, nullptr, fuse_tail);
+        }
+    }
+    if (!g) return denoise_step_body(h, x, B, F, T, actions, mode, v_out, prepared, s, fuse_head ? &head : nullptr, fuse_tail);
+    if (g->head) {
+        g->head_args.v = sp;
+        void* args[1] = {&g->head_args};
+        hipKernelNodeParams kp = g->head_kp;
+        kp.kernelParams = args;
+        kp.extra = nullptr;
+        const hipError_t e = fusion == 2 ? hipErrorNotSupported : hipGraphExecKernelNodeSetParams(g->exec, g->head, &kp);
+        if (e != hipSuccess) {
+            (void)hipGetLastError();
+            char why[160];
+            snprintf(why, sizeof(why), "the runtime refused to update the head node of a captured step (%s)", hipGetErrorString(e));
+            RET_IF(step_head_give_up(h, why, s));
+            RET_IF(step_setup_unfused(h, sp, B, F, T, mode, prepared, s));
+            return denoise_step_body(h, x, B, F, T, actions, mode, v_out, prepared, s, nullptr, fuse_tail);
+        }
+    }
+    GTAV_CHECK_HIP(hipGraphLaunch(g->exec, s));
     return 0;
 }
 
@@ -572,7 +692,7 @@
     if (min_tokens_b >= 0) h->fold.min_m_b = min_tokens_b;
     if (mode == 2 || (mode == 1 && (h->fold.min_m_a < (1 << 30) || h->fold.min_m_b < (1 << 30)))) RET_IF(fold_alloc(h));
     h->drop_graphs();
-    h->prepared.valid = false;
+    h->invalidate_prepared();
     h->fold.mode = mode;
     return 0;
 }
@@ -657,6 +777,7 @@
     if (changed) {
         h->finalized = false;
         h->kvrec.valid = false;
+        h->invalidate_prepared();
         h->drop_graphs();
     }
     h->any_bf16 = false;
diff --git a/ai-generated-gtav_amd/csrc/api_internal.h b/ai-generated-gtav_amd/csrc/api_internal.h
--- a/ai-generated-gtav_amd/csrc/api_internal.h
+++ b/ai-generated-gtav_amd/csrc/api_internal.h
@@ -344,8 +344,26 @@
             return std::tie(B, F, T, mode, x, actions, vout) < std::tie(o.B, o.F, o.T, o.mode, o.x, o.actions, o.vout);
         }
     };
-    std::map<GraphKey, hipGraphExec_t> graphs;
+    struct StepGraph {
+        hipGraphExec_t exec = nullptr;
+        hipGraph_t graph = nullptr;
+        hipGraphNode_t head = nullptr;
+        hipKernelNodeParams head_kp;
+        StepHead head_args;
+    };
+    std::map<GraphKey, StepGraph> graphs;
     bool use_graph = true;
+    int step_fusion = 1;
+    bool head_refused = false;
+    int* head_last = nullptr;
+    size_t head_last_words = 0;
+    struct CondKey {
+        bool valid = false, have_actions = false;
+        int B = 0, T = 0, t_ctx = 0;
+        std::vector<int> t_steps;
+        std::vector<float> action_rows;
+    } cond_key;
+    void invalidate_prepared() { prepared.valid = false; cond_key.valid = false; }
     bool fuse_tattn = false;
     bool fuse_sattn = false;
     bool w_prefetch = true;
@@ -366,8 +384,10 @@
     } fold;
     hipStream_t cap_stream = nullptr;
     void drop_graphs() {
-        for (auto& kv : graphs)
-            if (kv.second) (void)hipGraphExecDestroy(kv.second);
+        for (auto& kv : graphs) {
+            if (kv.second.exec) (void)hipGraphExecDestroy(kv.second.exec);
+            if (kv.second.graph) (void)hipGraphDestroy(kv.second.graph);
+        }
         graphs.clear();
     }
     ~gtav_dit() {
diff --git a/ai-generated-gtav_amd/csrc/api_train.hip b/ai-generated-gtav_amd/csrc/api_train.hip
--- a/ai-generated-gtav_amd/csrc/api_train.hip
+++ b/ai-generated-gtav_amd/csrc/api_train.hip
@@ -336,7 +336,7 @@
     hipStream_t s = (hipStream_t)stream;
     gtav_dit::Train& tr = h->tr;
     const int D = h->D, P = h->P, NB = B * T, M = NB * P, L = h->L, rows = NB, ldhc = D + h->Apad;
-    h->prepared.valid = false;
+    h->invalidate_prepared();
     h->kvrec.valid = false;
     tr.rc_block = -1;
     RET_IF(launch_cond_inputs(t64, rows, 1, nullptr, 0, h->sincos, h->E, actions, h->A, 0, h->A, h->HC, ldhc, D, h->Apad, h->err_flag, s));
@@ -590,7 +590,7 @@
         if (tr.adam_n[ty])
             RET_IF(operand_ops(ty != 0).adamw_multi(tr.adam_params, tr.adam_items + (ty ? tr.adam_n[0] : 0), tr.adam_n[ty], tr.ctl, lr, beta1, beta2, eps, weight_decay, s));
     RET_IF(launch_add_f32(h->b_t2, h->b_ext, h->b_t2a, h->D, s));
-    h->prepared.valid = false;
+    h->invalidate_prepared();
     h->kvrec.valid = false;
     return 0;
 }
@@ -635,7 +635,7 @@
     for (unsigned char b : h->grp_bf16) h->any_bf16 |= b != 0;
     h->tr.have_fwd = false;
     h->tr.rc_block = -1;
-    h->prepared.valid = false;
+    h->invalidate_prepared();
     h->kvrec.valid = false;
     h->drop_graphs();
     GTAV_CHECK_HIP(hipStreamSynchronize(s));
diff --git a/ai-generated-gtav_amd/csrc/common.h b/ai-generated-gtav_amd/csrc/common.h
--- a/ai-generated-gtav_amd/csrc/common.h
+++ b/ai-generated-gtav_amd/csrc/common.h
@@ -106,9 +106,26 @@
     int rt, nkt, splitk;
     int kt_limit;
 };
+struct StepParams {
+    int first;
+    int cur;
+    int t_ctx;
+    int t_cur;
+    int is_final;
+    float alpha_t, alpha_next;
+    int cond_step;
+};
 }
 namespace gtav {
 using gtav_shared::PrefetchDesc;
+using gtav_shared::StepParams;
+__device__ __forceinline__ float ddim_one(float xc, float vp, float at, float an, int is_final) {
+#pragma clang fp contract(off)
+    const float x0 = __builtin_fmaf(sqrtf(at), xc, -(sqrtf(1.0f - at) * vp));
+    if (is_final) return x0;
+    const float eps = __builtin_fmaf(sqrtf(1.0f / at), xc, -x0) / sqrtf(1.0f / at - 1.0f);
+    return sqrtf(an) * x0 + sqrtf(1.0f - an) * eps;
+}
 __device__ __forceinline__ void l2_prefetch_slice(const PrefetchDesc& d, int xcd, int j, int nb, int t, int nt, unsigned& sink) {
     const int sk = d.splitk;
     int ks0, ksn, rt0, rtn;
diff --git a/ai-generated-gtav_amd/csrc/elementwise.hip b/ai-generated-gtav_amd/csrc/elementwise.hip
--- a/ai-generated-gtav_amd/csrc/elementwise.hip
+++ b/ai-generated-gtav_amd/csrc/elementwise.hip
@@ -195,26 +195,31 @@
     sat_report(am, err_flag);
 }
 
+template <class FrameOf>
+__device__ __forceinline__ void patchify_elem(const float* __restrict__ img, FrameOf frame_of, size_t idx, int C, int H, int W, int p, f16* __restrict__ out, int ldo,
+                                              float a, float b, int* err_flag) {
+    const int gh = H / p, gw = W / p, Kp = C * p * p;
+    const int k = (int)(idx % ldo);
+    const size_t m = idx / ldo;
+    float val = 0.f;
+    if (k < Kp) {
+        const int pw = k % p, ph = (k / p) % p, c = k / (p * p);
+        const int x = (int)(m % gw), y = (int)((m / gw) % gh), nb = (int)(m / ((size_t)gw * gh));
+        const int f = frame_of(nb);
+        val = a * img[(((size_t)f * C + c) * H + (y * p + ph)) * W + (x * p + pw)] + b;
+        if (!(__builtin_fabsf(val) <= F16_MAX)) {
+            if (err_flag) atomicOr(err_flag, val != val || __builtin_isinf(val) ? ERR_NONFINITE : ERR_F16_SAT);
+            if (val == val) val = __builtin_amdgcn_fmed3f(val, -F16_MAX, F16_MAX);
+        }
+    }
+    out[tiled_off((int)m, k, ldo)] = (f16)val;
+}
+
 __global__ void patchify_kernel(const float* __restrict__ img, const int* __restrict__ frame_index, int NB, int C, int H,
                                 int W, int p, f16* __restrict__ out, int ldo, float a, float b, int* err_flag) {
-    const int gh = H / p, gw = W / p, Kp = C * p * p;
-    const size_t total = (size_t)NB * gh * gw * ldo;
-    for (size_t idx = (size_t)blockIdx.x * blockDim.x + threadIdx.x; idx < total; idx += (size_t)gridDim.x * blockDim.x) {
-        const int k = (int)(idx % ldo);
-        const size_t m = idx / ldo;
-        float val = 0.f;
-        if (k < Kp) {
-            const int pw = k % p, ph = (k / p) % p, c = k / (p * p);
-            const int x = (int)(m % gw), y = (int)((m / gw) % gh), nb = (int)(m / ((size_t)gw * gh));
-            const int f = frame_index ? frame_index[nb] : nb;
-            val = a * img[(((size_t)f * C + c) * H + (y * p + ph)) * W + (x * p + pw)] + b;
-            if (!(__builtin_fabsf(val) <= F16_MAX)) {
-                if (err_flag) atomicOr(err_flag, val != val || __builtin_isinf(val) ? ERR_NONFINITE : ERR_F16_SAT);
-                if (val == val) val = __builtin_amdgcn_fmed3f(val, -F16_MAX, F16_MAX);
-            }
-        }
-        out[tiled_off((int)m, k, ldo)] = (f16)val;
-    }
+    const size_t total = (size_t)NB * (H / p) * (W / p) * ldo;
+    for (size_t idx = (size_t)blockIdx.x * blockDim.x + threadIdx.x; idx < total; idx += (size_t)gridDim.x * blockDim.x)
+        patchify_elem(img, [&](int nb) { return frame_index ? frame_index[nb] : nb; }, idx, C, H, W, p, out, ldo, a, b, err_flag);
 }
 
 __global__ __launch_bounds__(256) void patchify4_kernel(const float* __restrict__ img, const int* __restrict__ frame_index, int C, int H, int W, int p,
@@ -338,6 +343,47 @@
         const size_t c = ((size_t)(blockIdx.x - nb1) * 256 + threadIdx.x) * 4;
         if (c >= (size_t)W2) return;
         *(f32x4*)(cur2 + (size_t)slot * W2 + c) = *(const f32x4*)(table2 + (size_t)rows[slot] * W2 + c);
+    }
+}
+
+__global__ __launch_bounds__(256) void step_head_kernel(StepHead a) {
+    const StepParams v = a.v;
+    const int first = a.use_cur ? v.cur : v.first, slots = a.B * a.Tq;
+    const int bid = blockIdx.x;
+    if (bid < a.nb_patch) {
+        const size_t total = (size_t)slots * (a.H / a.p) * (a.Wimg / a.p) * a.ldo;
+        for (size_t idx = (size_t)bid * 256 + threadIdx.x; idx < total; idx += (size_t)a.nb_patch * 256)
+            patchify_elem(a.x, [&](int nb) { const int b = nb / a.Tq; return b * a.F + first + (nb - b * a.Tq); }, idx, a.C, a.H, a.Wimg, a.p, a.xp, a.ldo, 1.f, 0.f,
+                          a.err_flag);
+        return;
+    }
+    const int gid = bid - a.nb_patch;
+    if (gid < slots * a.nb_gather) {
+        const int slot = gid / a.nb_gather, g = gid - slot * a.nb_gather;
+        const int b = slot / a.Tq, tw = a.use_cur ? a.T - 1 : slot - b * a.Tq;
+        const int r = tw < a.T - 1 ? b * (a.T - 1) + tw : a.B * (a.T - 1) + v.cond_step * a.B + b;
+        const bool same = a.last[gid] == r;
+        __syncthreads();
+        if (same) return;
+        if (threadIdx.x == 0) a.last[gid] = r;
+        const int nb1 = (a.W + 1023) >> 10;
+        if (g < nb1) {
+            const size_t c = ((size_t)g * 256 + threadIdx.x) * 4;
+            if (c < (size_t)a.W) *(f32x4*)(a.cur + (size_t)slot * a.W + c) = *(const f32x4*)(a.table + (size_t)r * a.W + c);
+        } else {
+            const size_t c = ((size_t)(g - nb1) * 256 + threadIdx.x) * 4;
+            if (c < (size_t)a.W2) *(f32x4*)(a.cur2 + (size_t)slot * a.W2 + c) = *(const f32x4*)(a.table2 + (size_t)r * a.W2 + c);
+        }
+        return;
+    }
+    if (threadIdx.x == 0) *a.step_dev = v;
+    for (int i = threadIdx.x; i < slots; i += 256) {
+        const int b = i / a.Tq, tl = i - b * a.Tq;
+        a.frame_idx[i] = b * a.F + first + tl;
+        if (v.cond_step >= 0) {
+            const int tw = a.use_cur ? a.T - 1 : tl;
+            a.mod_rows[i] = tw < a.T - 1 ? b * (a.T - 1) + tw : a.B * (a.T - 1) + v.cond_step * a.B + b;
+        }
     }
 }
 
@@ -417,13 +463,6 @@
     for (int j = threadIdx.x; j < 256; j += blockDim.x) E[(size_t)r * 256 + j] = sincos[(size_t)t * 256 + j];
     const float* arow = actions ? actions + ro * act_outer + (frame0 + ri) * act_inner : nullptr;
     for (int j = threadIdx.x; j < Apad; j += blockDim.x) HC[(size_t)r * ldhc + D + j] = (arow && j < A) ? arow[j] : 0.f;
-}
-
-__device__ __forceinline__ float ddim_one(float xc, float vp, float at, float an, int is_final) {
-    const float x0 = sqrtf(at) * xc - sqrtf(1.0f - at) * vp;
-    if (is_final) return x0;
-    const float eps = (sqrtf(1.0f / at) * xc - x0) / sqrtf(1.0f / at - 1.0f);
-    return sqrtf(an) * x0 + sqrtf(1.0f - an) * eps;
 }
 
 __global__ void ddim_update_kernel(const float* __restrict__ x, size_t x_stride, const float* __restrict__ v, size_t v_stride,
@@ -876,6 +915,25 @@
     return 0;
 }
 
+int step_head_last_words(int slots, int W, int W2) { return slots * (cdiv(W, 1024) + cdiv(W2, 1024)); }
+
+int launch_step_head(StepHead* a, hipStream_t stream) {
+    GTAV_REQUIRE(a && a->step_dev && a->frame_idx && a->mod_rows && a->x && a->xp && a->B > 0 && a->Tq > 0 && a->T >= a->Tq, "step_head: missing buffers / bad window");
+    GTAV_REQUIRE(a->p > 0 && a->H % a->p == 0 && a->Wimg % a->p == 0 && a->ldo >= a->C * a->p * a->p, "step_head: bad patch geometry");
+    if (a->table) {
+        GTAV_REQUIRE(a->cur && a->last && a->W > 0 && a->W % 4 == 0 && a->W2 % 4 == 0 && (!a->table2 || (a->cur2 && a->W2 > 0)) && a->v.cond_step >= 0,
+                     "step_head: gather W=%d W2=%d cond_step=%d", a->W, a->W2, a->v.cond_step);
+        if (!a->table2) a->W2 = 0;
+        a->nb_gather = cdiv(a->W, 1024) + cdiv(a->W2, 1024);
+    } else {
+        a->nb_gather = 0;
+    }
+    a->nb_patch = grid_for((size_t)a->B * a->Tq * (a->H / a->p) * (a->Wimg / a->p) * a->ldo);
+    hipLaunchKernelGGL(step_head_kernel, dim3(a->nb_patch + a->B * a->Tq * a->nb_gather + 1), dim3(256), 0, stream, *a);
+    GTAV_CHECK_HIP(hipGetLastError());
+    return 0;
+}
+
 int launch_ctab_inputs(const float* mod, int MODW, int R, int Rp, int D, const int* col, const int* is_scale, int n_groups, f16* sx, size_t group_stride,
                        hipStream_t stream) {
     GTAV_REQUIRE(D % 64 == 0 && Rp % 128 == 0 && R <= Rp && n_groups > 0, "ctab_inputs: bad geometry");
diff --git a/ai-generated-gtav_amd/csrc/gemm.h b/ai-generated-gtav_amd/csrc/gemm.h
--- a/ai-generated-gtav_amd/csrc/gemm.h
+++ b/ai-generated-gtav_amd/csrc/gemm.h
@@ -17,9 +17,10 @@
     EPI_QKV_FOLD = 9,
     EPI_GELU_TANH_FOLD = 10,
     EPI_F32_FOLD = 11,
+    EPI_F32_DDIM = 12,
 };
 constexpr bool epi_is_fold_consumer(int e) { return e == EPI_QKV_FOLD || e == EPI_GELU_TANH_FOLD || e == EPI_F32_FOLD; }
-constexpr int epi_base(int e) { return e == EPI_QKV_FOLD ? EPI_QKV : e == EPI_GELU_TANH_FOLD ? EPI_GELU_TANH : e == EPI_F32_FOLD ? EPI_F32 : e; }
+constexpr int epi_base(int e) { return e == EPI_QKV_FOLD ? EPI_QKV : e == EPI_GELU_TANH_FOLD ? EPI_GELU_TANH : e == EPI_F32_FOLD || e == EPI_F32_DDIM ? EPI_F32 : e; }
 
 enum QkvMode : int {
     QKV_SPATIAL = 0,
diff --git a/ai-generated-gtav_amd/csrc/gemm.hip b/ai-generated-gtav_amd/csrc/gemm.hip
--- a/ai-generated-gtav_amd/csrc/gemm.hip
+++ b/ai-generated-gtav_amd/csrc/gemm.hip
@@ -1133,6 +1133,54 @@
                     float* dst = (float*)p.out + (size_t)m * p.ldo + n;
                     if (p.out_sc1) store16_sc1(dst, x);
                     else *(f32x4*)dst = x;
+                }
+            }
+        }
+        return;
+    }
+    if constexpr (EPIX == EPI_F32_DDIM) {
+        const GemmParams::Ddim& d = p.dd;
+        const int gw = d.W / d.p, P = (d.H / d.p) * gw, HW = d.H * d.W;
+        const size_t fsz = (size_t)d.C * HW;
+        const int cur = d.sp->cur, fin = d.sp->is_final;
+        const float at = d.sp->alpha_t, an = d.sp->alpha_next;
+        size_t img_off[FJ], x_off[FJ], vo_off[FJ];
+        bool newest[FJ];
+#pragma unroll
+        for (int j = 0; j < FJ; ++j) {
+            const int m = m0 + 16 * FJ * wm + 16 * j + li;
+            const int mm = m < p.M ? m : p.M - 1;
+            const int nb = mm / P, t = mm - nb * P, gy = t / gw, gx = t - gy * gw, b = nb / d.Tq;
+            const size_t pix = (size_t)(gy * d.p) * d.W + gx * d.p;
+            img_off[j] = (size_t)nb * fsz + pix;
+            newest[j] = nb - b * d.Tq == d.Tq - 1;
+            x_off[j] = ((size_t)b * d.F + cur) * fsz + pix;
+            vo_off[j] = (size_t)b * fsz + pix;
+        }
+#pragma unroll
+        for (int i = 0; i < FI; ++i) {
+            const int n = n0 + 16 * FI * wn + 16 * i + 4 * g;
+            if (n >= p.N) continue;
+            const f32x4 bv = pbias[i];
+            int f_off[4];
+#pragma unroll
+            for (int e = 0; e < 4; ++e) {
+                const int q = (n + e) / d.C, c = (n + e) - q * d.C, ph = q / d.p, pw = q - ph * d.p;
+                f_off[e] = c * HW + ph * d.W + pw;
+            }
+#pragma unroll
+            for (int j = 0; j < FJ; ++j) {
+                const int m = m0 + 16 * FJ * wm + 16 * j + li;
+                if (m >= p.M) continue;
+                const f32x4 v = acc[i][j] + bv;
+#pragma unroll
+                for (int e = 0; e < 4; ++e) {
+                    ((float*)p.out)[img_off[j] + f_off[e]] = v[e];
+                    if (newest[j]) {
+                        float* xe = d.x + x_off[j] + f_off[e];
+                        *xe = ddim_one(*xe, v[e], at, an, fin);
+                        if (d.v_out) d.v_out[vo_off[j] + f_off[e]] = v[e];
+                    }
                 }
             }
         }
@@ -2521,12 +2569,18 @@
     } else {
         GTAV_REQUIRE(p.out && p.ldo >= p.N && p.ldo % 4 == 0, "gemm: bad output ldo=%d", p.ldo);
         if (epi == EPI_RESID && p.gate) GTAV_REQUIRE(p.rows_per_gate > 0, "gemm/resid: rows_per_gate");
+        if (epi_x == EPI_F32_DDIM) {
+            const GemmParams::Ddim& d = p.dd;
+            GTAV_REQUIRE(d.x && d.sp && d.C > 0 && d.p > 0 && d.H > 0 && d.W > 0 && d.H % d.p == 0 && d.W % d.p == 0 && d.Tq > 0 && d.F > 0, "gemm/ddim: missing buffers / bad geometry");
+            const int P = (d.H / d.p) * (d.W / d.p);
+            GTAV_REQUIRE(p.N == d.C * d.p * d.p && p.M % P == 0 && (p.M / P) % d.Tq == 0, "gemm/ddim: M=%d N=%d do not describe whole windows of %d frames of %d tokens x %d features", p.M, p.N, d.Tq, P, d.C * d.p * d.p);
+        }
         if (epi == EPI_GELU_TANH || epi == EPI_GELU_ERF || epi == EPI_F16_TILED) GTAV_REQUIRE(p.ldo % 64 == 0, "gemm/gelu: tile-major output needs ldo %% 64 == 0");
         if (fold_p) GTAV_REQUIRE(p.splitk <= 1, "gemm/fold: the producer epilogue needs the complete sum (no split-K)");
         if (epi == EPI_PARTIAL) GTAV_REQUIRE(p.splitk >= 1 && (p.K / TK) % p.splitk == 0, "gemm/partial: splitk=%d must divide K/64=%d", p.splitk, p.K / TK);
     }
     GemmPlan plan;
-    if (int rc_ = gemm_plan(GemmProblem{p.M, p.N, p.K, epi_x, p.qkv_mode, p.S, p.splitk, p.gate ? p.rows_per_gate : 0}, &plan)) return rc_;
+    if (int rc_ = gemm_plan(GemmProblem{p.M, p.N, p.K, epi_x == EPI_F32_DDIM ? (int)EPI_F32 : epi_x , p.qkv_mode, p.S, p.splitk, p.gate ? p.rows_per_gate : 0}, &plan)) return rc_;
     if (fold_c || fold_p) {
         const int span = gemm_shape(plan.shape)->span();
         GTAV_REQUIRE(p.f_P >= span, "gemm/fold: frames of %d tokens are shorter than the token span (%d) of a wave of block shape %d", p.f_P, span, plan.shape);
@@ -2547,6 +2601,7 @@
             GTAV_REQUIRE(false, "gemm: the LayerNorm-fold epilogues exist only in the experiments build (csrc/build.sh exp)");
 #endif
         case EPI_F32: return launch_epi<EPI_F32>(p, plan, stream);
+        case EPI_F32_DDIM: return launch_epi<EPI_F32_DDIM>(p, plan, stream);
         case EPI_F16: return launch_epi<EPI_F16>(p, plan, stream);
         case EPI_GELU_TANH: return launch_epi<EPI_GELU_TANH>(p, plan, stream);
         case EPI_GELU_ERF: return launch_epi<EPI_GELU_ERF>(p, plan, stream);
diff --git a/ai-generated-gtav_amd/csrc/gemm_plan.h b/ai-generated-gtav_amd/csrc/gemm_plan.h
--- a/ai-generated-gtav_amd/csrc/gemm_plan.h
+++ b/ai-generated-gtav_amd/csrc/gemm_plan.h
@@ -82,6 +82,7 @@
 void gemm_set_stages(int ns);
 void gemm_set_wm(int wm);
 bool gemm_forced_wfill();
+int step_fusion_mode();
 int gemm_debug(bool lab = GEMM_LAB_BUILD);
 void gemm_set_debug(int bits);
 
diff --git a/ai-generated-gtav_amd/csrc/gemm_plan.hip b/ai-generated-gtav_amd/csrc/gemm_plan.hip
--- a/ai-generated-gtav_amd/csrc/gemm_plan.hip
+++ b/ai-generated-gtav_amd/csrc/gemm_plan.hip
@@ -8,8 +8,10 @@
 static thread_local int t_force_stages = 0, t_force_shape = 0, t_force_wfill = 0;
 static thread_local int t_env_shape = GTAV_ENV_INT("GTAV_GEMM_SHAPE", 0);
 void gemm_set_stages(int ns) { t_force_stages = ns; }
-void gemm_set_wm(int wm) { t_force_shape = wm & 0xFF; t_force_wfill = wm >> 8 & 1; t_env_shape = 0; }
+static thread_local int t_step_fusion = 1;
+void gemm_set_wm(int wm) { t_force_shape = wm & 0xFF; t_force_wfill = wm >> 8 & 1; t_step_fusion = wm & 0x200 ? 0 : wm & 0x400 ? 2 : 1; t_env_shape = 0; }
 bool gemm_forced_wfill() { return t_force_wfill != 0; }
+int step_fusion_mode() { return t_step_fusion; }
 static int forced_shape(bool lab) { return t_force_shape ? t_force_shape : lab ? t_env_shape : 0; }
 
 struct LabKnobs {
diff --git a/ai-generated-gtav_amd/csrc/gemm_typed.inc b/ai-generated-gtav_amd/csrc/gemm_typed.inc
--- a/ai-generated-gtav_amd/csrc/gemm_typed.inc
+++ b/ai-generated-gtav_amd/csrc/gemm_typed.inc
@@ -43,8 +43,9 @@
     float* sk_ws;
     int* sk_flags;
     int sk_dp, sk_r;
+    struct Ddim { float* x; float* v_out; const StepParams* sp; int C, H, W, p, Tq, F; } dd;
 };
-static_assert(sizeof(GemmParams) == 352, "GemmParams: every build and both operand types must see the same struct");
+static_assert(sizeof(GemmParams) == 400, "GemmParams: every build and both operand types must see the same struct");
 
 struct GemmGroup { const f16* X; const f16* W; float* out; const float* bias; int N; int ldo; };
 int launch_gemm_grouped(const GemmGroup* groups_dev, int n_groups, int max_N, int M, int K, hipStream_t stream);
diff --git a/ai-generated-gtav_amd/csrc/ops.h b/ai-generated-gtav_amd/csrc/ops.h
--- a/ai-generated-gtav_amd/csrc/ops.h
+++ b/ai-generated-gtav_amd/csrc/ops.h
@@ -10,15 +10,6 @@
                       int K, int act_silu, hipStream_t stream);
 int skinny_init();
 
-struct StepParams {
-    int first;
-    int cur;
-    int t_ctx;
-    int t_cur;
-    int is_final;
-    float alpha_t, alpha_next;
-    int cond_step;
-};
 int launch_step_setup(StepParams* dst, const StepParams& v, int* frame_idx, int* mod_rows, int* last_rows, int* changed, int B, int Tq, int T, int F,
                       int use_cur, hipStream_t stream);
 int launch_gather_rows(const float* table, const int* rows, const int* changed, float* cur, int slots, int W, const float* table2, float* cur2, int W2,
diff --git a/ai-generated-gtav_amd/csrc/ops_bf16.h b/ai-generated-gtav_amd/csrc/ops_bf16.h
--- a/ai-generated-gtav_amd/csrc/ops_bf16.h
+++ b/ai-generated-gtav_amd/csrc/ops_bf16.h
@@ -4,6 +4,7 @@
 namespace gtav_bf16 {
 typedef __bf16 f16;
 using gtav_shared::PrefetchDesc;
+using gtav_shared::StepParams;
 #include "gemm_typed.inc"
 #include "ops_typed.inc"
 }
@@ -15,6 +16,7 @@
     F(ln_modulate, launch_ln_modulate)                      \
     F(ln_affine, launch_ln_affine)                          \
     F(patchify, launch_patchify)                            \
+    F(step_head, launch_step_head)                          \
     F(convert_pad, launch_convert_pad_f16)                  \
     F(unpad, launch_unpad_f16_to_f32)                       \
     F(attn_spatial, launch_attn_spatial)                    \
diff --git a/ai-generated-gtav_amd/csrc/ops_typed.inc b/ai-generated-gtav_amd/csrc/ops_typed.inc
--- a/ai-generated-gtav_amd/csrc/ops_typed.inc
+++ b/ai-generated-gtav_amd/csrc/ops_typed.inc
@@ -30,6 +30,25 @@
 
 int launch_patchify(const float* img, const int* frame_index, int NB, int C, int H, int W, int p, f16* out, int ldo,
                     float a, float b, int* err_flag, hipStream_t stream);
+
+struct StepHead {
+    StepParams v;
+    StepParams* step_dev;
+    int *frame_idx, *mod_rows;
+    int B, Tq, T, F, use_cur;
+    int W, W2;
+    const float* table; float* cur;
+    const float* table2; float* cur2;
+    int* last;
+    const float* x;
+    f16* xp;
+    int* err_flag;
+    int C, H, Wimg, p, ldo;
+    int nb_patch, nb_gather;
+};
+static_assert(sizeof(StepHead) == 184, "StepHead: every build and both operand types must see the same struct");
+int step_head_last_words(int slots, int W, int W2);
+int launch_step_head(StepHead* a, hipStream_t stream);
 
 int launch_convert_pad_f16(const float* src, int lds, int R, int C, f16* dst, int Rp, int Cp, float scale, int tiled,
                            hipStream_t stream, int* err_flag = nullptr);
diff --git a/include/gtav_amd_testing.h b/include/gtav_amd_testing.h
--- a/include/gtav_amd_testing.h
+++ b/include/gtav_amd_testing.h
@@ -4,6 +4,8 @@
 #include <stdint.h>
 
 #define GTAV_GEMM_WM_NT_WEIGHT_FILLS 0x100
+#define GTAV_GEMM_WM_STEP_UNFUSED 0x200
+#define GTAV_GEMM_WM_STEP_UPDATE_REFUSED 0x400
 
 #ifdef __cplusplus
 extern "C" {
```

After: 5.514 (median of 2 runs). No clear change (+0.3%).
